# automerge/automerge-classic

Hardware: AMD Instinct MI355X
Metric: CRDT ops/sec applied (bulk replay) (higher is better)
Workload: dtype u32

## Files before the change

### automerge_classic_amd/csrc/am355_api.hip

```cpp
#include "am355_ctx.h"
#include "am355_scan.h"

static bool ctx_init(am355_ctx* c) {
  {
    unsigned hw = std::thread::hardware_concurrency();
    const char* env = getenv("AM355_HOST_THREADS");
    unsigned want = env && atoi(env) > 0 ? (unsigned)atoi(env) : std::min(hw ? hw : 4u, 64u);
    c->pool.reset(new HostPool(want > 1 ? want - 1 : 0));
  }
  int prio_low = 0, prio_high = 0;
  (void)hipDeviceGetStreamPriorityRange(&prio_low, &prio_high);
  auto make_stream = [](Stream& s, int prio) { return hipStreamCreateWithPriority(&s.h, hipStreamNonBlocking, prio) == hipSuccess; };
  if (!make_stream(c->stream, prio_high)) return false;
  {
    const char* env = getenv("AM355_HASH_CUS");
    int want = env ? atoi(env) : 0;
    bool made = false;
    if (want > 0) {
      hipDeviceProp_t prop;
      if (hipGetDeviceProperties(&prop, c->device) == hipSuccess && prop.multiProcessorCount > want) {
        int n_cu = prop.multiProcessorCount;
        std::vector<uint32_t> mask((size_t)(n_cu + 31) / 32, 0u);
        for (int k = 0; k < want; k++) { int cu = n_cu - 1 - k; mask[(size_t)cu / 32] |= 1u << (cu % 32); }
        made = hipExtStreamCreateWithCUMask(&c->stream2.h, (uint32_t)mask.size(), mask.data()) == hipSuccess;
// ... 54 lines not shown
extern "C" int am355_get_hashes(const am355_ctx* c, uint8_t* out) {
  if (!c || !out) return AM355_E_ARG;
  if (!c->replayed || !c->h_hashes.p || c->is_document) return AM355_E_STATE;
  memcpy(out, c->h_hashes.p, 32 * (size_t)c->n_changes);
  return AM355_OK;
}

extern "C" int am355_arena_epoch(const am355_ctx* c, uint64_t* epoch) {
  if (!c || !epoch) return AM355_E_ARG;
  *epoch = c->arena_epoch;
  return AM355_OK;
}

extern "C" int am355_get_hashes_range(const am355_ctx* c, uint32_t first, uint32_t count, uint8_t* out) {
  if (!c || (!out && count)) return AM355_E_ARG;
  if (!c->replayed || !c->h_hashes.p || c->is_document) return AM355_E_STATE;
  if (first > c->n_changes || count > c->n_changes - first) return AM355_E_ARG;
  if (count) memcpy(out, (const uint8_t*)c->h_hashes.p + 32 * (size_t)first, 32 * (size_t)count);
  return AM355_OK;
}

extern "C" int am355_applied_in_input_order(const am355_ctx* c, int* yes) {
  if (!c || !yes) return AM355_E_ARG;
  if (!c->replayed || c->is_document) return AM355_E_STATE;
  bool ok = c->pending_change.empty() && c->n_pending == 0 && c->applied_change.size() == c->n_changes;
  for (uint32_t i = 0; ok && i < c->n_changes; i++) ok = c->applied_change[i] == i;
  *yes = ok ? 1 : 0;
  return AM355_OK;
}

extern "C" int am355_resident_counters(const am355_ctx* c, uint64_t out[3]) {
  if (!c || !out) return AM355_E_ARG;
  out[0] = c->n_resident_calls;
  out[1] = c->n_resident_fallbacks;
  out[2] = c->n_resorder_calls;
  return AM355_OK;
}

extern "C" int am355_resident_maps_only_calls(const am355_ctx* c, uint64_t* out) {
  if (!c || !out) return AM355_E_ARG;
  *out = c->n_maps_only_calls;
  return AM355_OK;
}

extern "C" int am355_set_resident_new_actors(am355_ctx* c, int on) {
  if (!c) return AM355_E_ARG;
  c->resident_new_actors = on != 0;
  return AM355_OK;
}

extern "C" int am355_resident_new_actor_calls(const am355_ctx* c, uint64_t out[2]) {
  if (!c || !out) return AM355_E_ARG;
  out[0] = c->n_new_actor_calls;
  out[1] = c->n_rank_rewrites;
  return AM355_OK;
}

extern "C" int am355_set_resident_map_merge(am355_ctx* c, int on) {
  if (!c) return AM355_E_ARG;
  c->resident_map_merge = on != 0;
  return AM355_OK;
}

extern "C" int am355_resident_map_merge_calls(const am355_ctx* c, uint64_t out[2]) {
  if (!c || !out) return AM355_E_ARG;
  out[0] = c->n_map_merge_calls;
  out[1] = c->n_map_merge_declined;
  return AM355_OK;
}

extern "C" int am355_set_resident_new_objects(am355_ctx* c, int on) {
  if (!c) return AM355_E_ARG;
  c->resident_new_objects = on != 0;
  return AM355_OK;
}

extern "C" int am355_resident_new_object_calls(const am355_ctx* c, uint64_t out[2]) {
  if (!c || !out) return AM355_E_ARG;
  out[0] = c->n_new_object_calls;
  out[1] = c->n_new_object_declined;
  return AM355_OK;
}

extern "C" int am355_get_raw(const am355_ctx* c, const uint8_t** arena, const uint64_t** offsets, uint32_t* n) {
  if (!c || !c->staged) return AM355_E_STATE;
  if (arena) *arena = c->raw.data();
  if (offsets) *offsets = c->raw_off.data();
  if (n) *n = c->n_changes;
  return AM355_OK;
}

extern "C" int am355_get_applied(const am355_ctx* c, uint32_t* out, uint32_t* n_applied) {
  if (!c || !n_applied) return AM355_E_ARG;
  if (!c->replayed || c->is_document) return AM355_E_STATE;
  *n_applied = (uint32_t)c->applied_change.size();
  if (out) memcpy(out, c->applied_change.data(), 4 * c->applied_change.size());
  return AM355_OK;
}

extern "C" int am355_test_sort(am355_ctx* c, uint64_t* keys, uint32_t* vals, uint32_t n, int key_bits) {
  if (!c) return AM355_E_ARG;
  (void)hipSetDevice(c->device);
  DevBuf ka, kb, va, vb, ws;
  if (!ka.ensure(8 * (size_t)n + 8) || !kb.ensure(8 * (size_t)n + 8) || !va.ensure(4 * (size_t)n + 4) || !vb.ensure(4 * (size_t)n + 4) || !ws.ensure(sort_workspace_bytes(n)))
    return fail(c, AM355_E_NOMEM, "alloc");
  hipStream_t st = c->stream;
  (void)hipMemcpyAsync(ka.p, keys, 8 * (size_t)n, hipMemcpyHostToDevice, st);
  (void)hipMemcpyAsync(va.p, vals, 4 * (size_t)n, hipMemcpyHostToDevice, st);
  int res = radix_sort_pairs(ka.as<uint64_t>(), va.as<uint32_t>(), kb.as<uint64_t>(), vb.as<uint32_t>(), n, 0, key_bits, ws.p, st);
  (void)hipMemcpyAsync(keys, res ? kb.p : ka.p, 8 * (size_t)n, hipMemcpyDeviceToHost, st);
  (void)hipMemcpyAsync(vals, res ? vb.p : va.p, 4 * (size_t)n, hipMemcpyDeviceToHost, st);
  HIPCHK(c, hipStreamSynchronize(st));
  HIPCHK(c, hipGetLastError());
  return AM355_OK;
}

extern "C" int am355_test_scan(am355_ctx* c, const uint32_t* in, uint32_t* out, uint32_t n, uint32_t* total) {
  if (!c) return AM355_E_ARG;
  (void)hipSetDevice(c->device);
  DevBuf di, dt, ws;
  if (!di.ensure(4 * (size_t)n + 4) || !dt.ensure(4) || !ws.ensure(scan_workspace_bytes(n))) return fail(c, AM355_E_NOMEM, "alloc");
  hipStream_t st = c->stream;
  (void)hipMemcpyAsync(di.p, in, 4 * (size_t)n, hipMemcpyHostToDevice, st);
  exclusive_scan_u32(di.as<uint32_t>(), di.as<uint32_t>(), n, dt.as<uint32_t>(), ws.p, st);
  (void)hipMemcpyAsync(out, di.p, 4 * (size_t)n, hipMemcpyDeviceToHost, st);
  (void)hipMemcpyAsync(total, dt.p, 4, hipMemcpyDeviceToHost, st);
  HIPCHK(c, hipStreamSynchronize(st));
  return AM355_OK;
}

namespace {
struct TestImage {
  DevBuf d;
  uint8_t* p = nullptr;
  size_t bytes = 0;
  bool up(const void* host, size_t n, hipStream_t st) {
    if (!d.ensure(n + 16)) return false;
    p = (uint8_t*)(((uintptr_t)d.p + 15) & ~(uintptr_t)15);
    bytes = n;
    if (n) (void)hipMemcpyAsync(p, host, n, hipMemcpyHostToDevice, st);
    return true;
  }
  void down(void* host, hipStream_t st) const {
    if (bytes) (void)hipMemcpyAsync(host, p, bytes, hipMemcpyDeviceToHost, st);
  }
  uint32_t* words(size_t off = 0) const { return (uint32_t*)p + off; }
};
int test_finish(am355_ctx* c) {
  HIPCHK(c, hipStreamSynchronize(c->stream));
  HIPCHK(c, hipGetLastError());
  return AM355_OK;
}

__global__ __launch_bounds__(BLOCK) void k_test_carry_produce(const uint32_t* __restrict__ v, uint32_t n, CarryScan cs) {
  __shared__ uint32_t s[BLOCK / WAVE];
  const uint32_t i = gtid();
  (void)carry_publish(cs, i < n ? v[i] : 0u, s);
}
__global__ __launch_bounds__(BLOCK) void k_test_carry_consume(const uint32_t* __restrict__ v, uint32_t n, CarryScan cs, uint32_t* __restrict__ out,
                                                              uint32_t* __restrict__ out_wg, uint32_t* __restrict__ wg_total) {
  __shared__ uint32_t s[BLOCK / WAVE];
  const uint32_t i = gtid();
  const uint32_t x = i < n ? v[i] : 0u;
  uint32_t total;
  const uint32_t in_wg = block_exclusive_scan_u32(x, s, &total);
  const uint32_t pre = carry_prefix(cs, x, s);
// ... 170 lines not shown
    db.down(buf, st);
    return test_finish(c);
  });
}

extern "C" int am355_test_copy(am355_ctx* c, uint8_t* dst, size_t dst_bytes, const uint8_t* src, size_t src_bytes, int src_pinned, const uint32_t* ranges, uint32_t n_ranges,
                               uint32_t* n_added) {
  if (!c || !dst || !src || (!ranges && n_ranges)) return AM355_E_ARG;
  return guarded(c, [&]() -> int {
    (void)hipSetDevice(c->device);
    hipStream_t st = c->stream;
    TestImage dd, ds;
    HostBuf hs;
    const uint8_t* s0;
    if (!dd.up(dst, dst_bytes, st)) return fail(c, AM355_E_NOMEM, "alloc");
    if (src_pinned) {
      if (!hs.ensure(src_bytes + 16)) return fail(c, AM355_E_NOMEM, "alloc");
      uint8_t* h = (uint8_t*)(((uintptr_t)hs.p + 15) & ~(uintptr_t)15);
      memcpy(h, src, src_bytes);
      s0 = h;
    } else {
      if (!ds.up(src, src_bytes, st)) return fail(c, AM355_E_NOMEM, "alloc");
      s0 = ds.p;
    }
    CopyRanges r;
    for (uint32_t k = 0; k < n_ranges; k++) {
      const uint32_t* q = ranges + 3 * (size_t)k;
      if ((size_t)q[0] + q[2] > dst_bytes || (size_t)q[1] + q[2] > src_bytes) return fail(c, AM355_E_ARG, "am355_test_copy: range %u leaves its buffer", k);
      if (!r.add(dd.p + q[0], s0 + q[1], q[2])) return fail(c, AM355_E_ARG, "am355_test_copy: add() refused range %u", k);
    }
    if (n_added) *n_added = r.n;
    launch_copy_ranges(r, st);
    dd.down(dst, st);
    return test_finish(c);
  });
}

extern "C" int am355_test_signal_words(am355_ctx* c, const uint32_t* a, uint32_t n_a, const uint32_t* b, uint32_t n_b, uint32_t seq, uint32_t* host_words,
                                       uint32_t host_words_n, uint32_t* seq_word) {
  if (!c || (!a && n_a) || (!b && n_b) || !host_words || !seq_word || (size_t)n_a + n_b > host_words_n) return AM355_E_ARG;
  return guarded(c, [&]() -> int {
    (void)hipSetDevice(c->device);
    hipStream_t st = c->stream;
    TestImage da, db;
    HostBuf h;
    if (!da.up(a, 4 * (size_t)n_a, st) || !db.up(b, 4 * (size_t)n_b, st) || !h.ensure(4 * ((size_t)host_words_n + 1))) return fail(c, AM355_E_NOMEM, "alloc");
    uint32_t* hw = h.as<uint32_t>();
    memcpy(hw, host_words, 4 * (size_t)host_words_n);
    hw[host_words_n] = *seq_word;
    launch_signal_words(da.words(), n_a, db.words(), n_b, hw, (volatile uint32_t*)(hw + host_words_n), seq, st);
    int rc = test_finish(c);
    if (rc != AM355_OK) return rc;
    memcpy(host_words, hw, 4 * (size_t)host_words_n);
    *seq_word = hw[host_words_n];
    return AM355_OK;
  });
}

extern "C" int am355_test_carried_scan(am355_ctx* c, const uint32_t* v, uint32_t n, uint32_t* out, uint32_t* out_wg, uint32_t* wg_total) {
  if (!c || !v || !out || !out_wg || !wg_total || !n || n > 0xffffff00u) return AM355_E_ARG;
  return guarded(c, [&]() -> int {
    (void)hipSetDevice(c->device);
    hipStream_t st = c->stream;
    const uint32_t wgs = (n + BLOCK - 1) / BLOCK;
    const size_t group_words = ((size_t)(wgs >> CARRY_GROUP_SHIFT) + 1) * CARRY_GROUP_STRIDE;
    TestImage dv;
    DevBuf d_out, d_wg, d_tot, d_carry;
    if (!dv.up(v, 4 * (size_t)n, st) || !d_out.ensure(4 * (size_t)n) || !d_wg.ensure(4 * (size_t)n) || !d_tot.ensure(4 * (size_t)wgs) ||
        !d_carry.ensure(4 * (wgs + group_words)))
      return fail(c, AM355_E_NOMEM, "alloc");
    CarryScan cs;
    cs.wg_sum = d_carry.as<uint32_t>();
    cs.group_sum = cs.wg_sum + wgs;
    (void)hipMemsetAsync(cs.group_sum, 0, 4 * group_words, st);
    hipLaunchKernelGGL(k_test_carry_produce, dim3(wgs), dim3(BLOCK), 0, st, (const uint32_t*)dv.words(), n, cs);
    hipLaunchKernelGGL(k_test_carry_consume, dim3(wgs), dim3(BLOCK), 0, st, (const uint32_t*)dv.words(), n, cs, d_out.as<uint32_t>(), d_wg.as<uint32_t>(), d_tot.as<uint32_t>());
    (void)hipMemcpyAsync(out, d_out.p, 4 * (size_t)n, hipMemcpyDeviceToHost, st);
    (void)hipMemcpyAsync(out_wg, d_wg.p, 4 * (size_t)n, hipMemcpyDeviceToHost, st);
    (void)hipMemcpyAsync(wg_total, d_tot.p, 4 * (size_t)wgs, hipMemcpyDeviceToHost, st);
    return test_finish(c);
  });
}

extern "C" int am355_get_rows(am355_ctx* c, uint32_t* obj_actor, uint32_t* obj_ctr, uint32_t* key_actor, uint32_t* key_ctr, uint32_t* key_off,
                              uint32_t* key_len, uint32_t* action, uint32_t* val_tl, uint32_t* val_off, uint32_t* pred_num, uint32_t* id_ctr,
                              uint32_t* id_actor, uint8_t* insert, uint32_t* succ_cnt) {
  if (!c || !c->replayed) return AM355_E_STATE;
  if (c->shard_world > 1) return fail(c, AM355_E_UNSUPPORTED, "am355_get_rows on a sharded context (foreign rows are decoded as far as their object columns only)");
  (void)hipSetDevice(c->device);
  size_t N = c->n_ops;
  hipStream_t st = c->stream;
  auto pull = [&](void* dst, const void* src, size_t bytes) { if (dst && bytes) (void)hipMemcpyAsync(dst, src, bytes, hipMemcpyDeviceToHost, st); };
  pull(obj_actor, c->cols.obj_actor, 4 * N); pull(obj_ctr, c->cols.obj_ctr, 4 * N); pull(key_actor, c->cols.key_actor, 4 * N);
  pull(key_ctr, c->cols.key_ctr, 4 * N); pull(key_off, c->cols.key_off, 4 * N); pull(key_len, c->cols.key_len, 4 * N);
  pull(action, c->cols.action, 4 * N); pull(val_tl, c->cols.val_tl, 4 * N); pull(val_off, c->cols.val_off, 4 * N);
  pull(pred_num, c->cols.pred_num, 4 * N); pull(id_ctr, c->cols.id_ctr, 4 * N); pull(id_actor, c->cols.id_actor, 4 * N);
  pull(insert, c->cols.insert, N); pull(succ_cnt, c->mb.succ_cnt, 4 * N);
  HIPCHK(c, hipStreamSynchronize(st));
  return AM355_OK;
}

extern "C" int am355_load_changes(am355_ctx* c, const uint8_t* arena, const uint64_t* offsets, uint32_t n) { return guarded(c, [&]() { return load_changes_impl(c, arena, offsets, n); }); }
extern "C" int am355_load_document(am355_ctx* c, const uint8_t* doc, size_t len) { return guarded(c, [&]() { return load_document_impl(c, doc, len); }); }
extern "C" int am355_backend_load(am355_ctx* c, const uint8_t* doc, size_t len) { return guarded(c, [&]() { return backend_load_impl(c, doc, len); }); }
extern "C" int am355_replay(am355_ctx* c) { return guarded(c, [&]() { return replay_impl(c); }); }
extern "C" int am355_fetch_ir(am355_ctx* c, am355_patch_ir* out) { return guarded(c, [&]() { return fetch_ir_impl(c, out); }); }
extern "C" int am355_patch_json(am355_ctx* c, const char** json, size_t* len) { return guarded(c, [&]() { return patch_json_impl(c, json, len); }); }
extern "C" int am355_save(am355_ctx* c, uint32_t flags, const uint8_t** out_bytes, size_t* out_len) { return guarded(c, [&]() { return save_impl(c, flags, out_bytes, out_len); }); }
extern "C" int am355_doc_changes(am355_ctx* c, uint32_t flags, const uint8_t** arena, const uint64_t** offsets, uint32_t* n, const uint8_t** hashes) { return guarded(c, [&]() { return doc_changes_impl(c, flags, arena, offsets, n, hashes); }); }
extern "C" int am355_import_fragments(am355_ctx* c, const uint8_t* frags, const uint64_t* offsets, uint32_t world) { return guarded(c, [&]() { return import_fragments_impl(c, frags, offsets, world); }); }
extern "C" int am355_apply_changes(am355_ctx* c, const uint8_t* arena, const uint64_t* offsets, uint32_t n) { return guarded(c, [&]() { return apply_changes_impl(c, arena, offsets, n); }); }
extern "C" int am355_apply_patch_json(am355_ctx* c, const char** json, size_t* len) { return guarded(c, [&]() { return apply_patch_json_impl(c, json, len); }); }
extern "C" int am355_get_dep_graph(am355_ctx* c, const uint32_t** dep_first, const uint32_t** dep_index, uint32_t* n) { return guarded(c, [&]() { return get_dep_graph_impl(c, dep_first, dep_index, n); }); }
extern "C" int am355_sync_bloom_build(am355_ctx* c, const uint32_t* idx, uint32_t n, uint8_t* bits, size_t cap) {
  return guarded(c, [&]() { return sync_bloom_impl(c, idx, n, n, 10, 7, nullptr, 0, bits, cap, true); });
}
extern "C" int am355_sync_bloom_probe(am355_ctx* c, const uint32_t* idx, uint32_t n, uint32_t num_entries, uint32_t bits_per_entry, uint32_t num_probes, const uint8_t* bits,
                                      size_t n_bytes, uint8_t* contains) {
  return guarded(c, [&]() { return sync_bloom_impl(c, idx, n, num_entries, bits_per_entry, num_probes, bits, n_bytes, contains, n, false); });
}
```

### automerge_classic_amd/csrc/am355_ctx.h

```cpp
#pragma once
#include "../../include/am355.h"
#include "am355_decode.h"
#include "am355_merge.h"
#include "am355_bigcol.h"
#include "am355_encode.h"
#include "am355_prims.h"
#include "am355_render.h"
#include "am355_host.h"
#include "am355_pinflate.h"
#include "am355_history.h"
#include "am355_delta.h"
#include "am355_resorder.h"
#include "am355_apply.h"
#include "am355_sync.h"
#include "am355_sched.h"
#include "am355_hist.h"
#include "am355_canary.h"

#include <zlib.h>

#include <algorithm>
#include <atomic>
#include <chrono>
#include <cstdarg>
// ... 234 lines not shown
      cv_.wait(l, [&]() { return stop_ || state_.load(std::memory_order_acquire) == 1; });
      sleeping_.store(false, std::memory_order_release);
      if (stop_) return;
    }
  }
  static uint64_t now_us() { return (uint64_t)std::chrono::duration_cast<std::chrono::microseconds>(std::chrono::steady_clock::now().time_since_epoch()).count(); }
  std::function<void()> job_;
  std::atomic<int> state_{0};
  std::atomic<bool> sleeping_{false};
  std::mutex m_;
  std::condition_variable cv_;
  bool stop_ = false;
  std::thread t_;
};

struct Hash32 {
  uint8_t b[32];
  bool operator==(const Hash32& o) const { return memcmp(b, o.b, 32) == 0; }
};
struct Hash32Hasher {
  size_t operator()(const Hash32& h) const { size_t v; memcpy(&v, h.b, sizeof v); return v; }
};

}
using namespace am355_host;

struct am355_ctx {
  ~am355_ctx();
  int device = 0;
  Stream stream;
  Stream stream2;
  Stream stream3;
  Stream stream4;
  Event ev_fork, ev_join;
  Event ev[8];
  Event ev_parse, ev_b0, ev_b1;
  Event ev_counts, ev_runs;
  std::string err;
  uint32_t flags = 0;

  PinnedBytes raw;
  std::unique_ptr<HostPool> pool;
  std::unique_ptr<AsyncLane> lane;
  std::vector<uint64_t> raw_off;
  uint32_t n_changes = 0;
  DevBuf d_plan_totals;
  bool spec_launched = false;
  bool spec_large_launched = false;
  uint32_t spec_cap_ops = 0, spec_cap_preds = 0;
  uint32_t hint_ops = 0, hint_preds = 0, hint_large = 0;
  bool staged = false, replayed = false, ir_fetched = false;
  int ir_copy_enqueued = 0;
  bool prefetch_ir = false;
  bool has_unknown_cols = false;
  bool staging_in_flight = false;
  bool is_document = false;
  ChangeMeta doc_meta{};
  std::vector<uint32_t> doc_actor_rank;
  DevBuf d_arena, d_offsets, d_metas;
  uint64_t arena_epoch = 1;
  CopyRanges pending_up;
  std::vector<uint32_t> breaks_dev;
  void* breaks_dev_ptr = nullptr;
  HostBuf h_breaks_ahead;
  bool offsets_on_device = false;
  HostBuf h_metas, h_offsets, h_sig;
  uint32_t sig_seq = 0;
  Event ev_s1;
  Event ev_fills;
  Event ev_sched;
  Event ev_plan, ev_tables;
  void* counts_zeroed_at = nullptr; size_t counts_zeroed = 0;
  bool phase_events = false;
  bool inline_fills = true;
  DevBuf d_big, d_bigvals, d_ks;
  HostBuf h_biginfo;
  BigColDesc doc_cols{};
  bool doc_serial = false;
  DevBuf d_entries, d_amap_base, d_amap_prov, d_slots, d_first_idx, d_hashes, d_hash_tab, d_min_idx, d_has_dep, d_words, d_slot_rank, d_scan1, d_plan_sums, d_dep_idx, d_self_idx, d_rank_ids;
  HostBuf h_dep_idx, h_self_idx, h_amap, h_amap_base;
  HostBuf h_slots, h_hashes, h_has_dep, h_words, h_stage, h_s1;
  DevBuf d_s1;
  ChangeBrief* hp_briefs = nullptr;
  uint32_t* hp_distinct = nullptr;
  bool have_host_metas = false;
  uint32_t amap_cap = 0, slot_mask = 0, hash_mask = 0;
  bool used_fast_path = false;

  std::vector<ChangePlan> plans;
  std::vector<uint32_t> applied_change, applied_op_base;
  struct DocSum {
    static constexpr size_t PIECE = (size_t)4 << 20;
    std::thread t;
    std::unique_ptr<std::atomic<uint8_t>[]> copied;
    size_t n_pieces = 0;
    bool pending = false, ok = false;
    bool wait() {
      if (t.joinable()) t.join();
      pending = false;
      return ok;
    }
    ~DocSum() { if (t.joinable()) t.join(); }
  } doc_sum;
  std::vector<uint8_t> doc_bytes;
  std::vector<uint8_t> saved;
  HistoryOutput history;
  bool history_ok = false; uint32_t history_flags = 0;
  std::vector<std::vector<uint8_t>> inflate_scratch;
  std::vector<std::unique_ptr<PInflateJob>> pinflate_jobs;
  std::vector<uint32_t> doc_col_rows;
  std::vector<std::pair<uint32_t, std::vector<uint8_t>>> doc_chg_cols;
  std::vector<uint8_t> doc_tail;
  bool doc_other_ops_cols = false;
  DevBuf d_save, d_enc, d_encout;
  HostBuf h_encout;
  std::vector<uint32_t> amap;
  std::vector<ActorSpan> spans;
  std::vector<uint32_t> actor_tab_off;
  std::vector<std::string> actors;
  std::vector<uint32_t> clock_actor;
  std::vector<uint64_t> clock_seq;
  std::vector<uint8_t> heads;
  uint32_t n_applied = 0, n_pending = 0;
  uint64_t n_ops = 0, n_preds = 0, max_op = 0;
  DevBuf d_plans, d_amap, d_tables;
  ActorSpan* p_spans = nullptr;
  uint32_t* p_tab_off = nullptr;

  DevBuf d_cols, d_pred, d_merge, d_sort, d_ir, d_counts;
  OpCols cols{};
  MergeBufs mb{};
  PatchIR ir{};
  HostBuf h_counts;
  Counts counts{};

  HostBuf h_ir, h_rows;
  am355_patch_ir hir{};
  std::vector<uint32_t> actor_off;
  std::vector<uint8_t> actor_bytes;
  std::string json;

  am355_stats stats{};

  std::vector<uint32_t> pending_change;
  std::vector<uint32_t> pass_first_row;
  DevBuf d_delta, d_pass, d_delta_edit, d_sched, d_hist;
  HostBuf h_sched;
  bool key_unbounded = false;
  bool device_scheduled = false;
  HostBuf h_delta;
  DeltaBufs delta{};
  bool h_tables_current = false, h_tables_were_current = false;
  bool batch_list_only = false;
  void* apply_tail = nullptr;
  ApplyPatch apply;
  bool apply_ready = false;
  std::vector<uint32_t> dep_first, dep_index;
  bool dep_graph_ready = false;
  DevBuf d_sync;
  std::vector<uint32_t> stream_breaks;
  bool breaks_exact = true, children_hazard = false, in_apply = false;
  uint32_t graph_mode = 0, doc_n_changes = 0, sched_prefix = 0;
  bool doc_head_index_known = true, sched_graph_after = true;
  bool doc_graph_known = false;
  uint64_t doc_rows = 0;
  bool doc_rows_known = false;
  bool no_history = false;
  DevBuf d_breaks;
  HostBuf h_delta_tabs;
  bool state_checked = false;
  std::string apply_json;

  struct Keep { bool want = false; uint32_t n_changes = 0; uint64_t n_ops = 0, n_preds = 0; } keep;
  uint32_t cols_cap_ops = 0, cols_cap_preds = 0;
  bool resident_valid = false;
  struct ResidentMark { uint32_t lost[8] = {}; uint32_t n_changes = 0; uint64_t n_ops = 0, n_preds = 0; } res_mark;
  uint32_t seed_list_inc = 0;
  std::vector<uint32_t> hash_index;
  uint32_t hash_index_n = 0;
  std::vector<uint32_t> res_rank_of;
  uint32_t res_rank_n = 0;
  struct ActorMemo { std::vector<uint8_t> bytes; std::vector<uint32_t> ranks; };
  std::vector<ActorMemo> res_actor_memo;
  DevBuf d_pos, d_order_alt, d_resorder;
  uint32_t* order_alt_ptr = nullptr;
  HostBuf h_resorder;
  bool pos_valid = false;
  bool ir_stale = false;
  uint64_t n_resorder_calls = 0;
  uint64_t n_maps_only_calls = 0;
  HostBuf h_res_metas;
  uint32_t res_dep_base = 0;
  std::vector<uint32_t> res_dep_first, res_dep_index;
  uint64_t n_resident_calls = 0, n_resident_fallbacks = 0;
  bool resident_new_actors = false;
  uint64_t n_new_actor_calls = 0, n_rank_rewrites = 0;
  bool resident_map_merge = false;
  uint64_t n_map_merge_calls = 0, n_map_merge_declined = 0;
  bool resident_new_objects = false;
  uint64_t n_new_object_calls = 0, n_new_object_declined = 0;
  DevBuf d_map_alt, d_mapmerge;
  am355_ir_map* map_alt_ptr = nullptr;
  std::string resident_why;

  uint32_t shard_rank = 0, shard_world = 1;
  std::vector<uint8_t> stitched;
  void* shard_comm = nullptr;
  DevBuf d_shard_send, d_shard_recv, d_shard_sizes;
  HostBuf h_shard_sizes, h_shard_frags;
  std::vector<uint64_t> shard_fragment_bytes;
// ... 89 lines not shown
```

### automerge_classic_amd/csrc/am355_decode.h

```cpp
#pragma once
#include "am355_internal.h"

namespace am355 {
struct ParseFills {
  uint32_t* p[5];
  uint64_t n_words[5];
  uint32_t value[5];
  uint32_t n;
};
void parse_changes_host(const uint8_t* arena, const uint64_t* offsets, uint32_t n_changes, ChangeMeta* metas, uint32_t* n_entries);
void launch_parse_changes(const uint8_t* arena, const uint64_t* offsets, uint32_t n_changes, ChangeMeta* metas, uint32_t* n_entries, const ParseFills& fills,
                          hipStream_t st, bool fat = false);
int change_wave_class(const ChangeMeta& m);
void launch_hash_changes(const uint8_t* arena, const uint64_t* offsets, uint32_t n, uint8_t* hashes, uint32_t* min_idx, uint32_t* hash_tab,
                         uint32_t tab_mask, uint32_t* flags, hipStream_t st);
void launch_deps_resolve(const uint8_t* arena, const ChangeMeta* metas, const uint8_t* hashes, uint32_t n, const uint32_t* hash_tab, uint32_t tab_mask,
                         const uint32_t* min_idx, uint8_t* has_dependent, uint32_t* fast_flags, uint32_t* dep_idx, uint32_t* self_idx, hipStream_t st);
void launch_actor_intern(const uint8_t* arena, ChangeMeta* metas, uint32_t n, const uint32_t* amap_base, uint32_t* amap, uint32_t amap_cap,
                         unsigned long long* slots, uint32_t slot_mask, uint32_t* first_idx, uint32_t* flags, uint32_t* fast_flags, uint32_t* distinct,
                         void* rank_ids, ChangeBrief* briefs, uint32_t* slot_rank, unsigned long long* block_sums, uint32_t* plan_words, hipStream_t st,
                         ChangeBrief* host_briefs = nullptr);
size_t rank_ids_bytes();
size_t plan_block_sums_bytes(uint32_t n);
uint32_t distinct_capacity();
void launch_plan(const ChangeBrief* briefs, uint32_t n, const uint32_t* distinct, const uint32_t* slot_rank, uint32_t slot_mask, const unsigned long long* block_sums,
                 ChangePlan* plans, ChangePlan* plans_serial, const uint32_t* words, const uint32_t* plan_words, HostSignals* sig, uint32_t seq, hipStream_t st,
                 PlanTotals* dev_totals = nullptr, uint32_t* host_s1 = nullptr);
void launch_decode_speculative(const uint8_t* arena, const ChangeMeta* metas, const ChangePlan* plans, uint32_t n_changes, const PlanTotals* totals, uint32_t cap_ops,
                               uint32_t cap_preds, uint32_t cap_distinct, const uint32_t* amap, const uint32_t* slot_rank, OpCols cols, uint32_t* flags, hipStream_t st,
                               hipStream_t aux, bool with_large, uint32_t shard_rank = 0, uint32_t shard_world = 1);
void launch_decode_planned(const uint8_t* arena, const ChangeMeta* metas, const ChangePlan* plans, const ChangePlan* plans_serial, uint32_t n_changes,
                           uint32_t n_small, uint32_t n_large, uint32_t n_serial, const uint32_t* amap, const uint32_t* slot_rank, OpCols cols, uint32_t* flags,
                           hipStream_t st, hipStream_t aux, uint32_t shard_rank = 0, uint32_t shard_world = 1);
void launch_decode_columns(const uint8_t* arena, const ChangeMeta* metas, const ChangePlan* plans, uint32_t n_small, uint32_t n_large, uint32_t n_serial,
                           const uint32_t* amap, const uint32_t* slot_rank, OpCols cols, uint32_t* flags, hipStream_t st, hipStream_t aux, uint32_t shard_rank = 0,
                           uint32_t shard_world = 1);
void launch_doc_count(const uint8_t* arena, ChangeMeta* meta, hipStream_t st);
void launch_decode_document(const uint8_t* arena, const ChangeMeta* meta, const ChangePlan* plan, const uint32_t* actor_rank, OpCols cols,
                            uint32_t* flags, hipStream_t st);
void launch_keystr_expand(const uint32_t* run_start, const uint32_t* run_off, const uint32_t* run_len, const uint32_t* n_runs, uint32_t n_rows,
                          uint32_t* key_off, uint32_t* key_len, hipStream_t st);
}
```

### automerge_classic_amd/csrc/am355_decode.hip

```cpp
#include "am355_decode.h"
#include "am355_scan.h"

#include <cstdlib>

namespace am355 {

struct __attribute__((packed)) U8B {
  uint64_t v;
};
__host__ __device__ __forceinline__ uint64_t load_u64_unaligned(const uint8_t* p) { return ((const U8B*)p)->v; }
#ifdef AM355_LDS_IS_DISTINCT
__device__ __forceinline__ uint64_t load_u64_unaligned(LdsBytes p) { return ((const __attribute__((address_space(3))) U8B*)p)->v; }
#endif

template <class P>
struct CurT {
  P p;
  uint32_t off, len;
  uint64_t win;
  uint32_t win_off;
  __host__ __device__ __forceinline__ CurT() {}
  static constexpr uint32_t WIN_EMPTY = 0xffffff00u;
  __host__ __device__ __forceinline__ CurT(P p_, uint32_t off_, uint32_t len_) : p(p_), off(off_), len(len_), win(0), win_off(WIN_EMPTY) {}
  __host__ __device__ __forceinline__ uint32_t byte_at(uint32_t o) {
// ... 1034 lines not shown
  if (s_fallback) { if (t == 0) plan_words[0] = 1; return; }
#pragma unroll
  for (uint32_t k = 0; k < PER; k++) {
    const uint32_t a = t + k * BLOCK;
    if (a >= nd) break;
    uint32_t rank = 0;
    const uint32_t my_len = rec[k].len;
    static_assert(PLAN_ID_MAX == 32, "rank_actors compares four 64-bit words");
    const unsigned long long m0 = rec[k].w[0], m1 = rec[k].w[1], m2 = rec[k].w[2], m3 = rec[k].w[3];
    for (uint32_t j = 0; j < nd; j++) {
      const unsigned long long x0 = s_id[j][0], x1 = s_id[j][1], x2 = s_id[j][2], x3 = s_id[j][3];
      const bool less = x0 != m0 ? x0 < m0 : x1 != m1 ? x1 < m1 : x2 != m2 ? x2 < m2 : x3 != m3 ? x3 < m3 : s_len[j] < my_len;
      rank += less ? 1u : 0u;
    }
    slot_rank[slot_of[k]] = rank;
  }
}

__global__ __launch_bounds__(WAVE) void k_actor_first(ChangeMeta* __restrict__ metas, uint32_t n, const uint32_t* __restrict__ amap_base,
                                                       const uint32_t* __restrict__ amap, uint32_t amap_cap, const uint32_t* __restrict__ first_idx,
                                                       uint32_t* __restrict__ fast_flags) {
  wave_priority_high();
  uint32_t c = blockIdx.x, lane = threadIdx.x;
  if (c >= n) return;
  ChangeMeta* m = &metas[c];
  if (m->flags) return;
  uint32_t base = amap_base[c], ne = m->n_entries;
  if ((uint64_t)base + ne > amap_cap) return;
  uint32_t mx = 0;
  for (uint32_t k = lane; k < ne; k += WAVE) {
    uint32_t f = first_idx[amap[base + k]];
    mx = f > mx ? f : mx;
  }
  for (int d = WAVE / 2; d >= 1; d >>= 1) {
    uint32_t o = __shfl_xor(mx, d);
    mx = o > mx ? o : mx;
  }
  if (lane == 0) {
    m->max_first = mx;
    if (mx > c) atomicOr(fast_flags, (uint32_t)FF_LATE_ACTOR);
  }
}

__global__ __launch_bounds__(BLOCK) void k_actor_check(const uint8_t* __restrict__ arena, ChangeMeta* __restrict__ metas, uint32_t n,
                                                       const uint32_t* __restrict__ amap_base, const uint32_t* __restrict__ amap, uint32_t amap_cap,
                                                       const uint32_t* __restrict__ first_idx, uint32_t* __restrict__ flags, uint32_t* __restrict__ fast_flags,
                                                       ChangeBrief* __restrict__ briefs, const uint32_t* __restrict__ distinct, const RankId* __restrict__ rank_ids,
                                                       uint32_t* __restrict__ slot_rank, unsigned long long* __restrict__ block_sums, uint32_t* __restrict__ plan_words,
                                                       ChangeBrief* __restrict__ host_briefs) {
  wave_priority_high();
  __shared__ unsigned long long s_scan[BLOCK / WAVE][3];
  if (blockIdx.x + 1 == gridDim.x) {
    rank_actors(distinct, rank_ids, slot_rank, plan_words);
    return;
  }
  uint32_t c = gtid();
  const bool in_range = c < n;
  ChangeBrief br{};
  if (in_range) {
    ChangeMeta* m = &metas[c];
    br.seq = m->seq;
    br.start_op = (uint32_t)m->start_op;
    br.n_ops = m->n_ops;
    br.n_preds = m->n_preds;
    br.n_entries = m->n_entries;
    br.author_slot = m->author_slot;
    br.flags_fits = m->flags;
    if (!m->flags) {
      int wc = wave_class_of(*m);
      if (wc >= 1) br.flags_fits |= 0x80000000u;
      if (wc == 2) br.flags_fits |= 0x40000000u;
      if (m->pad & 1) br.flags_fits |= 0x20000000u;
    }
    briefs[c] = br;
    if (host_briefs) host_briefs[c] = br;
  }
  const bool valid = in_range && !(br.flags_fits & 0x1fffffffu);
  const bool has = valid && br.n_ops != 0;
  const bool small = has && (br.flags_fits & 0x40000000u), large = has && !small && (br.flags_fits & 0x80000000u), serial = has && !small && !large;
  unsigned long long ex[3], t1[3], t2[3];
  block_scan3(valid ? br.n_ops : 0u, valid ? br.n_preds : 0u, valid ? br.n_entries : 0u, s_scan, ex, t1);
  block_scan3(small ? 1u : 0u, large ? 1u : 0u, serial ? 1u : 0u, s_scan, ex, t2);
  uint32_t mx_op = has ? br.start_op + br.n_ops - 1 : 0u, bad = in_range ? (br.flags_fits & 0x1fffffffu) : 0u, unknown = in_range ? (br.flags_fits & 0x20000000u) : 0u;
  for (int d = WAVE / 2; d >= 1; d >>= 1) {
    uint32_t o = __shfl_xor(mx_op, d), ob = __shfl_xor(bad, d), ou = __shfl_xor(unknown, d);
    mx_op = o > mx_op ? o : mx_op;
    bad |= ob;
    unknown |= ou;
  }
  if ((threadIdx.x & (WAVE - 1)) == 0) {
    if (mx_op) atomicMax(&plan_words[1], mx_op);
    if (bad) atomicOr(&plan_words[2], bad);
    if (unknown) atomicOr(&plan_words[3], 1u);
  }
  if (threadIdx.x == 0) {
    unsigned long long* out = block_sums + (size_t)blockIdx.x * PLAN_SUMS;
    out[0] = t1[0]; out[1] = t1[1]; out[2] = t1[2]; out[3] = t2[0]; out[4] = t2[1]; out[5] = t2[2];
  }
}

__global__ __launch_bounds__(BLOCK) void k_plan_apply(const ChangeBrief* __restrict__ briefs, uint32_t n, const uint32_t* __restrict__ slot_rank, uint32_t slot_mask,
                                                      const unsigned long long* __restrict__ block_sums, ChangePlan* __restrict__ plans,
                                                      ChangePlan* __restrict__ plans_serial, const uint32_t* __restrict__ words, const uint32_t* __restrict__ plan_words,
                                                      const uint32_t* __restrict__ distinct, HostSignals* sig, uint32_t seq, PlanTotals* __restrict__ dev_totals,
                                                      uint32_t* __restrict__ host_s1) {
  wave_priority_high();
  __shared__ unsigned long long s_scan[BLOCK / WAVE][3];
  __shared__ unsigned long long s_base[6];
  {
    unsigned long long p0 = 0, p1 = 0, p2 = 0, p3 = 0, p4 = 0, p5 = 0;
    for (uint32_t j = threadIdx.x; j < blockIdx.x; j += BLOCK) {
      const unsigned long long* q = block_sums + (size_t)j * PLAN_SUMS;
      p0 += q[0]; p1 += q[1]; p2 += q[2]; p3 += q[3]; p4 += q[4]; p5 += q[5];
    }
    unsigned long long ex[3], t1[3], t2[3];
    block_scan3(p0, p1, p2, s_scan, ex, t1);
    block_scan3(p3, p4, p5, s_scan, ex, t2);
    if (threadIdx.x == 0) { s_base[0] = t1[0]; s_base[1] = t1[1]; s_base[2] = t1[2]; s_base[3] = t2[0]; s_base[4] = t2[1]; s_base[5] = t2[2]; }
    __syncthreads();
  }
  const uint32_t c = gtid();
  const bool in_range = c < n;
  ChangeBrief br{};
  if (in_range) br = briefs[c];
  const bool valid = in_range && !(br.flags_fits & 0x1fffffffu);
  const bool has = valid && br.n_ops != 0;
  const bool small = has && (br.flags_fits & 0x40000000u), large = has && !small && (br.flags_fits & 0x80000000u), serial = has && !small && !large;
  unsigned long long e1[3], e2[3], t1[3], t2[3];
  block_scan3(valid ? br.n_ops : 0u, valid ? br.n_preds : 0u, valid ? br.n_entries : 0u, s_scan, e1, t1);
  block_scan3(small ? 1u : 0u, large ? 1u : 0u, serial ? 1u : 0u, s_scan, e2, t2);
  if (has) {
    ChangePlan pl{c, (uint32_t)(s_base[0] + e1[0]), (uint32_t)(s_base[1] + e1[1]), (uint32_t)(s_base[2] + e1[2]),
                  br.author_slot <= slot_mask ? slot_rank[br.author_slot] : 0u, br.n_entries};
    if (small) plans[(uint32_t)(s_base[3] + e2[0])] = pl;
    else if (large) plans[n - 1 - (uint32_t)(s_base[4] + e2[1])] = pl;
    else plans_serial[(uint32_t)(s_base[5] + e2[2])] = pl;
  }
  if (blockIdx.x + 1 == gridDim.x && host_s1) {
    const uint32_t nd = distinct[0] < DISTINCT_CAP ? distinct[0] : DISTINCT_CAP;
    const uint32_t* src = words;
    for (uint32_t i = threadIdx.x; i < 16; i += BLOCK) host_s1[i] = src[i];
    uint32_t* hd = host_s1 + 16;
    for (uint32_t i = threadIdx.x; i < 1 + nd; i += BLOCK) hd[i] = distinct[i];
    const unsigned long long* ids = (const unsigned long long*)(distinct + 2 + DISTINCT_CAP);
    unsigned long long* hids = (unsigned long long*)(hd + 2 + DISTINCT_CAP);
    for (uint32_t i = threadIdx.x; i < nd; i += BLOCK) hids[i] = ids[i];
    __threadfence_system();
    __syncthreads();
  }
  if (blockIdx.x + 1 == gridDim.x && threadIdx.x == 0) {
    unsigned long long ops = s_base[0] + t1[0], preds = s_base[1] + t1[1], ent = s_base[2] + t1[2];
    PlanTotals z{};
    z.n_ops = (uint32_t)ops; z.n_preds = (uint32_t)preds; z.n_entries = (uint32_t)ent;
    z.n_small = (uint32_t)(s_base[3] + t2[0]); z.n_large = (uint32_t)(s_base[4] + t2[1]); z.n_serial = (uint32_t)(s_base[5] + t2[2]);
    z.max_op = plan_words[1];
    z.fallback = (plan_words[0] || ops >= 0x7ffffff0ull || preds >= 0xfffffff0ull || ent >= 0xfffffff0ull) ? 1u : 0u;
    z.flags_a = words[0] | plan_words[2]; z.fast_a = words[1]; z.total_entries = words[2]; z.n_distinct = distinct[0];
    z.reserved[0] = plan_words[3];
    if (dev_totals) *dev_totals = z;
    signal_host((uint32_t*)&sig->plan, (const uint32_t*)&z, sizeof(PlanTotals) / 4, &sig->plan_seq, seq);
  }
}

struct Rle {
  Cur c;
  int state;
  int64_t count;
  bool have_last, last_null;
  int64_t last;
  uint32_t last_off, last_len;
};

__device__ __forceinline__ void rle_init(Rle& r, const uint8_t* p, uint32_t len) {
  r.c = Cur(p, 0, len);
  r.state = 0;
  r.count = 0;
  r.have_last = false;
  r.last_null = true;
  r.last = 0;
  r.last_off = r.last_len = 0;
}

enum { RT_UINT = 0, RT_INT = 1, RT_UTF8 = 2 };

struct RVal {
  bool is_null;
  int64_t i;
  uint32_t off, len;
};

template <int TYPE>
__device__ __forceinline__ bool rle_raw(Rle& r, RVal& v) {
  v.is_null = false;
  if (TYPE == RT_UINT) {
    uint64_t u;
    if (!read_uleb(r.c, u)) return false;
    v.i = (int64_t)u;
  } else if (TYPE == RT_INT) {
    if (!read_sleb(r.c, v.i)) return false;
  } else {
    uint64_t n;
    if (!read_uleb(r.c, n)) return false;
    v.off = r.c.off;
    v.len = (uint32_t)n;
    if (!skip_bytes(r.c, n)) return false;
  }
  return true;
}

template <int TYPE>
__device__ __forceinline__ bool rle_same(const Rle& r, const RVal& v) {
  if (!r.have_last || r.last_null) return false;
  if (TYPE == RT_UTF8) {
    return r.last_len == v.len && bytes_equal(r.c.p, r.last_off, v.off, v.len, r.c.len);
  }
  return r.last == v.i;
}

template <int TYPE>
__device__ __forceinline__ void rle_set_last(Rle& r, const RVal& v) {
  r.have_last = true;
  r.last_null = v.is_null;
  r.last = v.i;
  r.last_off = v.off;
  r.last_len = v.len;
}

template <int TYPE>
__device__ bool rle_next(Rle& r, RVal& v) {
  if (r.count == 0 && r.c.off >= r.c.len) {
    v.is_null = true;
    v.i = 0;
    v.off = v.len = 0;
    return true;
  }
  if (r.count == 0) {
    int64_t n;
    if (!read_sleb(r.c, n)) return false;
    if (n > 1) {
      RVal x;
      x.off = x.len = 0;
      x.i = 0;
      if (!rle_raw<TYPE>(r, x)) return false;
// ... 865 lines not shown
      if (nul) k = 0;
      int64_t incl = carry + wave_incl_scan_i64(k, lane);
      carry = __shfl(incl, WAVE - 1);
      if (i < n) {
        if ((uint64_t)incl > n_preds_cap) { err |= F_BAD_RLE; k = 0; incl = 0; }
        o.pred_num[base + i] = (uint32_t)k;
        o.pred_first[base + i] = pl.pred_base + (uint32_t)(incl - k);
      }
    }
    total_preds = (uint64_t)carry > n_preds_cap ? 0 : (uint32_t)carry;
  }
  load_col(C_PRED_ACTOR);
  err |= L.err;
  for (uint32_t j = lane; j < total_preds; j += WAVE) {
    bool nul; int64_t v;
    wv_row_value<false>(L, j, nul, v, err);
    uint32_t r = 0;
    if (nul) err |= F_UNSUPPORTED;
    else if ((uint64_t)v >= pl.n_actors) err |= F_BAD_ROW;
    else r = L.rank[v];
    o.pred_actor[pl.pred_base + j] = r;
  }
  load_col(C_PRED_CTR);
  err |= L.err;
  {
    int64_t carry = 0;
    for (uint32_t j0 = 0; j0 < total_preds; j0 += WAVE) {
      uint32_t j = j0 + lane;
      bool nul = true; int64_t d = 0;
      if (j < total_preds) wv_row_value<true>(L, j, nul, d, err);
      int64_t abs = carry + wave_incl_scan_i64(nul ? 0 : d, lane);
      carry = __shfl(abs, WAVE - 1);
      if (j < total_preds) {
        if (nul) err |= F_UNSUPPORTED;
        else if (abs < 0 || (uint64_t)abs >= NONE32) err |= F_OVERFLOW;
        o.pred_ctr[pl.pred_base + j] = (uint32_t)abs;
      }
    }
  }
  }
  if (err) atomicOr(flags, err);
}

int change_wave_class(const ChangeMeta& m) { return wave_class_of(m); }

void launch_parse_changes(const uint8_t* arena, const uint64_t* offsets, uint32_t n_changes, ChangeMeta* metas, uint32_t* n_entries, const ParseFills& fills,
                          hipStream_t st, bool fat) {
  if (!n_changes && !fills.n) return;
  if (fat) hipLaunchKernelGGL(k_parse_changes<true>, dim3(n_changes ? n_changes : 64), dim3(WAVE), 0, st, arena, offsets, n_changes, metas, n_entries, fills);
  else hipLaunchKernelGGL(k_parse_changes<false>, dim3(n_changes ? n_changes : 64), dim3(WAVE), 0, st, arena, offsets, n_changes, metas, n_entries, fills);
}

void launch_hash_changes(const uint8_t* arena, const uint64_t* offsets, uint32_t n, uint8_t* hashes, uint32_t* min_idx, uint32_t* hash_tab,
                         uint32_t tab_mask, uint32_t* flags, hipStream_t st) {
  if (!n) return;
  hipLaunchKernelGGL(k_hash_changes, dim3((n + HASH_LANES - 1) / HASH_LANES), dim3(2 * HASH_LANES), 0, st, arena, offsets, n, hashes, min_idx, flags);
  AM355_LAUNCH_INDEPENDENT(k_hash_insert, dim3((n + BLOCK - 1) / BLOCK), dim3(BLOCK), st, (const uint8_t*)hashes, n, hash_tab, tab_mask, min_idx);
}

void launch_deps_resolve(const uint8_t* arena, const ChangeMeta* metas, const uint8_t* hashes, uint32_t n, const uint32_t* hash_tab, uint32_t tab_mask,
                         const uint32_t* min_idx, uint8_t* has_dependent, uint32_t* fast_flags, uint32_t* dep_idx, uint32_t* self_idx, hipStream_t st) {
  if (!n) return;
  AM355_LAUNCH_INDEPENDENT(k_deps_resolve, dim3(n), dim3(WAVE), st, arena, metas, hashes, n, hash_tab, tab_mask, min_idx, has_dependent, fast_flags, dep_idx,
                           self_idx);
}

void launch_actor_intern(const uint8_t* arena, ChangeMeta* metas, uint32_t n, const uint32_t* amap_base, uint32_t* amap, uint32_t amap_cap,
                         unsigned long long* slots, uint32_t slot_mask, uint32_t* first_idx, uint32_t* flags, uint32_t* fast_flags, uint32_t* distinct,
                         void* rank_ids, ChangeBrief* briefs, uint32_t* slot_rank, unsigned long long* block_sums, uint32_t* plan_words, hipStream_t st,
                         ChangeBrief* host_briefs) {
  if (n)
    hipLaunchKernelGGL(k_actor_intern, dim3(n), dim3(WAVE), 0, st, arena, metas, n, amap_base, amap, amap_cap, slots, slot_mask, first_idx, flags,
                       fast_flags, distinct, (RankId*)rank_ids);
  if (n) hipLaunchKernelGGL(k_actor_first, dim3(n), dim3(WAVE), 0, st, metas, n, amap_base, (const uint32_t*)amap, amap_cap, (const uint32_t*)first_idx, fast_flags);
  hipLaunchKernelGGL(k_actor_check, dim3((n + BLOCK - 1) / BLOCK + 1), dim3(BLOCK), 0, st, arena, metas, n, amap_base, (const uint32_t*)amap, amap_cap,
                     (const uint32_t*)first_idx, flags, fast_flags, briefs, (const uint32_t*)distinct, (const RankId*)rank_ids, slot_rank, block_sums, plan_words,
                     host_briefs);
}

size_t rank_ids_bytes() { return sizeof(RankId) * PLAN_RANK_MAX; }

size_t plan_block_sums_bytes(uint32_t n) { return sizeof(unsigned long long) * PLAN_SUMS * ((size_t)(n + BLOCK - 1) / BLOCK + 1); }

void launch_plan(const ChangeBrief* briefs, uint32_t n, const uint32_t* distinct, const uint32_t* slot_rank, uint32_t slot_mask, const unsigned long long* block_sums,
                 ChangePlan* plans, ChangePlan* plans_serial, const uint32_t* words, const uint32_t* plan_words, HostSignals* sig, uint32_t seq, hipStream_t st,
                 PlanTotals* dev_totals, uint32_t* host_s1) {
  uint32_t nb = (n + BLOCK - 1) / BLOCK;
  hipLaunchKernelGGL(k_plan_apply, dim3(nb ? nb : 1), dim3(BLOCK), 0, st, briefs, n, slot_rank, slot_mask, block_sums, plans, plans_serial, words, plan_words,
                     distinct, sig, seq, dev_totals, host_s1);
}

uint32_t distinct_capacity() { return DISTINCT_CAP; }

__global__ __launch_bounds__(WAVE) void k_doc_count(const uint8_t* __restrict__ arena, ChangeMeta* __restrict__ meta) {
  uint32_t lane = threadIdx.x;
  if (lane > 1) return;
  int slot = lane == 0 ? C_ACTION : C_PRED_NUM;
  uint64_t cnt, sum;
  bool ok = rle_count_sum(arena + meta->base + meta->col_off[slot], meta->col_len[slot], cnt, sum);
  if (!ok) { atomicOr(&meta->flags, (uint32_t)F_BAD_RLE); return; }
  if (lane == 0) meta->n_ops = (uint32_t)cnt; else meta->n_preds = (uint32_t)sum;
}

void launch_doc_count(const uint8_t* arena, ChangeMeta* meta, hipStream_t st) {
  AM355_LAUNCH_INDEPENDENT(k_doc_count, dim3(1), dim3(WAVE), st, arena, meta);
}

__global__ __launch_bounds__(BLOCK) void k_keystr_expand(const uint32_t* __restrict__ run_start, const uint32_t* __restrict__ run_off,
                                                          const uint32_t* __restrict__ run_len, const uint32_t* __restrict__ n_runs_p, uint32_t n_rows,
                                                          uint32_t* __restrict__ key_off, uint32_t* __restrict__ key_len) {
  uint32_t row = gtid();
  if (row >= n_rows) return;
  uint32_t nr = *n_runs_p;
  uint32_t off = 0, len = NONE32;
  if (nr && row < run_start[nr]) {
    uint32_t lo = 0, hi = nr;
    while (hi - lo > 1) {
      uint32_t mid = (lo + hi) >> 1;
      if (run_start[mid] <= row) lo = mid; else hi = mid;
    }
    off = run_off[lo];
    len = run_len[lo];
  }
  key_off[row] = off;
  key_len[row] = len;
}

void launch_keystr_expand(const uint32_t* run_start, const uint32_t* run_off, const uint32_t* run_len, const uint32_t* n_runs, uint32_t n_rows,
                          uint32_t* key_off, uint32_t* key_len, hipStream_t st) {
  if (!n_rows) return;
  AM355_LAUNCH_INDEPENDENT(k_keystr_expand, dim3((n_rows + BLOCK - 1) / BLOCK), dim3(BLOCK), st, run_start, run_off, run_len, n_runs, n_rows, key_off, key_len);
}

void launch_decode_document(const uint8_t* arena, const ChangeMeta* meta, const ChangePlan* plan, const uint32_t* actor_rank, OpCols cols,
                            uint32_t* flags, hipStream_t st) {
  ActorXlate x{actor_rank, nullptr, 0, 1};
  AM355_LAUNCH_INDEPENDENT(k_decode_columns, dim3(1, T_NUM_DOC), dim3(WAVE), st, arena, meta, plan, 1u, x, cols, flags, 0);
}

static uint32_t decode_group_split(uint32_t n_waves, uint32_t shard_world, bool large_class = false) {
  static const uint32_t split_max = []() { const char* e = getenv("AM355_DECODE_SPLIT_MAX"); return e && atol(e) > 0 ? (uint32_t)atol(e) : 1536u; }();
  return (shard_world <= 1 && n_waves <= (large_class ? 512u : split_max)) ? 4u : 1u;
}

void launch_decode_columns(const uint8_t* arena, const ChangeMeta* metas, const ChangePlan* plans, uint32_t n_small, uint32_t n_large, uint32_t n_serial,
                           const uint32_t* amap, const uint32_t* slot_rank, OpCols cols, uint32_t* flags, hipStream_t st, hipStream_t aux, uint32_t shard_rank,
                           uint32_t shard_world) {
  ActorXlate x{amap, slot_rank, shard_rank, shard_world};
  if (n_large && n_small + n_large <= 1024) { n_large += n_small; n_small = 0; }
  hipStream_t s2 = (n_small && aux) ? aux : st;
  if (n_small) hipLaunchKernelGGL(k_decode_wave<WaveLdsSmall>, dim3(n_small, decode_group_split(n_small, shard_world)), dim3(WAVE), 0, st, arena, metas, plans, n_small, x, cols, flags, DecodeGate{});
  if (n_large) hipLaunchKernelGGL(k_decode_wave<WaveLdsLarge>, dim3(n_large, decode_group_split(n_large, shard_world, true)), dim3(WAVE), 0, s2, arena, metas, plans + n_small, n_large, x, cols, flags, DecodeGate{});
  if (n_serial)
    AM355_LAUNCH_INDEPENDENT(k_decode_columns, dim3((n_serial + WAVE - 1) / WAVE, T_NUM), dim3(WAVE), s2, arena, metas, plans + n_small + n_large, n_serial,
                             x, cols, flags, 0);
}

void launch_decode_planned(const uint8_t* arena, const ChangeMeta* metas, const ChangePlan* plans, const ChangePlan* plans_serial, uint32_t n_changes,
                           uint32_t n_small, uint32_t n_large, uint32_t n_serial, const uint32_t* amap, const uint32_t* slot_rank, OpCols cols, uint32_t* flags,
                           hipStream_t st, hipStream_t aux, uint32_t shard_rank, uint32_t shard_world) {
  ActorXlate x{amap, slot_rank, shard_rank, shard_world};
  hipStream_t s2 = (n_small && aux) ? aux : st;
  if (n_small) hipLaunchKernelGGL(k_decode_wave<WaveLdsSmall>, dim3(n_small, decode_group_split(n_small, shard_world)), dim3(WAVE), 0, st, arena, metas, plans, n_small, x, cols, flags, DecodeGate{});
  if (n_large) hipLaunchKernelGGL(k_decode_wave<WaveLdsLarge>, dim3(n_large, decode_group_split(n_large, shard_world, true)), dim3(WAVE), 0, s2, arena, metas, plans + (n_changes - n_large), n_large, x, cols, flags, DecodeGate{});
  if (n_serial)
    AM355_LAUNCH_INDEPENDENT(k_decode_columns, dim3((n_serial + WAVE - 1) / WAVE, T_NUM), dim3(WAVE), s2, arena, metas, plans_serial, n_serial, x, cols, flags, 0);
// ... 16 lines not shown
```

### automerge_classic_amd/csrc/am355_internal.h

```cpp
#pragma once
#include "am355_device.h"

namespace am355 {

enum ColSlot { C_OBJ_ACTOR, C_OBJ_CTR, C_KEY_ACTOR, C_KEY_CTR, C_KEY_STR, C_INSERT, C_ACTION, C_VAL_LEN, C_VAL_RAW, C_PRED_NUM, C_PRED_ACTOR, C_PRED_CTR,
               C_ID_ACTOR, C_ID_CTR, C_NUM };

struct ChangeMeta {
  uint64_t base;
  uint32_t len;
  uint32_t flags;
  uint64_t seq, start_op;
  uint32_t n_entries;
  uint32_t author_slot;
  uint32_t max_first;
  uint32_t pad;
  uint32_t n_deps, deps_off;
  uint32_t actor_off, actor_len;
  uint32_t n_other, others_off;
  uint32_t col_off[C_NUM], col_len[C_NUM];
  uint32_t n_ops, n_preds;
};

struct ChangeBrief {
  uint64_t seq;
  uint32_t start_op, n_ops, n_preds, n_entries, author_slot;
  uint32_t flags_fits;
};

enum FastFlag : uint32_t {
  FF_DUP_HASH = 1u << 0,
  FF_MISSING_DEP = 1u << 1,
  FF_LATE_DEP = 1u << 2,
  FF_LATE_ACTOR = 1u << 3,
  FF_CAPACITY = 1u << 4
};

struct ChangePlan {
  uint32_t change;
  uint32_t op_base;
  uint32_t pred_base;
  uint32_t amap_base;
  uint32_t author;
  uint32_t n_actors;
};

struct PlanTotals {
  uint32_t n_ops, n_preds, n_entries;
  uint32_t n_small, n_large, n_serial;
  uint32_t max_op;
  uint32_t fallback;
  uint32_t flags_a, fast_a, total_entries, n_distinct;
  uint32_t reserved[4];
};

__host__ __device__ inline bool decode_gate_open(const PlanTotals& t, uint32_t cap_ops, uint32_t cap_preds, uint32_t cap_distinct) {
  return !t.fallback && !t.flags_a && !t.fast_a && t.n_ops <= cap_ops && t.n_preds <= cap_preds && t.n_distinct <= cap_distinct;
}
struct DecodeGate {
  const PlanTotals* totals = nullptr;
  uint32_t cap_ops = 0, cap_preds = 0, cap_distinct = 0, n_changes = 0, large = 0;
};

struct HostSignals {
  volatile uint32_t plan_seq;    uint32_t pad0[15];
  PlanTotals plan;
  volatile uint32_t counts_seq;  uint32_t pad1[15];
  uint32_t counts[32];
  volatile uint32_t runs_seq;    uint32_t pad2[15];
  uint32_t runs[16];
  volatile uint32_t final_seq;   uint32_t pad3[15];
  uint32_t final_counts[16];
  volatile uint32_t resorder_seq;  uint32_t pad4[15];
  uint32_t resorder[16];
  volatile uint32_t delta_mid_seq; uint32_t pad5[15];
  uint32_t delta_mid[16];
  volatile uint32_t delta_end_seq; uint32_t pad6[15];
  uint32_t delta_end[16];
  volatile uint32_t mapmerge_seq;  uint32_t pad7[15];
  uint32_t mapmerge[16];
};

struct ActorSpan {
  uint32_t start_op, n_ops, op_base;
};

struct OpCols {
  uint32_t *obj_actor, *obj_ctr;
  uint32_t *key_actor, *key_ctr;
  uint32_t *key_off, *key_len;
  uint32_t *action, *val_tl, *val_off;
  uint32_t *pred_first, *pred_num;
  uint32_t *id_ctr, *id_actor;
  uint8_t* insert;
  uint32_t *pred_actor, *pred_ctr;
};

__host__ __device__ __forceinline__ uint32_t shard_owner(uint32_t obj_actor, uint32_t obj_ctr, uint32_t world) {
  return obj_actor == NONE32 ? 0u : (obj_ctr + obj_actor) % world;
}

}
```

### automerge_classic_amd/csrc/am355_merge.h

```cpp
#pragma once
#include "am355_internal.h"
#include "am355_scan.h"
#include "am355_prims.h"
#include "../../include/am355.h"
#include <stddef.h>

namespace am355 {

struct Counts {
  uint32_t flags;
  uint32_t n_map_emit;
  uint32_t n_list_ins;
  uint32_t n_list_upd;
  uint32_t n_objects;
  uint32_t max_key_len;
  uint32_t n_edits;
  uint32_t pad;
  uint32_t n_runs;
  uint32_t euler_done;
  uint32_t n_erecs;
  uint32_t n_head_children;
  uint32_t n_quirk;
  uint32_t n_list_inc;
  uint32_t map_group_big;
  uint32_t reserved[1];
};

struct MapKeyStats {
  uint32_t or_len, or_inv_len;
  uint32_t or_b[4], or_inv_b[4];
};
constexpr uint32_t MAP_KEY_STATS_WORD = 16;

struct MergeBufs {
  const uint8_t* arena;
  OpCols ops;
  uint32_t n_ops, n_preds, n_actors;
  uint32_t shard_rank, shard_world;
  uint32_t first_row, seed_list_inc, row_stride;
  const uint32_t* actor_tab_off;
  const ActorSpan* spans;
  uint32_t bits_ctr, bits_actor;
  uint32_t *obj_row, *ref_row, *succ_cnt, *inc_cnt, *val_cnt, *obj_index;
  unsigned long long *inc_sum, *last_inc;
  uint8_t* kind;
  uint32_t *em_row;
  unsigned long long* em_trig;
  uint32_t *ins_row;
  uint32_t *upd_row;
  uint64_t *key_a, *key_b;
  uint32_t *val_a, *val_b;
  void* sort_ws;
  uint32_t *first_child;
  uint32_t *next_sib;
  uint32_t *child_head;
  uint32_t *child_next;
  uint32_t *head_child;
  uint32_t *obj_n;
  uint32_t *run_heads, *row_run;
  uint32_t *list_vis, *list_cnt;
  CarryScan cs_ins, cs_make, cs_runs, cs_vis, cs_cnt, cs_erec;
  unsigned long long *euler_a, *euler_b;
  uint32_t *order;
  uint32_t *scan_a, *scan_b;
  uint32_t *obj_first_pos;
  void* scan_ws;
  Counts* counts;
  size_t counts_bytes;
  void* zero_base;
  size_t zero_bytes;
  HostSignals* sig;
  uint32_t sig_seq;
  void* fill_base;
  size_t fill_bytes;
};

size_t merge_counts_bytes(uint32_t n_ops);
void merge_bind_counts(MergeBufs& b, void* d_counts_block);

struct PatchIR {
  am355_ir_object* obj;
  am355_ir_map* map;
  am355_ir_edit* edit;
  uint32_t *e_row;
  uint32_t *e_elem;
  uint32_t *e_index;
  uint32_t *e_flags;
};

size_t merge_scratch_pairs(uint32_t n_ops);

bool wait_host_signal(volatile uint32_t* seq_word, uint32_t seq, hipStream_t st);

enum { MERGE_FILL_ROWS = 1, MERGE_FILL_TABLES = 2 };
bool merge_prepare(MergeBufs& b, hipStream_t aux, int what = MERGE_FILL_ROWS | MERGE_FILL_TABLES, const FillRanges* extra = nullptr);
void merge_run(MergeBufs& b, PatchIR& ir, Counts* h_counts, hipStream_t st, hipEvent_t ev_counts, hipEvent_t ev_runs, bool resolved = false);
void merge_run_maps(MergeBufs& b, PatchIR& ir, Counts* h_counts, hipStream_t st);
void merge_resolve(MergeBufs& b, hipStream_t st);

struct MapMergeBufs {
  uint32_t T0, n_new;
  uint32_t n_map, n_obj;
  const am355_ir_map* map;
  am355_ir_map* map_new;
  uint32_t *dead, *dead_ex;
  uint32_t *obj_base;
  uint32_t *row_gap;
  uint32_t *srt_gap, *srt_oi;
  uint32_t *words;
  HostSignals* sig;
  uint32_t sig_seq;
};
enum MapMergeWord { MM_DECLINE = 0,
                    MM_OTHER_ROWS = 1,
                    MM_N_NEW = 2,
                    MM_MAX_KEY = 3,
                    MM_N_DEAD = 4,
                    MM_FLAGS = 5,
                    MM_WORDS = 8 };
constexpr uint32_t MAPMERGE_ROWS_MAX = 16384;
size_t mapmerge_bytes(uint32_t n_new, uint32_t n_map, uint32_t n_obj);
void mapmerge_bind(MapMergeBufs& m, void* block, uint32_t n_new, uint32_t n_map, uint32_t n_obj);
void mapmerge_find(MergeBufs& b, const PatchIR& ir, MapMergeBufs& m, hipStream_t st);
void mapmerge_write(MergeBufs& b, PatchIR& ir, MapMergeBufs& m, uint32_t n_new_rec, uint32_t max_key, hipStream_t st);

void doc_patch(MergeBufs& b, PatchIR& ir, Counts* h_counts, hipStream_t st);

struct SaveBufs {
  uint32_t *map_flag, *map_ex, *upd_flag, *upd_ex, *upd_cnt, *pos_of, *list_off, *final_pos, *src_of, *map_perm;
  uint32_t *obj_rank, *rank_obj, *base_by_rank;
  uint32_t *map_begin, *map_end, *list_begin, *list_end;
  uint64_t *succ_key_a, *succ_key_b;
  uint32_t *succ_val_a, *succ_val_b;
  uint32_t* words;
  OpCols out;
};
void save_phase1(MergeBufs& b, SaveBufs& s, hipStream_t st);
void save_phase2(MergeBufs& b, PatchIR& ir, SaveBufs& s, const uint32_t* words, uint32_t n_obj, uint32_t n_ins, const uint32_t* doc_actor, hipStream_t st);

}
```

### automerge_classic_amd/csrc/am355_merge.hip

```cpp
#include "am355_merge.h"
#include "am355_prims.h"
#include "am355_rows.h"

#include <algorithm>
#include <atomic>
#include <chrono>
#include <cstdio>
#include <cstdlib>
#include <cstring>

namespace am355 {

__global__ __launch_bounds__(BLOCK) void k_resolve(MergeBufs b) {
  wave_priority_high();
  uint32_t g = b.first_row + gtid();
  const bool in_range = g < b.n_ops;
  if (b.seed_list_inc && gtid() == 0) atomicAdd(&b.counts->n_list_inc, b.seed_list_inc);
  const OpCols& o = b.ops;
  uint32_t err = 0;
  uint32_t a = in_range ? o.action[g] : 1;
  bool ins = in_range && o.insert[g] != 0;
  unsigned long long my_id = in_range ? pack_id(o.id_ctr[g], o.id_actor[g]) : 0;

  uint32_t oa = in_range ? o.obj_actor[g] : NONE32, oc = in_range ? o.obj_ctr[g] : 0;
// ... 535 lines not shown
  if (m.sig) signal_host(m.sig->mapmerge, m.words, MM_WORDS, &m.sig->mapmerge_seq, m.sig_seq);
}

__global__ __launch_bounds__(BLOCK) void k_mm_place(MergeBufs b, MapMergeBufs m, const uint32_t* __restrict__ perm, uint32_t n_rec) {
  const uint32_t k = gtid();
  if (k >= n_rec) return;
  const uint32_t g = b.em_row[perm[k]], gap = m.row_gap[g - m.T0];
  m.srt_gap[k] = gap;
  m.srt_oi[k] = obj_index_of(b, b.obj_row[g]);
  m.map_new[gap - m.dead_ex[gap] + k] = map_record_of(b, g);
}

__global__ __launch_bounds__(BLOCK) void k_mm_write(PatchIR ir, MapMergeBufs m, uint32_t n_rec, uint32_t rec_blocks) {
  if (blockIdx.x < rec_blocks) {
    const uint32_t i = gtid();
    if (i >= m.n_map || m.dead[i]) return;
    uint32_t lo = 0, hi = n_rec;
    while (lo < hi) { const uint32_t mid = (lo + hi) >> 1; if (m.srt_gap[mid] <= i) lo = mid + 1; else hi = mid; }
    m.map_new[i - m.dead_ex[i] + lo] = m.map[i];
    return;
  }
  const uint32_t oi = (blockIdx.x - rec_blocks) * BLOCK + threadIdx.x;
  if (oi >= m.n_obj) return;
  const uint32_t first = m.obj_base[oi], end = m.obj_base[oi + 1];
  uint32_t lo = 0, hi = n_rec;
  while (lo < hi) { const uint32_t mid = (lo + hi) >> 1; if (m.srt_oi[mid] < oi) lo = mid + 1; else hi = mid; }
  const uint32_t in_front = lo;
  hi = n_rec;
  while (lo < hi) { const uint32_t mid = (lo + hi) >> 1; if (m.srt_oi[mid] <= oi) lo = mid + 1; else hi = mid; }
  const uint32_t begin_new = first - m.dead_ex[first] + in_front, end_new = end - m.dead_ex[end] + lo;
  ir.obj[oi].map_begin = end_new > begin_new ? begin_new : 0u;
  ir.obj[oi].map_end = end_new > begin_new ? end_new : 0u;
}

static int bits_for(uint64_t max_value) {
  int b = 1;
  while (b < 64 && (max_value >> b)) b++;
  return b;
}

struct ListKeyBits {
  int b_row, b_ctr, b_actor;
};

__global__ __launch_bounds__(BLOCK) void k_list_keys(MergeBufs b, uint64_t* __restrict__ keys, uint32_t* __restrict__ vals, uint32_t n, ListKeyBits kb) {
  uint32_t i = gtid();
  if (i >= n) return;
  uint32_t g = b.ins_row[i];
  uint32_t ref = b.ref_row[g];
  uint64_t is_head = ref == NONE32 ? 1 : 0;
  uint64_t parent = is_head ? b.obj_row[g] : ref;
  uint64_t mask_c = (1ull << kb.b_ctr) - 1, mask_a = (1ull << kb.b_actor) - 1;
  uint64_t k = is_head << (kb.b_row + kb.b_ctr + kb.b_actor) | parent << (kb.b_ctr + kb.b_actor) | (~(uint64_t)b.ops.id_ctr[g] & mask_c) << kb.b_actor |
               (~(uint64_t)b.ops.id_actor[g] & mask_a);
  keys[i] = k;
  vals[i] = g;
}

__global__ __launch_bounds__(BLOCK) void k_list_link(MergeBufs b, const uint64_t* __restrict__ keys, const uint32_t* __restrict__ vals, uint32_t n,
                                                     ListKeyBits kb) {
  uint32_t j = gtid();
  if (j >= n) return;
  int sh = kb.b_ctr + kb.b_actor;
  uint64_t pk = keys[j] >> sh;
  uint32_t v = vals[j];
  bool is_head = (pk >> kb.b_row) != 0;
  bool first = j == 0 || (keys[j - 1] >> sh) != pk;
  bool last = j + 1 == n || (keys[j + 1] >> sh) != pk;
  if (first) {
    uint32_t parent = (uint32_t)(pk & ((1ull << kb.b_row) - 1));
    b.first_child[is_head ? b.n_ops + parent : parent] = v;
  }
  b.next_sib[v] = last ? NONE32 : vals[j + 1];
}

constexpr uint32_t SEG_SORT_MAX = 256;

__device__ __forceinline__ uint32_t parent_slot(const MergeBufs& b, uint32_t g) {
  uint32_t ref = b.ref_row[g];
  return ref == NONE32 ? b.n_ops + b.obj_row[g] : ref;
}

constexpr uint32_t HEAD_CHILD_MAX = 2048;
constexpr uint32_t HEAD_CHILD_THREADS = 1024;

__global__ __launch_bounds__(BLOCK) void k_child_push(MergeBufs b) {
  wave_priority_high();
  uint32_t i = gtid();
  bool in_range = i < b.counts->n_list_ins;
  uint32_t v = in_range ? b.ins_row[i] : 0;
  bool head_child = in_range && b.ref_row[v] == NONE32;
  if (in_range) b.child_next[v] = atomicExch(&b.child_head[parent_slot(b, v)], v);
  uint32_t slot = wave_append(&b.counts->n_head_children, head_child);
  if (head_child && slot < HEAD_CHILD_MAX) b.head_child[slot] = v;
}

__global__ __launch_bounds__(HEAD_CHILD_THREADS) void k_head_children(MergeBufs b) {
  wave_priority_high();
  __shared__ unsigned long long s_id[HEAD_CHILD_MAX];
  __shared__ uint32_t s_obj[HEAD_CHILD_MAX], s_row[HEAD_CHILD_MAX];
  const uint32_t n = b.counts->n_head_children;
  if (n == 0 || n > HEAD_CHILD_MAX) return;
  for (uint32_t k = threadIdx.x; k < n; k += HEAD_CHILD_THREADS) {
    uint32_t v = b.head_child[k];
    s_row[k] = v;
    s_obj[k] = b.obj_row[v];
    s_id[k] = pack_id(b.ops.id_ctr[v], b.ops.id_actor[v]);
  }
  __syncthreads();
  for (uint32_t k = threadIdx.x; k < n; k += HEAD_CHILD_THREADS) {
    const uint32_t obj = s_obj[k];
    const unsigned long long kv = s_id[k];
    unsigned long long best_id = 0;
    uint32_t greater = 0, best = NONE32;
    for (uint32_t j = 0; j < n; j++) {
      if (s_obj[j] != obj || j == k) continue;
      unsigned long long ku = s_id[j];
      if (ku > kv) greater++;
      else if (best == NONE32 || ku > best_id) { best = s_row[j]; best_id = ku; }
    }
    uint32_t v = s_row[k];
    b.next_sib[v] = best;
    if (greater == 0) b.first_child[b.n_ops + obj] = v;
  }
}

template <bool FROM_LINKS>
__global__ __launch_bounds__(BLOCK) void k_child_order(MergeBufs b, uint32_t* __restrict__ is_head) {
  wave_priority_high();
  __shared__ uint32_t s_red[BLOCK / WAVE];
  const uint32_t ni = b.counts->n_list_ins;
  if (blockIdx.x * BLOCK >= ni) return;
  uint32_t i = gtid();
  uint32_t head = 0;
  if (i < ni) {
    const OpCols& o = b.ops;
    uint32_t v = b.ins_row[i], ps = parent_slot(b, v);
    bool first, none_after;
    if (FROM_LINKS) {
      first = b.first_child[ps] == v;
      none_after = b.next_sib[v] == NONE32;
    } else if (ps >= b.n_ops && b.counts->n_head_children <= HEAD_CHILD_MAX) {
      first = none_after = false;
    } else {
      unsigned long long kv = pack_id(o.id_ctr[v], o.id_actor[v]), best_id = 0;
      uint32_t greater = 0, best = NONE32, steps = 0;
      bool abandoned = false;
      for (uint32_t u = b.child_head[ps]; u != NONE32; u = b.child_next[u]) {
        if (++steps > SEG_SORT_MAX) { abandoned = true; break; }
        if (u == v) continue;
        unsigned long long ku = pack_id(o.id_ctr[u], o.id_actor[u]);
        if (ku > kv) greater++;
        else if (best == NONE32 || ku > best_id) { best = u; best_id = ku; }
      }
      if (abandoned) {
        b.counts->pad = 1;
        b.next_sib[v] = NONE32;
        first = false;
        none_after = false;
      } else {
        b.next_sib[v] = best;
        if (greater == 0) b.first_child[ps] = v;
        first = greater == 0;
        none_after = best == NONE32;
      }
    }
    head = (i > 0 && ps == b.ins_row[i - 1] && first && none_after) ? 0u : 1u;
    is_head[i] = head;
  }
  carry_publish(b.cs_runs, head, s_red);
}

__global__ __launch_bounds__(BLOCK) void k_run_heads(MergeBufs b, const uint32_t* __restrict__ is_head, uint32_t* __restrict__ head_ex,
                                                     uint32_t* __restrict__ heads, uint32_t* __restrict__ row_run) {
  wave_priority_high();
  __shared__ uint32_t s_red[BLOCK / WAVE];
  const uint32_t n = b.counts->n_list_ins;
  if (blockIdx.x * BLOCK >= n) return;
  uint32_t i = gtid();
  uint32_t flag = i < n ? is_head[i] : 0;
  uint32_t k = carry_prefix(b.cs_runs, flag, s_red);
  if (i >= n) return;
  head_ex[i] = k;
  if (flag) {
    heads[k] = i;
    row_run[b.ins_row[i]] = k;
    if (i > 0) row_run[b.ins_row[i - 1]] = k - 1;
  }
  if (i + 1 == n) {
    uint32_t H = k + flag;
    heads[H] = n;
    row_run[b.ins_row[i]] = H - 1;
    b.counts->n_runs = H;
    if (b.sig) signal_host(b.sig->runs, (const uint32_t*)b.counts, 16, &b.sig->runs_seq, b.sig_seq);
  }
}

__device__ __forceinline__ unsigned long long euler_pack(uint32_t succ, uint32_t dist) { return (unsigned long long)dist << 32 | succ; }

__global__ __launch_bounds__(BLOCK) void k_euler_init_runs(MergeBufs b, const uint32_t* __restrict__ heads, const uint32_t* __restrict__ row_run,
                                                           unsigned long long* __restrict__ el) {
  wave_priority_high();
  uint32_t k = gtid();
  uint32_t H = b.counts->n_runs, END = 2 * H;
  if (k == 0) el[END] = euler_pack(END, 0);
  if (k >= H) return;
  uint32_t i0 = heads[k], i1 = heads[k + 1];
  uint32_t h = b.ins_row[i0], t = b.ins_row[i1 - 1];
  uint32_t fc = b.first_child[t], ns = b.next_sib[h], ref = b.ref_row[h];
  el[2 * (size_t)k] = euler_pack(fc != NONE32 ? 2 * row_run[fc] : 2 * k + 1, i1 - i0);
  el[2 * (size_t)k + 1] = euler_pack(ns != NONE32 ? 2 * row_run[ns] : (ref != NONE32 ? 2 * row_run[ref] + 1 : END), 0);
}

constexpr uint32_t EULER_LDS_ENTRIES = 16384;
constexpr uint32_t EULER_LDS_THREADS = 1024;
__global__ __launch_bounds__(EULER_LDS_THREADS) void k_euler_rank_lds(Counts* __restrict__ counts, unsigned long long* __restrict__ el) {
  wave_priority_high();
  __shared__ unsigned long long L[EULER_LDS_ENTRIES];
  __shared__ uint32_t s_wave[EULER_LDS_THREADS / WAVE];
  const uint32_t H = counts->n_runs, END = 2 * H, E = END + 1;
  if (H == 0 || E > EULER_LDS_ENTRIES) return;
  const uint32_t t = threadIdx.x, lane = t & (WAVE - 1), wv = t / WAVE;
  constexpr uint32_t PER = EULER_LDS_ENTRIES / EULER_LDS_THREADS;
  int rounds = 1;
  while ((E >> rounds) != 0) rounds++;
  unsigned long long e[PER];
  uint32_t ends = 0;
#pragma unroll
  for (uint32_t j = 0; j < PER; j++) {
    const uint32_t x = t + j * EULER_LDS_THREADS;
    e[j] = x < E ? el[x] : 0ull;
    ends += (x < END && (uint32_t)e[j] == END) ? 1u : 0u;
  }
  ends = wave_sum_u32(ends);
  if (lane == 0) s_wave[wv] = ends;
  __syncthreads();
  uint32_t paths = 0;
  for (uint32_t k = 0; k < EULER_LDS_THREADS / WAVE; k++) paths += s_wave[k];
  __syncthreads();
  if (paths == 1) {
    uint32_t* P = (uint32_t*)L;
    uint32_t* Wt = P + EULER_LDS_ENTRIES;
#pragma unroll
    for (uint32_t j = 0; j < PER; j++) {
      const uint32_t x = t + j * EULER_LDS_THREADS;
      if (x < E) P[x] = (uint32_t)e[j] << 16 | (x < END ? 1u : 0u);
      Wt[x] = 0;
    }
    __syncthreads();
    uint32_t pv[PER];
#pragma unroll
    for (uint32_t j = 0; j < PER; j++) {
      const uint32_t x = t + j * EULER_LDS_THREADS;
// ... 654 lines not shown
      fits &= f.add(b.order, 4 * ((size_t)N + 2), 0xffffffffu);
      fits &= f.add(b.first_child, 4 * (2 * (size_t)N + 4), 0xffffffffu);
      fits &= f.add(b.child_head, 4 * (2 * (size_t)N + 3), 0xffffffffu);
    }
  }
  if (extra)
    for (uint32_t k = 0; k < extra->n; k++) fits &= f.add(extra->p[k], 4 * (size_t)extra->n_words[k], extra->value[k]);
  if (!fits) return false;
  launch_fill_ranges(f, aux);
  return true;
}

static void order_map_emissions(MergeBufs& b, PatchIR& ir, const Counts* hc, hipStream_t st, uint32_t* ride_with_list_order = nullptr,
                                const MapKeyStats* ks = nullptr, bool trigger_passes = false, const uint32_t** perm_only = nullptr) {
  uint32_t ne = hc->n_map_emit;
  if (!ne) return;
  uint32_t* perm_a = b.val_a;
  uint32_t* perm_b = b.val_b;
  int cur = 0;
  bool by_rank = false;
  bool last_is_chunk0 = false;
  auto pass = [&](int mode, uint32_t chunk, int bits, int begin_bit = 0) {
    last_is_chunk0 = mode == MK_CHUNK && chunk == 0;
    uint32_t* pin = cur ? perm_b : perm_a;
    uint64_t* kin = cur ? b.key_b : b.key_a;
    const bool fused = sort_is_fused(ne) && bits > begin_bit;
    if (fused)
      hipLaunchKernelGGL(k_map_keys_hist, dim3(sort_tiles(ne)), dim3(BLOCK), 0, st, b, (const uint32_t*)pin, kin, ne, mode, chunk, (const uint32_t*)nullptr, begin_bit,
                         sort_first_table(b.sort_ws), sort_tiles(ne));
    else
      AM355_LAUNCH_INDEPENDENT(k_map_keys, grid_for(ne), dim3(BLOCK), st, b, (const uint32_t*)pin, kin, ne, mode, chunk, (const uint32_t*)nullptr);
    int res = cur ? radix_sort_pairs(b.key_b, perm_b, b.key_a, perm_a, ne, begin_bit, bits, b.sort_ws, st, fused)
                  : radix_sort_pairs(b.key_a, perm_a, b.key_b, perm_b, ne, begin_bit, bits, b.sort_ws, st, fused);
    cur ^= res;
  };
  if (ne <= BLOCK && !perm_only) {
    if (ride_with_list_order) *ride_with_list_order = ne;
    else hipLaunchKernelGGL(k_map_small_finish, dim3(1), dim3(BLOCK), 0, st, b, ne, ir);
    return;
  }
  if (ne <= MAP_SORT_SMALL) {
    hipLaunchKernelGGL(k_map_sort_small, grid_for(ne), dim3(BLOCK), 0, st, b, ne, (const uint32_t*)nullptr, perm_b);
    cur = 1;
  } else {
    AM355_LAUNCH_INDEPENDENT(k_iota, grid_for(ne), dim3(BLOCK), st, perm_a, ne);
    static const bool trigger_env = getenv("AM355_MAP_TRIGGER_PASSES") != nullptr;
    by_rank = !(trigger_passes || trigger_env);
    if (!by_rank) pass(MK_TRIGGER, 0, b.bits_ctr + b.bits_actor);
    static const bool all_passes = getenv("AM355_MAP_ALL_PASSES") != nullptr;
    const bool have_stats = ks && !all_passes;
    if (!have_stats || (ks->or_len & ks->or_inv_len)) pass(MK_LEN, 0, bits_for(hc->max_key_len));
    uint32_t chunks = (hc->max_key_len + 7) / 8;
    for (uint32_t c = chunks; c-- > 0;) {
      uint32_t used = hc->max_key_len - 8 * c < 8 ? hc->max_key_len - 8 * c : 8;
      auto varies = [&](uint32_t j) {
        const uint32_t pos = 8 * c + j;
        if (!have_stats || pos >= 16) return true;
        const uint32_t sh = 24 - 8 * (pos & 3);
        return (((ks->or_b[pos >> 2] & ks->or_inv_b[pos >> 2]) >> sh) & 0xffu) != 0;
      };
      for (int j = (int)used - 1; j >= 0;) {
        if (!varies((uint32_t)j)) { j--; continue; }
        int j_hi = j;
        while (j - 1 >= 0 && varies((uint32_t)(j - 1))) j--;
        pass(MK_CHUNK, c, 64 - 8 * j, 64 - 8 * (j_hi + 1));
        j--;
      }
    }
    if (hc->n_objects) pass(MK_OBJECT, 0, bits_for(hc->n_objects));
  }
  if (by_rank) {
    AM355_LAUNCH_INDEPENDENT(k_map_group_rank, grid_for(ne), dim3(BLOCK), st, b, (const uint32_t*)(cur ? perm_b : perm_a), cur ? perm_a : perm_b, ne,
                             last_is_chunk0 ? (const uint64_t*)(cur ? b.key_b : b.key_a) : (const uint64_t*)nullptr);
    cur ^= 1;
  }
  if (perm_only) { *perm_only = cur ? perm_b : perm_a; return; }
  AM355_LAUNCH_INDEPENDENT(k_map_finish, grid_for(ne), dim3(BLOCK), st, b, (const uint32_t*)(cur ? perm_b : perm_a), ne, ir);
}

void merge_resolve(MergeBufs& b, hipStream_t st) {
  if (b.n_ops) hipLaunchKernelGGL(k_resolve, grid_for(std::max(b.n_ops - b.first_row, 1u)), dim3(BLOCK), 0, st, b);
}

void merge_run(MergeBufs& b, PatchIR& ir, Counts* hc, hipStream_t st, hipEvent_t ev_counts, hipEvent_t ev_runs, bool resolved) {
  const uint32_t N = b.n_ops;
  const bool trace = getenv("AM355_TRACE") != nullptr;
  auto t_begin = std::chrono::steady_clock::now();
  auto lap = [&](const char* what) {
    if (trace) fprintf(stderr, "  merge_run: %-24s +%8.3f ms\n", what, std::chrono::duration<double, std::milli>(std::chrono::steady_clock::now() - t_begin).count());
  };
  Counts* hc_runs = hc + 1;
  if (!N) {
    (void)hipMemsetAsync(ir.obj, 0, sizeof(am355_ir_object), st);
    (void)hipMemsetAsync(ir.edit, 0, sizeof(am355_ir_edit), st);
    (void)hipMemcpyAsync(hc, b.counts, sizeof(Counts), hipMemcpyDeviceToHost, st);
    (void)hipStreamSynchronize(st);
    return;
  }
  uint32_t* is_head = b.scan_a;
  uint32_t* head_ex = b.scan_b;
  uint32_t* heads = b.run_heads;
  uint32_t* row_run = b.row_run;
  if (!resolved) hipLaunchKernelGGL(k_resolve, grid_for(std::max(N - b.first_row, 1u)), dim3(BLOCK), 0, st, b);
  hipLaunchKernelGGL(k_emit, grid_for(N), dim3(BLOCK), 0, st, b);
  hipLaunchKernelGGL(k_compact_rows, grid_for(N), dim3(BLOCK), 0, st, b, ir);
  if (!b.sig) (void)hipMemcpyAsync(hc, b.counts, sizeof(Counts), hipMemcpyDeviceToHost, st);
  if (ev_counts) (void)hipEventRecord(ev_counts, st);
  hipLaunchKernelGGL(k_child_push, grid_for(N), dim3(BLOCK), 0, st, b);
  hipLaunchKernelGGL(k_head_children, dim3(1), dim3(HEAD_CHILD_THREADS), 0, st, b);
  hipLaunchKernelGGL(k_child_order<false>, grid_for(N), dim3(BLOCK), 0, st, b, is_head);
  hipLaunchKernelGGL(k_run_heads, grid_for(N), dim3(BLOCK), 0, st, b, (const uint32_t*)is_head, head_ex, heads, row_run);
  if (!b.sig) {
    (void)hipMemcpyAsync(hc_runs, b.counts, sizeof(Counts), hipMemcpyDeviceToHost, st);
    (void)hipEventRecord(ev_runs, st);
  }
  AM355_LAUNCH_INDEPENDENT(k_euler_init_runs, grid_for(N), dim3(BLOCK), st, b, (const uint32_t*)heads, (const uint32_t*)row_run, b.euler_a);
  hipLaunchKernelGGL(k_euler_rank_lds, dim3(1), dim3(EULER_LDS_THREADS), 0, st, b.counts, b.euler_a);

  lap("first half enqueued");
  MapKeyStats key_stats;
  if (b.sig) read_phase_counts(b, &b.sig->counts_seq, b.sig->counts, hc, st, &key_stats);
  else (void)hipEventSynchronize(ev_counts);
  lap("counts read");
  if (hc->flags) { (void)hipStreamSynchronize(st); return; }
  const uint32_t ni = hc->n_list_ins, nu = hc->n_list_upd, n_obj = hc->n_objects + 1;
  uint32_t map_small = 0;
  order_map_emissions(b, ir, hc, st, ni && n_obj <= OBJ_LDS_MAX ? &map_small : nullptr, b.sig ? &key_stats : nullptr);

  if (ni) {
    if (b.sig) read_phase_counts(b, &b.sig->runs_seq, b.sig->runs, hc_runs, st);
    else (void)hipEventSynchronize(ev_runs);
    lap("runs read");
    uint32_t H = hc_runs->n_runs;
    ListKeyBits kb{bits_for(N), (int)b.bits_ctr, (int)b.bits_actor};
    if (hc_runs->pad) {
      int total_bits = 1 + kb.b_row + kb.b_ctr + kb.b_actor;
      (void)hipMemsetAsync(&b.counts->pad, 0, 3 * sizeof(uint32_t), st);
      (void)hipMemsetAsync(b.cs_runs.group_sum, 0, (size_t)((uint8_t*)b.counts + b.counts_bytes - (uint8_t*)b.cs_runs.group_sum), st);
      (void)hipMemsetAsync(b.first_child, 0xff, sizeof(uint32_t) * (2 * (size_t)N + 1), st);
      AM355_LAUNCH_INDEPENDENT(k_list_keys, grid_for(ni), dim3(BLOCK), st, b, b.key_a, b.val_a, ni, kb);
      int res = radix_sort_pairs(b.key_a, b.val_a, b.key_b, b.val_b, ni, 0, total_bits, b.sort_ws, st);
      AM355_LAUNCH_INDEPENDENT(k_list_link, grid_for(ni), dim3(BLOCK), st, b, (const uint64_t*)(res ? b.key_b : b.key_a), (const uint32_t*)(res ? b.val_b : b.val_a), ni, kb);
      hipLaunchKernelGGL(k_child_order<true>, grid_for(ni), dim3(BLOCK), 0, st, b, is_head);
      hipLaunchKernelGGL(k_run_heads, grid_for(ni), dim3(BLOCK), 0, st, b, (const uint32_t*)is_head, head_ex, heads, row_run);
      (void)hipMemcpyAsync(hc_runs, b.counts, sizeof(Counts), hipMemcpyDeviceToHost, st);
      AM355_LAUNCH_INDEPENDENT(k_euler_init_runs, grid_for(ni), dim3(BLOCK), st, b, (const uint32_t*)heads, (const uint32_t*)row_run, b.euler_a);
      hipLaunchKernelGGL(k_euler_rank_lds, dim3(1), dim3(EULER_LDS_THREADS), 0, st, b.counts, b.euler_a);
      (void)hipStreamSynchronize(st);
      H = hc_runs->n_runs;
    }
    const unsigned long long* el = b.euler_a;
    if (2 * (uint64_t)H + 1 > EULER_LDS_ENTRIES) {
      int rounds = bits_for(2ull * H + 1);
      unsigned long long *e0 = b.euler_a, *e1 = b.euler_b;
      for (int r = 0; r < rounds; r++) {
        AM355_LAUNCH_INDEPENDENT(k_euler_jump, grid_for(2 * H + 1), dim3(BLOCK), st, H, (const unsigned long long*)e0, e1);
        unsigned long long* t = e0;
        e0 = e1;
        e1 = t;
      }
      el = e0;
    }
    if (n_obj <= OBJ_LDS_MAX) {
      hipLaunchKernelGGL(k_list_order_objs, dim3(grid_for(ni).x + (map_small ? 1u : 0u)), dim3(BLOCK), 0, st, b, ir, n_obj, ni, (const uint32_t*)is_head,
                         (const uint32_t*)head_ex, (const uint32_t*)heads, (const uint32_t*)row_run, el, map_small);
    } else {
      AM355_LAUNCH_INDEPENDENT(k_obj_n, grid_for(n_obj + 1), dim3(BLOCK), st, b, ir, n_obj, (const uint32_t*)row_run, el);
      exclusive_scan_u32(b.obj_n, b.obj_first_pos, n_obj + 1, nullptr, b.scan_ws, st);
      AM355_LAUNCH_INDEPENDENT(k_list_order, grid_for(ni), dim3(BLOCK), st, b, ni, (const uint32_t*)is_head, (const uint32_t*)head_ex, (const uint32_t*)heads, el);
    }
    uint32_t* vis_ex = b.scan_a;
    uint32_t* cnt_ex = b.scan_b;
    unsigned long long* vl_min = nullptr;
    if (hc->n_quirk) {
      vl_min = el == b.euler_a ? b.euler_b : b.euler_a;
      (void)hipMemsetAsync(vl_min, 0xff, sizeof(unsigned long long) * (size_t)N, st);
      AM355_LAUNCH_INDEPENDENT(k_quirk_rows, grid_for(N), dim3(BLOCK), st, b, vl_min);
    }
    static const bool unfused = getenv("AM355_LIST_UNFUSED") != nullptr;
    uint32_t* vis_base = unfused ? nullptr : b.list_vis;
    if (unfused) {
      hipLaunchKernelGGL(k_list_counts, grid_for(ni), dim3(BLOCK), 0, st, b, ni, (const unsigned long long*)vl_min);
      hipLaunchKernelGGL(k_list_scan, grid_for(ni), dim3(BLOCK), 0, st, b, ni, vis_ex, cnt_ex);
    } else {
      hipLaunchKernelGGL(k_list_counts_pub, grid_for(ni), dim3(BLOCK), 0, st, b, ni, (const unsigned long long*)vl_min);
    }
    const uint64_t* uk = b.key_a;
    const uint32_t* uv = b.val_a;
    if (nu) {
      AM355_LAUNCH_INDEPENDENT(k_upd_keys, grid_for(nu), dim3(BLOCK), st, b, b.key_a, b.val_a, nu);
      int r2 = radix_sort_pairs(b.key_a, b.val_a, b.key_b, b.val_b, nu, 0, kb.b_row + kb.b_ctr + kb.b_actor, b.sort_ws, st);
      uk = r2 ? b.key_b : b.key_a;
      uv = r2 ? b.val_b : b.val_a;
    }
    if (unfused)
      AM355_LAUNCH_INDEPENDENT(k_list_edits, grid_for(ni), dim3(BLOCK), st, b, ni, (const uint32_t*)vis_ex, (const uint32_t*)cnt_ex, uk, uv, nu, ir,
                               (const unsigned long long*)vl_min);
    else
      hipLaunchKernelGGL(k_list_scan_edits, grid_for(ni), dim3(BLOCK), 0, st, b, ni, uk, uv, nu, ir, (const unsigned long long*)vl_min, vis_base);
    hipLaunchKernelGGL(k_edit_runs, grid_for(N), dim3(BLOCK), 0, st, b, ir);
    hipLaunchKernelGGL(k_edit_pack, grid_for(N), dim3(BLOCK), 0, st, b, ir, (const uint32_t*)vis_base);
  } else {
// ... 365 lines not shown
```

### automerge_classic_amd/csrc/am355_replay.hip

```cpp
#include "am355_ctx.h"


struct HashSet {
  std::vector<const uint8_t*> slot;
  size_t mask = 0;
  void init(size_t n) {
    size_t cap = 16;
    while (cap < n * 2 + 2) cap <<= 1;
    slot.assign(cap, nullptr);
    mask = cap - 1;
  }
  static uint64_t key(const uint8_t* h) { uint64_t v; memcpy(&v, h, 8); return v * 0x9e3779b97f4a7c15ull; }
  const uint8_t** find(const uint8_t* h) {
    size_t i = (size_t)(key(h) >> 20) & mask;
    while (slot[i]) {
      if (slot[i] != (const uint8_t*)1 && memcmp(slot[i], h, 32) == 0) return &slot[i];
      i = (i + 1) & mask;
    }
    return nullptr;
  }
  bool has(const uint8_t* h) { return find(h) != nullptr; }
  void add(const uint8_t* h) {
    size_t i = (size_t)(key(h) >> 20) & mask;
    while (slot[i] && slot[i] != (const uint8_t*)1) i = (i + 1) & mask;
// ... 317 lines not shown
  if (getenv("AM355_DEBUG_TIMING")) {
    auto T4 = std::chrono::steady_clock::now();
    auto ms = [](auto a, auto b) { return std::chrono::duration<double, std::milli>(b - a).count(); };
    fprintf(stderr, "schedule: actors %.3f rank %.3f causal %.3f plan %.3f ms\n", ms(T0, T1), ms(T1, T2), ms(T2, T3), ms(T3, T4));
  }
  return AM355_OK;
}





static uint32_t rank_device_actors(am355_ctx* c, std::vector<uint32_t>& slot_rank) {
  const uint32_t* distinct = c->hp_distinct;
  const unsigned long long* slots = (const unsigned long long*)(distinct + 2 + distinct_capacity());
  const uint8_t* raw = c->raw.data();
  uint32_t n_slots = c->slot_mask + 1;
  struct Ent { uint32_t slot, off, len; };
  static thread_local std::vector<Ent> ents;
  ents.clear();
  uint32_t nd = distinct[0];
  for (uint32_t k = 0; k < nd; k++) {
    uint32_t i = distinct[1 + k];
    ents.push_back(Ent{i, (uint32_t)((slots[k] >> 16) - 1), (uint32_t)(slots[k] & 0xffff)});
  }
  std::sort(ents.begin(), ents.end(), [&](const Ent& x, const Ent& y) {
    uint32_t m = std::min(x.len, y.len);
    int r = m ? memcmp(raw + x.off, raw + y.off, m) : 0;
    return r ? r < 0 : x.len < y.len;
  });
  uint32_t na = (uint32_t)ents.size();
  slot_rank.assign(n_slots, 0);
  c->actors.resize(na);
  for (uint32_t r = 0; r < na; r++) {
    slot_rank[ents[r].slot] = r;
    c->actors[r].assign((const char*)raw + ents[r].off, ents[r].len);
  }
  return na;
}

static int plan_fast(am355_ctx* c, std::vector<uint32_t>& slot_rank, const uint32_t* order = nullptr, uint32_t n_applied = 0, const uint32_t* pass = nullptr) {
  const ChangeBrief* br = c->hp_briefs;
  uint32_t n = order ? n_applied : c->n_changes;
  uint32_t na = rank_device_actors(c, slot_rank);
  static thread_local std::vector<uint64_t> clock;
  static thread_local std::vector<uint32_t> span_cnt;
  clock.assign(na, 0);
  span_cnt.assign(na + 1, 0);
  c->clock_actor.clear();
  c->plans.clear();
  c->plans.reserve(n);
  c->applied_change.resize(n);
  c->applied_op_base.resize(n);
  c->pass_first_row.clear();
  uint64_t ops = 0, preds = 0, entries = 0, max_op = 0;
  for (uint32_t t = 0; t < n; t++) {
    const uint32_t ci = order ? order[t] : t;
    const ChangeBrief& m = br[ci];
    if (order && t > 0 && pass[ci] != pass[order[t - 1]]) c->pass_first_row.push_back((uint32_t)ops);
    c->applied_change[t] = ci;
    c->applied_op_base[t] = (uint32_t)ops;
    uint32_t author = slot_rank[m.author_slot];
    if (m.seq != clock[author] + 1) { c->flags |= AM355_F_BAD_SEQ; return fail(c, AM355_E_INVALID, "sequence number %llu out of order", (unsigned long long)m.seq); }
    if (clock[author] == 0) c->clock_actor.push_back(author);
    clock[author] = m.seq;
    if (m.n_ops) {
      c->plans.push_back(ChangePlan{ci, (uint32_t)ops, (uint32_t)preds, (uint32_t)entries, author, m.n_entries});
      span_cnt[author]++;
      max_op = std::max<uint64_t>(max_op, (uint64_t)m.start_op + m.n_ops - 1);
    }
    ops += m.n_ops;
    preds += m.n_preds;
    entries += m.n_entries;
    if (ops >= 0x7ffffff0ull || preds >= 0xfffffff0ull) { c->flags |= AM355_F_OVERFLOW; return fail(c, AM355_E_UNSUPPORTED, "more than 2^31 ops in one batch"); }
  }
  c->n_applied = n;
  c->n_pending = 0;
  c->pending_change.clear();
  c->n_ops = ops;
  c->n_preds = preds;
  c->max_op = max_op;
  c->clock_seq.clear();
  for (uint32_t a : c->clock_actor) c->clock_seq.push_back(clock[a]);
  c->actor_tab_off.assign(na + 1, 0);
  for (uint32_t a = 0; a < na; a++) c->actor_tab_off[a + 1] = c->actor_tab_off[a] + span_cnt[a];
  c->spans.resize(c->actor_tab_off[na]);
  for (uint32_t a = 0; a < na; a++) span_cnt[a] = c->actor_tab_off[a];
  for (const ChangePlan& pl : c->plans) c->spans[span_cnt[pl.author]++] = ActorSpan{br[pl.change].start_op, br[pl.change].n_ops, pl.op_base};
  for (uint32_t a = 0; a < na; a++) {
    ActorSpan* v = c->spans.data() + c->actor_tab_off[a];
    size_t k_n = c->actor_tab_off[a + 1] - c->actor_tab_off[a];
    bool sorted = true;
    for (size_t k = 1; k < k_n; k++) sorted = sorted && v[k - 1].start_op <= v[k].start_op;
    if (!sorted) std::sort(v, v + k_n, [](const ActorSpan& x, const ActorSpan& y) { return x.start_op < y.start_op; });
    for (size_t k = 1; k < k_n; k++)
      if ((uint64_t)v[k - 1].start_op + v[k - 1].n_ops > v[k].start_op) {
        c->flags |= AM355_F_DUP_OPID;
        return fail(c, AM355_E_INVALID, "overlapping op id ranges for one actor (duplicate operation ID)");
      }
  }
  return AM355_OK;
}

static int carve_cols(am355_ctx* c, uint32_t N, uint32_t P, bool estimate = false) {
  canary_scope("replay buffers (carve_cols: op rows, preds)");
  static const bool no_cap = getenv("AM355_NO_ROW_CAP") != nullptr;
  if (c->in_apply && !no_cap && !estimate) {
    N = (uint32_t)std::min<uint64_t>((uint64_t)N + N / 4 + 65536, 0x7ffffff0u);
    P = (uint32_t)std::min<uint64_t>((uint64_t)P + P / 4 + 65536, 0xfffffff0u);
  }
  c->cols_cap_ops = N;
  c->cols_cap_preds = P;
  c->resident_valid = false;
  size_t Nc = (size_t)N + 1;
  size_t bytes = 13 * carve_size(Nc, 4) + carve_size(Nc, 1);
  if (!c->d_cols.ensure(bytes) || !c->d_pred.ensure(2 * carve_size((size_t)P + 1, 4))) return fail(c, AM355_E_NOMEM, "device allocation failed (op rows)");
  canary_forget(c->d_cols.p, c->d_cols.cap); canary_forget(c->d_pred.p, c->d_pred.cap);
  uint8_t* p = c->d_cols.as<uint8_t>();
  OpCols& o = c->cols;
  o.obj_actor = carve<uint32_t>(p, Nc); o.obj_ctr = carve<uint32_t>(p, Nc); o.key_actor = carve<uint32_t>(p, Nc); o.key_ctr = carve<uint32_t>(p, Nc);
  o.key_off = carve<uint32_t>(p, Nc); o.key_len = carve<uint32_t>(p, Nc); o.action = carve<uint32_t>(p, Nc); o.val_tl = carve<uint32_t>(p, Nc);
  o.val_off = carve<uint32_t>(p, Nc); o.pred_first = carve<uint32_t>(p, Nc); o.pred_num = carve<uint32_t>(p, Nc); o.id_ctr = carve<uint32_t>(p, Nc);
  o.id_actor = carve<uint32_t>(p, Nc); o.insert = carve<uint8_t>(p, Nc);
  uint8_t* q = c->d_pred.as<uint8_t>();
  o.pred_actor = carve<uint32_t>(q, (size_t)P + 1);
  o.pred_ctr = carve<uint32_t>(q, (size_t)P + 1);
  return AM355_OK;
}

int setup_buffers(am355_ctx* c, uint32_t NA) {
  uint32_t N = (uint32_t)c->n_ops, P = (uint32_t)c->n_preds;
  int bits_ctr = bits_for64(c->max_op), bits_actor = bits_for64(NA ? NA - 1 : 0), bits_row = bits_for64(N);
  if (1 + bits_row + bits_ctr + bits_actor > 64) { c->flags |= AM355_F_OVERFLOW; return fail(c, AM355_E_UNSUPPORTED, "sort key wider than 64 bits"); }
  size_t Nc = (size_t)N + 1;
  c->resident_valid = false;
  c->order_alt_ptr = nullptr;
  c->map_alt_ptr = nullptr;
  c->pos_valid = false;
  c->ir_stale = false;
  canary_scope("replay buffers (setup_buffers: op rows, preds, merge scratch, sort scratch, patch IR)");
  if (!(c->spec_launched && N <= c->spec_cap_ops && P <= c->spec_cap_preds)) {
    c->spec_launched = false;
    int rcc = carve_cols(c, N, P);
    if (rcc) return rcc;
  }
  canary_scope("replay buffers (setup_buffers: merge scratch, sort scratch, patch IR)");
  static const bool no_cap = getenv("AM355_NO_ROW_CAP") != nullptr;
  const bool by_cap = c->in_apply && c->cols_cap_ops >= N && !no_cap;
  if (by_cap) Nc = std::min<size_t>(c->cols_cap_ops, (size_t)N + N / 4 + 65536) + 1;
  {
    size_t cw = carry_words((uint32_t)(Nc - 1));
    size_t bytes = 10 * carve_size(Nc, 4) + 3 * carve_size(Nc, 8) + carve_size(Nc, 1) + carve_size(2 * Nc + 2, 4) + 4 * carve_size(2 * Nc + 2, 4) +
                   3 * carve_size(Nc + 1, 4) + scan_workspace_bytes((uint32_t)(2 * Nc + 2)) + 256 +
                   6 * carve_size(Nc + 3, 4) + 6 * carve_size(cw, 4) + carve_size(2048, 4);
    size_t sort_bytes = 2 * carve_size(Nc, 8) + 2 * carve_size(Nc, 4) + sort_workspace_bytes((uint32_t)Nc) + 256;
    size_t ir_bytes = carve_size(Nc + 1, sizeof(am355_ir_object)) + carve_size(Nc, sizeof(am355_ir_map)) + carve_size(Nc + 1, sizeof(am355_ir_edit)) +
                      4 * carve_size(Nc, 4);
    if (!c->d_merge.ensure(bytes) || !c->d_sort.ensure(sort_bytes) || !c->d_ir.ensure(ir_bytes) || !c->d_counts.ensure(merge_counts_bytes(N)))
      return fail(c, AM355_E_NOMEM, "device allocation failed (merge)");
    canary_forget(c->d_merge.p, c->d_merge.cap); canary_forget(c->d_sort.p, c->d_sort.cap); canary_forget(c->d_ir.p, c->d_ir.cap);
    uint8_t* p = c->d_merge.as<uint8_t>();
    MergeBufs& b = c->mb;
    b.arena = c->d_arena.as<uint8_t>();
    b.ops = c->cols;
    b.n_ops = N; b.n_preds = P; b.n_actors = NA;
    b.shard_rank = c->shard_rank; b.shard_world = c->shard_world;
    b.sig = c->h_sig.as<HostSignals>(); b.sig_seq = c->sig_seq;
    b.actor_tab_off = c->p_tab_off;
    b.spans = c->p_spans;
    b.bits_ctr = (uint32_t)bits_ctr; b.bits_actor = (uint32_t)bits_actor;
    static const bool fill_kernel = getenv("AM355_FILL_KERNEL") != nullptr;
    b.first_row = 0; b.seed_list_inc = 0; b.row_stride = (by_cap || fill_kernel) ? (uint32_t)Nc : 0u;
    b.zero_base = p;
    b.succ_cnt = carve<uint32_t>(p, Nc); b.inc_cnt = carve<uint32_t>(p, Nc); b.val_cnt = carve<uint32_t>(p, Nc);
    b.inc_sum = carve<unsigned long long>(p, Nc); b.last_inc = carve<unsigned long long>(p, Nc);
    b.zero_bytes = (size_t)(p - (uint8_t*)b.zero_base) - (canary_on() ? 256 : 0);
    canary_allow(b.zero_base, b.zero_bytes);
// ... 88 lines not shown
  launch_decode_columns(c->d_arena.as<uint8_t>(), c->d_metas.as<ChangeMeta>(), (const ChangePlan*)d_tables, n_small, n_large, (uint32_t)np - n_small - n_large, d_amap,
                        d_rank, c->cols, &c->d_counts.as<Counts>()->flags, st, c->stream3, c->shard_rank, c->shard_world);
  HIPCHK(c, hipEventRecord(c->ev[3], st));
  HIPCHK(c, hipEventRecord(c->ev_join, c->stream3));
  HIPCHK(c, hipStreamWaitEvent(st, c->ev_join, 0));

  Counts* hc = c->h_counts.as<Counts>();
  merge_run(c->mb, c->ir, hc, st, (c->phase_events || !c->mb.sig) ? c->ev_counts.h : nullptr, c->ev_runs);
  HIPCHK(c, hipEventRecord(c->ev[5], st));
  if (hc->flags) return error_for_flags(c, hc->flags, "op set rejected");
  c->counts = *hc;
  c->counts.n_objects += 1;
  return AM355_OK;
}

struct GeneralOrder { const uint32_t* order; const uint32_t* pass; uint32_t n_applied; hipEvent_t ready; };
static int run_device_planned(am355_ctx* c, const PlanTotals& tot, uint32_t n_distinct, float* ms_host_plan, const GeneralOrder* go = nullptr) {
  hipStream_t st = c->stream;
  const bool trace = getenv("AM355_TRACE") != nullptr;
  auto t_begin = std::chrono::steady_clock::now();
  auto lap = [&](const char* what) {
    if (trace) fprintf(stderr, "  planned: %-26s +%8.3f ms\n", what, std::chrono::duration<double, std::milli>(std::chrono::steady_clock::now() - t_begin).count());
  };
  uint32_t n = c->n_changes;
  c->n_ops = tot.n_ops;
  c->n_preds = tot.n_preds;
  c->max_op = tot.max_op;
  auto al = [](size_t b) { return (b + 255) & ~(size_t)255; };
  size_t o_tab = al(sizeof(ActorSpan) * (size_t)n + 16), tables_bytes = o_tab + al(4 * ((size_t)n_distinct + 1) + 16);
  if (!c->d_tables.ensure(tables_bytes) || !c->h_stage.ensure(tables_bytes)) return fail(c, AM355_E_NOMEM, "device allocation failed");
  uint8_t* d_tables = c->d_tables.as<uint8_t>();
  c->p_spans = (ActorSpan*)d_tables;
  c->p_tab_off = (uint32_t*)(d_tables + o_tab);
  c->sig_seq++;
  int rcb = setup_buffers(c, n_distinct);
  if (rcb) return rcb;
  lap("buffers carved");
  const bool spec_done = c->spec_launched && decode_gate_open(tot, c->spec_cap_ops, c->spec_cap_preds, distinct_capacity()) &&
                         c->counts_zeroed_at == c->d_counts.p && c->mb.counts_bytes <= c->counts_zeroed;
  if (trace && c->spec_launched && !spec_done)
    fprintf(stderr, "  planned: speculative decode not usable: ops %u / cap %u, preds %u / cap %u, distinct %u, fast_a %x flags_a %x fallback %u, counts %p/%p %zu/%zu\n", tot.n_ops,
            c->spec_cap_ops, tot.n_preds, c->spec_cap_preds, tot.n_distinct, tot.fast_a, tot.flags_a, tot.fallback, c->counts_zeroed_at, c->d_counts.p, c->mb.counts_bytes, c->counts_zeroed);
  if (c->spec_launched && !spec_done) {
    c->spec_launched = false;
    HIPCHK(c, hipStreamSynchronize(c->stream3));
    HIPCHK(c, hipStreamSynchronize(st));
    int rc2 = setup_buffers(c, n_distinct);
    if (rc2) return rc2;
  }
  if (!spec_done && !(c->counts_zeroed_at == c->d_counts.p && c->mb.counts_bytes <= c->counts_zeroed)) HIPCHK(c, hipMemsetAsync(c->d_counts.p, 0, c->mb.counts_bytes, st));
  c->counts_zeroed_at = nullptr;
  c->hint_large = tot.n_large;
  if (spec_done) {
    c->hint_ops = std::max(c->hint_ops, tot.n_ops);
    c->hint_preds = std::max(c->hint_preds, tot.n_preds);
    const uint32_t host_large = c->spec_large_launched ? 0u : tot.n_large;
    if (tot.n_serial || host_large) {
      if (!c->spec_large_launched) {
        HIPCHK(c, hipEventRecord(c->ev_fork, st));
        HIPCHK(c, hipStreamWaitEvent(c->stream3, c->ev_fork, 0));
      }
      launch_decode_planned(c->d_arena.as<uint8_t>(), c->d_metas.as<ChangeMeta>(), c->d_plans.as<ChangePlan>(), c->d_plans.as<ChangePlan>() + std::max(n, 1u), n, 0,
                            host_large, tot.n_serial, c->d_amap_prov.as<uint32_t>(), c->d_slot_rank.as<uint32_t>(), c->cols, &c->d_counts.as<Counts>()->flags,
                            c->stream3, nullptr, c->shard_rank, c->shard_world);
    }
    lap("decode was launched behind the plan kernel");
  } else {
    c->hint_ops = tot.n_ops;
    c->hint_preds = tot.n_preds;
    if (tot.n_small && (tot.n_large || tot.n_serial)) {
      HIPCHK(c, hipEventRecord(c->ev_fork, st));
      HIPCHK(c, hipStreamWaitEvent(c->stream3, c->ev_fork, 0));
    }
    if (c->phase_events) HIPCHK(c, hipEventRecord(c->ev[2], st));
    launch_decode_planned(c->d_arena.as<uint8_t>(), c->d_metas.as<ChangeMeta>(), c->d_plans.as<ChangePlan>(), c->d_plans.as<ChangePlan>() + std::max(n, 1u), n,
                          tot.n_small, tot.n_large, tot.n_serial, c->d_amap_prov.as<uint32_t>(), c->d_slot_rank.as<uint32_t>(), c->cols,
                          &c->d_counts.as<Counts>()->flags, st, c->stream3, c->shard_rank, c->shard_world);
    lap("decode launched");
    if (c->phase_events) HIPCHK(c, hipEventRecord(c->ev[3], st));
  }
  c->spec_launched = false;
  const bool second_class = tot.n_small && (tot.n_large || tot.n_serial);
  hipStream_t fill_stream = second_class ? c->stream4 : c->stream3;
  if (!merge_prepare(c->mb, fill_stream)) return fail(c, AM355_E_DEVICE, "merge fills: more ranges than one launch takes");
  if (second_class) {
    HIPCHK(c, hipEventRecord(c->ev_join, c->stream3));
    HIPCHK(c, hipStreamWaitEvent(st, c->ev_join, 0));
  }
  lap("fills enqueued");
  if (go) HIPCHK(c, hipEventSynchronize(go->ready));
  auto t0 = std::chrono::steady_clock::now();
  std::vector<uint32_t> slot_rank;
  int rc = go ? plan_fast(c, slot_rank, go->order, go->n_applied, go->pass) : plan_fast(c, slot_rank);
  *ms_host_plan = std::chrono::duration<float, std::milli>(std::chrono::steady_clock::now() - t0).count();
  lap("plan_fast done");
  if (rc == AM355_OK && (c->n_ops != tot.n_ops || c->n_preds != tot.n_preds || c->max_op != tot.max_op || c->actors.size() != n_distinct))
    rc = fail(c, AM355_E_DEVICE, "internal: device and host plans disagree (%llu / %u ops)", (unsigned long long)c->n_ops, tot.n_ops);
  if (rc) { (void)hipStreamSynchronize(st); return rc; }
  {
    uint8_t* h = c->h_stage.as<uint8_t>();
    size_t b_spans = sizeof(ActorSpan) * c->spans.size(), b_tab = 4 * c->actor_tab_off.size();
    if (b_spans) memcpy(h, c->spans.data(), b_spans);
    memcpy(h + o_tab, c->actor_tab_off.data(), b_tab);
    HIPCHK(c, hipMemcpyAsync(d_tables, h, o_tab + b_tab, hipMemcpyHostToDevice, fill_stream));
    HIPCHK(c, hipEventRecord(c->ev_tables, fill_stream));
    HIPCHK(c, hipStreamWaitEvent(st, c->ev_tables, 0));
  }
  lap("tables enqueued");
  Counts* hc = c->h_counts.as<Counts>();
  merge_run(c->mb, c->ir, hc, st, (c->phase_events || !c->mb.sig) ? c->ev_counts.h : nullptr, c->ev_runs);
  HIPCHK(c, hipEventRecord(c->ev[5], st));
  if (hc->flags) return error_for_flags(c, hc->flags, "op set rejected");
  c->counts = *hc;
  c->counts.n_objects += 1;
  return AM355_OK;
}

static int replay_document_stages(am355_ctx* c) {
  auto t_begin = std::chrono::steady_clock::now();
  const bool trace = getenv("AM355_TRACE") != nullptr;
  auto lap = [&](const char* what) {
    if (trace) fprintf(stderr, "replay_document: %-28s +%8.3f ms\n", what, std::chrono::duration<double, std::milli>(std::chrono::steady_clock::now() - t_begin).count());
  };
  hipStream_t st = c->stream;
  uint32_t NA = (uint32_t)c->actors.size();
  if (!c->d_plans.ensure(sizeof(ChangePlan)) || !c->d_amap.ensure(4 * (size_t)std::max(NA, 1u)) || !c->d_words.ensure(4 * W_NUM) || !c->h_words.ensure(4 * W_NUM))
    return fail(c, AM355_E_NOMEM, "device allocation failed");
  HIPCHK(c, hipEventRecord(c->ev[0], st));
  c->doc_col_rows.clear();
  if (c->doc_serial) {
    HIPCHK(c, hipMemcpyAsync(c->d_metas.p, &c->doc_meta, sizeof(ChangeMeta), hipMemcpyHostToDevice, st));
    launch_doc_count(c->d_arena.as<uint8_t>(), c->d_metas.as<ChangeMeta>(), st);
    HIPCHK(c, hipMemcpyAsync(c->h_metas.p, c->d_metas.p, sizeof(ChangeMeta), hipMemcpyDeviceToHost, st));
    HIPCHK(c, hipEventRecord(c->ev[1], st));
    HIPCHK(c, hipStreamSynchronize(st));
    const ChangeMeta* hm = c->h_metas.as<ChangeMeta>();
    if (hm->flags) return error_for_flags(c, hm->flags, "malformed document columns");
    c->n_ops = hm->n_ops;
    c->n_preds = hm->n_preds;
    c->n_applied = c->n_changes;
    c->n_pending = 0;
    c->max_op = 0xffffffffu >> 8;
    if (c->n_ops >= 0x7ffffff0ull) { c->flags |= AM355_F_OVERFLOW; return fail(c, AM355_E_UNSUPPORTED, "more than 2^31 rows in one document"); }
    int rc = setup_buffers(c, NA);
    if (rc) return rc;
    ChangePlan pl{0, 0, 0, 0, NONE32, NA};
    HIPCHK(c, hipMemcpyAsync(c->d_plans.p, &pl, sizeof pl, hipMemcpyHostToDevice, st));
    HIPCHK(c, hipMemcpyAsync(c->d_amap.p, c->doc_actor_rank.data(), 4 * (size_t)NA, hipMemcpyHostToDevice, st));
    HIPCHK(c, hipMemsetAsync(c->d_counts.p, 0, c->mb.counts_bytes, st));
    HIPCHK(c, hipMemsetAsync(c->d_words.p, 0, 4 * W_NUM, st));
    HIPCHK(c, hipEventRecord(c->ev[2], st));
    launch_decode_document(c->d_arena.as<uint8_t>(), c->d_metas.as<ChangeMeta>(), c->d_plans.as<ChangePlan>(), c->d_amap.as<uint32_t>(), c->cols,
                           &c->d_counts.as<Counts>()->flags, st);
  } else {
    const BigColDesc& d = c->doc_cols;
    const ChangeMeta& m = c->doc_meta;
    if (!c->d_big.ensure(bigcol_work_bytes(d.tok_bytes)) || !c->d_ks.ensure(keystr_work_bytes(m.col_len[C_KEY_STR])) || !c->h_biginfo.ensure(sizeof(BigColInfo)))
      return fail(c, AM355_E_NOMEM, "device allocation failed (document index)");
    BigColWork w;
    canary_forget(c->d_big.p, c->d_big.cap);
    bigcol_carve(w, c->d_big.p, d.tok_bytes);
    canary_arm();
    uint32_t *ks_start, *ks_off, *ks_len;
    uint32_t* d_words = c->d_words.as<uint32_t>();
    HIPCHK(c, hipMemsetAsync(d_words, 0, 4 * W_NUM, st));
    HIPCHK(c, hipMemcpyAsync(c->d_amap.p, c->doc_actor_rank.data(), 4 * (size_t)NA, hipMemcpyHostToDevice, st));
    lap("actor ranks enqueued");
    HIPCHK(c, hipEventRecord(c->ev_b0, st));
    HIPCHK(c, hipStreamWaitEvent(c->stream2, c->ev_b0, 0));
    KeyStage ks;
    ks.max_jumps = c->key_unbounded ? 0u : 64u;
    canary_forget(c->d_ks.p, c->d_ks.cap);
    keystr_index_begin(c->d_arena.as<uint8_t>(), m.col_off[C_KEY_STR], m.col_len[C_KEY_STR], c->d_ks.p, ks, d_words + W_TOTAL_ENTRIES, d_words + W_FAST_B,
                       c->stream2);
    keystr_index_finish(ks, false, &ks_start, &ks_off, &ks_len, d_words + W_FLAGS_B, c->stream2);
    HIPCHK(c, hipEventRecord(c->ev_b1, c->stream2));
    lap("key stream enqueued");
    BigColInfo* hi = c->h_biginfo.as<BigColInfo>();
    bigcol_index_tokens(c->d_arena.as<uint8_t>(), d, w, st);
    HIPCHK(c, hipMemcpyAsync(hi, w.info, sizeof(BigColInfo), hipMemcpyDeviceToHost, st));
    lap("token ends enqueued");
    HIPCHK(c, hipStreamSynchronize(st));
    bigcol_index_records(c->d_arena.as<uint8_t>(), d, w, hi->n_tokens, st);
    HIPCHK(c, hipMemcpyAsync(hi, w.info, sizeof(BigColInfo), hipMemcpyDeviceToHost, st));
    HIPCHK(c, hipEventRecord(c->ev[1], st));
    lap("enqueued index");
    HIPCHK(c, hipStreamSynchronize(st));
    lap("token index done");
    if (hi->flags) { (void)hipStreamSynchronize(c->stream2); return error_for_flags(c, hi->flags, "malformed document columns"); }
    BigColInfo info = *hi;
    c->doc_col_rows.assign(info.rows, info.rows + BIG_NCOL);
    uint32_t N = info.rows[BC_ACTION], Pcap = info.rows[BC_SUCC_ACTOR];
    if (N >= 0x7ffffff0u) { (void)hipStreamSynchronize(c->stream2); c->flags |= AM355_F_OVERFLOW; return fail(c, AM355_E_UNSUPPORTED, "more than 2^31 rows in one document"); }
// ... 901 lines not shown
      HIPCHK(c, hipMemcpy(cnt.data(), b.obj_n, 4 * NO, hipMemcpyDeviceToHost));
    }
    for (size_t k = 1; k < NO; k++) {
      const am355_ir_object &x = kept_obj[k], &y = obj[k];
      if (x.id_ctr != y.id_ctr || x.id_actor != y.id_actor || x.type != y.type || x.make_row != y.make_row)
        return fail(c, AM355_E_DEVICE, "internal: object %zu kept from the in-place calls is %u@%u type %u row %u, computed from scratch %u@%u type %u row %u", k,
                    x.id_ctr, x.id_actor, x.type, x.make_row, y.id_ctr, y.id_actor, y.type, y.make_row);
    }
    for (size_t k = 0; k < NO; k++)
      if (kept_first[k] != first[k] || kept_n[k] != cnt[k])
        return fail(c, AM355_E_DEVICE, "internal: object %zu kept from the in-place calls has %u elements from position %u, computed from scratch %u from %u", k,
                    kept_n[k], kept_first[k], cnt[k], first[k]);
  }
  return AM355_OK;
}

int replay_impl(am355_ctx* c) {
  if (!c) return AM355_E_ARG;
  if (!c->staged) return fail(c, AM355_E_STATE, "am355_load_changes must be called first");
  (void)hipSetDevice(c->device);
  c->replayed = c->ir_fetched = false;
  c->ir_copy_enqueued = 0;
  c->dep_graph_ready = false;
  c->flags = 0;
  c->spec_launched = false;
  c->batch_list_only = false;
  c->h_tables_were_current = c->h_tables_current;
  c->h_tables_current = false;
  if (c->is_document) return replay_document(c);
  auto t_begin = std::chrono::steady_clock::now();
  if (c->in_apply && c->keep.want) {
    c->keep.want = false;
    const int rr = replay_resident(c);
    if (rr != RESIDENT_FALLBACK) {
      if (rr != AM355_OK) return rr;
      am355_stats& s = c->stats;
      s.n_changes = c->n_changes; s.n_applied = c->n_applied; s.n_pending = 0; s.n_actors = (uint32_t)c->actors.size(); s.n_objects = c->counts.n_objects;
      s.n_heads = (uint32_t)(c->heads.size() / 32); s.n_ops = c->n_ops; s.max_op = c->max_op; s.raw_bytes = c->raw.size();
      s.n_map_values = c->counts.n_map_emit; s.n_list_elems = c->counts.n_list_ins; s.n_edits = c->counts.n_edits;
      s.ir_bytes = (uint64_t)c->counts.n_objects * sizeof(am355_ir_object) + (uint64_t)c->counts.n_map_emit * sizeof(am355_ir_map) +
                   ((uint64_t)c->counts.n_erecs + 1) * sizeof(am355_ir_edit);
      s.ms_parse = s.ms_decode = s.ms_merge = s.ms_order = s.ms_hash_stream = s.ms_host_schedule = 0;
      s.fast_path = 1;
      s.ms_total = std::chrono::duration<float, std::milli>(std::chrono::steady_clock::now() - t_begin).count();
      c->used_fast_path = true;
      c->device_scheduled = false;
      c->replayed = true;
      c->seed_list_inc = c->counts.n_list_inc;
      resident_mark(c);
      c->resident_valid = true;
      return AM355_OK;
    }
  }
  c->keep.want = false;
  { int orc = flush_uploads(c); if (!orc) orc = upload_offsets(c); if (orc) return orc; }
  const bool trace = getenv("AM355_TRACE") != nullptr;
  auto lap = [&](const char* what) {
    if (trace) fprintf(stderr, "replay: %-28s +%8.3f ms\n", what, std::chrono::duration<double, std::milli>(std::chrono::steady_clock::now() - t_begin).count());
  };
  hipStream_t sa = c->stream, sb = c->stream2;
  uint32_t n = c->n_changes;
  size_t n1 = std::max<size_t>(n, 1);
  c->slot_mask = pow2_at_least(4 * (uint64_t)n + 64) - 1;
  c->hash_mask = pow2_at_least(2 * (uint64_t)n + 64) - 1;
  if (c->amap_cap < 16 * n1 + 1024) c->amap_cap = (uint32_t)(16 * n1 + 1024);
  if (!c->d_entries.ensure(4 * n1) || !c->d_amap_base.ensure(4 * (n1 + 1)) || !c->d_amap_prov.ensure(4 * (size_t)c->amap_cap) ||
      !c->d_slots.ensure(8 * (size_t)(c->slot_mask + 1)) || !c->d_first_idx.ensure(4 * (size_t)(c->slot_mask + 1)) || !c->d_hashes.ensure(32 * n1) ||
      !c->d_hash_tab.ensure(4 * (size_t)(c->hash_mask + 1)) || !c->d_min_idx.ensure(4 * n1) || !c->d_has_dep.ensure(n1) || !c->d_words.ensure(4 * W_NUM) ||
      !c->d_scan1.ensure(scan_workspace_bytes((uint32_t)n1)) || !c->h_slots.ensure(8 * (size_t)(c->slot_mask + 1)) || !c->h_hashes.ensure(32 * n1) ||
      !c->h_has_dep.ensure(n1) || !c->h_words.ensure(4 * W_NUM) || !c->d_plans.ensure(2 * sizeof(ChangePlan) * n1) ||
      !c->d_slot_rank.ensure(4 * (size_t)(c->slot_mask + 1)) || !c->d_plan_sums.ensure(plan_block_sums_bytes(n)) ||
      !c->d_dep_idx.ensure(4 * (c->raw.size() / 32 + 2)) || !c->d_self_idx.ensure(4 * n1) || !c->d_rank_ids.ensure(rank_ids_bytes()))
    return fail(c, AM355_E_NOMEM, "device allocation failed (stage 1)");
  c->have_host_metas = false;
  const size_t s1_distinct = 64, s1_briefs = s1_distinct + ((12 * (size_t)distinct_capacity() + 16 + 63) & ~(size_t)63);
  const size_t s1_bytes = s1_briefs + sizeof(ChangeBrief) * n1;
  if (!c->d_s1.ensure(s1_bytes) || !c->h_s1.ensure(s1_bytes)) return fail(c, AM355_E_NOMEM, "device allocation failed (stage 1)");
  uint32_t* d_wa = c->d_s1.as<uint32_t>();
  uint32_t* d_distinct = (uint32_t*)(c->d_s1.as<uint8_t>() + s1_distinct);
  ChangeBrief* d_briefs = (ChangeBrief*)(c->d_s1.as<uint8_t>() + s1_briefs);
  const uint32_t* h_wa = c->h_s1.as<uint32_t>();
  c->hp_distinct = (uint32_t*)(c->h_s1.as<uint8_t>() + s1_distinct);
  c->hp_briefs = (ChangeBrief*)(c->h_s1.as<uint8_t>() + s1_briefs);
  uint32_t* d_words = c->d_words.as<uint32_t>();
  uint32_t* h_words = c->h_words.as<uint32_t>();
  HostSignals* sig = c->h_sig.as<HostSignals>();
  PlanTotals tot{};
  static const bool hash_after_parse = []() { const char* e = getenv("AM355_HASH_START"); return !(e && !strcmp(e, "intern")); }();

  HIPCHK(c, hipEventRecord(c->ev[0], sa));
  const size_t cb = merge_counts_bytes((uint32_t)std::min<size_t>(c->raw.size(), 0x7ffffff0u));
  c->counts_zeroed_at = nullptr;
  const bool counts_too = c->d_counts.ensure(cb);
  const bool fat_changes = n && c->raw.size() / n > 4096 && !getenv("AM355_PARSE_LEAN");
  if (c->inline_fills) {
    ParseFills f{};
    auto add = [&](void* q, size_t bytes, uint32_t v) { f.p[f.n] = (uint32_t*)q; f.n_words[f.n] = (bytes + 3) / 4; f.value[f.n] = v; f.n++; };
    add(d_words, 4 * W_NUM, 0);
    add(d_wa, s1_distinct + 16, 0);
    add(c->d_slots.p, 8 * (size_t)(c->slot_mask + 1), 0);
    add(c->d_first_idx.p, 4 * (size_t)(c->slot_mask + 1), 0xffffffffu);
    if (counts_too) add(c->d_counts.p, cb, 0);
    launch_parse_changes(c->d_arena.as<uint8_t>(), c->d_offsets.as<uint64_t>(), n, c->d_metas.as<ChangeMeta>(), c->d_entries.as<uint32_t>(), f, sa, fat_changes);
    HIPCHK(c, hipEventRecord(c->ev_parse, sa));
  } else {
    launch_parse_changes(c->d_arena.as<uint8_t>(), c->d_offsets.as<uint64_t>(), n, c->d_metas.as<ChangeMeta>(), c->d_entries.as<uint32_t>(), ParseFills{}, sa, fat_changes);
    HIPCHK(c, hipEventRecord(c->ev_parse, sa));
    HIPCHK(c, hipMemsetAsync(d_words, 0, 4 * W_NUM, c->stream3));
    HIPCHK(c, hipMemsetAsync(d_wa, 0, s1_distinct + 16, c->stream3));
    HIPCHK(c, hipMemsetAsync(c->d_slots.p, 0, 8 * (size_t)(c->slot_mask + 1), c->stream3));
    HIPCHK(c, hipMemsetAsync(c->d_first_idx.p, 0xff, 4 * (size_t)(c->slot_mask + 1), c->stream3));
    if (counts_too) HIPCHK(c, hipMemsetAsync(c->d_counts.p, 0, cb, c->stream3));
    HIPCHK(c, hipEventRecord(c->ev_join, c->stream3));
    HIPCHK(c, hipStreamWaitEvent(sa, c->ev_join, 0));
  }
  if (counts_too) {
    c->counts_zeroed_at = c->d_counts.p;
    c->counts_zeroed = cb;
  }

  auto enqueue_stream_b = [&]() -> int {
    HIPCHK(c, hipStreamWaitEvent(sb, hash_after_parse ? c->ev_parse : c->ev[1], 0));
    if (!c->inline_fills) HIPCHK(c, hipStreamWaitEvent(sb, c->ev_join, 0));
    HIPCHK(c, hipEventRecord(c->ev_b0, sb));
    HIPCHK(c, hipMemsetAsync(c->d_hash_tab.p, 0, 4 * (size_t)(c->hash_mask + 1), sb));
    HIPCHK(c, hipMemsetAsync(c->d_has_dep.p, 0, n1, sb));
    launch_hash_changes(c->d_arena.as<uint8_t>(), c->d_offsets.as<uint64_t>(), n, c->d_hashes.as<uint8_t>(), c->d_min_idx.as<uint32_t>(),
                    c->d_hash_tab.as<uint32_t>(), c->hash_mask, d_words + W_FLAGS_B, sb);
    launch_deps_resolve(c->d_arena.as<uint8_t>(), c->d_metas.as<ChangeMeta>(), c->d_hashes.as<uint8_t>(), n, c->d_hash_tab.as<uint32_t>(), c->hash_mask,
                    c->d_min_idx.as<uint32_t>(), c->d_has_dep.as<uint8_t>(), d_words + W_FAST_B, c->d_dep_idx.as<uint32_t>(), c->d_self_idx.as<uint32_t>(), sb);
    HIPCHK(c, hipMemcpyAsync(c->h_hashes.p, c->d_hashes.p, 32 * (size_t)n, hipMemcpyDeviceToHost, sb));
    HIPCHK(c, hipMemcpyAsync(c->h_has_dep.p, c->d_has_dep.p, n, hipMemcpyDeviceToHost, sb));
    HIPCHK(c, hipMemcpyAsync(h_words + W_FLAGS_B, d_words + W_FLAGS_B, 8, hipMemcpyDeviceToHost, sb));
    HIPCHK(c, hipEventRecord(c->ev_b1, sb));
    return AM355_OK;
  };
  static const bool enqueue_early = []() { const char* e = getenv("AM355_HASH_ENQUEUE"); return e && !strcmp(e, "early"); }();
  static const bool enqueue_thread = AM355_STREAMS_ORDER_ACROSS_THREADS && []() { const char* e = getenv("AM355_HASH_ENQUEUE"); return !e || !strcmp(e, "thread"); }();
  std::atomic<int> lane_rc{AM355_OK};
  struct LaneJoin {
    AsyncLane* l = nullptr;
    ~LaneJoin() { if (l) l->wait(); }
  } lane_join;
  bool b_enqueued = false;
  if (hash_after_parse && enqueue_early) { int rb = enqueue_stream_b(); if (rb) return rb; b_enqueued = true; }
  else if (hash_after_parse && enqueue_thread && n >= 512) {
    if (!c->lane) c->lane.reset(new AsyncLane);
    c->lane->post([&]() { (void)hipSetDevice(c->device); lane_rc.store(enqueue_stream_b()); });
    lane_join.l = c->lane.get();
    b_enqueued = true;
  }
  exclusive_scan_u32(c->d_entries.as<uint32_t>(), c->d_amap_base.as<uint32_t>(), n, d_wa + W_TOTAL_ENTRIES, c->d_scan1.p, sa);
  static const bool spec_env = []() { const char* e = getenv("AM355_SPEC_DECODE"); return !(e && *e == '0'); }();
  const bool spec_possible = spec_env && n && c->inline_fills && counts_too && hash_after_parse && !getenv("AM355_HOST_PLAN") && !(c->in_apply && c->graph_mode != 0) &&
                             c->d_plan_totals.ensure(sizeof(PlanTotals));
  for (int attempt = 0;; attempt++) {
    if (attempt) {
      HIPCHK(c, hipMemsetAsync(c->d_slots.p, 0, 8 * (size_t)(c->slot_mask + 1), sa));
      HIPCHK(c, hipMemsetAsync(c->d_first_idx.p, 0xff, 4 * (size_t)(c->slot_mask + 1), sa));
      HIPCHK(c, hipMemsetAsync(d_distinct, 0, 4, sa));
    }
    launch_actor_intern(c->d_arena.as<uint8_t>(), c->d_metas.as<ChangeMeta>(), n, c->d_amap_base.as<uint32_t>(), c->d_amap_prov.as<uint32_t>(), c->amap_cap,
                        c->d_slots.as<unsigned long long>(), c->slot_mask, c->d_first_idx.as<uint32_t>(), d_wa + W_FLAGS_A, d_wa + W_FAST_A,
                        d_distinct, c->d_rank_ids.p, d_briefs, c->d_slot_rank.as<uint32_t>(), c->d_plan_sums.as<unsigned long long>(), d_wa + 8, sa, c->hp_briefs);
    c->sig_seq++;
    launch_plan(d_briefs, n, d_distinct, c->d_slot_rank.as<uint32_t>(), c->slot_mask, c->d_plan_sums.as<unsigned long long>(), c->d_plans.as<ChangePlan>(),
                c->d_plans.as<ChangePlan>() + n1, d_wa, d_wa + 8, sig, c->sig_seq, sa, spec_possible ? c->d_plan_totals.as<PlanTotals>() : nullptr,
                c->h_s1.as<uint32_t>());
    const bool want_large_spec = spec_possible && attempt == 0 && c->hint_large != 0;
    if (want_large_spec) HIPCHK(c, hipEventRecord(c->ev_plan, sa));
    if (spec_possible && attempt == 0) {
      const uint64_t est = c->raw.size() / 2 + 1024;
      c->spec_cap_ops = (uint32_t)std::min<uint64_t>(std::max<uint64_t>(c->hint_ops, est), 0x7ffffff0u);
      c->spec_cap_preds = (uint32_t)std::min<uint64_t>(std::max<uint64_t>(c->hint_preds, est), 0x7ffffff0u);
      if (trace) fprintf(stderr, "replay: speculative decode: cap %u ops / %u preds (counter block %zu of %zu bytes)\n", c->spec_cap_ops, c->spec_cap_preds, merge_counts_bytes(c->spec_cap_ops), cb);
      if (merge_counts_bytes(c->spec_cap_ops) <= cb && carve_cols(c, c->spec_cap_ops, c->spec_cap_preds, true) == AM355_OK) {
        canary_arm();
        if (c->phase_events) { HIPCHK(c, hipEventRecord(c->ev[1], sa)); HIPCHK(c, hipEventRecord(c->ev[2], sa)); }
        if (want_large_spec) HIPCHK(c, hipStreamWaitEvent(c->stream3, c->ev_plan, 0));
        launch_decode_speculative(c->d_arena.as<uint8_t>(), c->d_metas.as<ChangeMeta>(), c->d_plans.as<ChangePlan>(), n, c->d_plan_totals.as<PlanTotals>(), c->spec_cap_ops,
                                  c->spec_cap_preds, distinct_capacity(), c->d_amap_prov.as<uint32_t>(), c->d_slot_rank.as<uint32_t>(), c->cols,
                                  &c->d_counts.as<Counts>()->flags, sa, c->stream3, want_large_spec, c->shard_rank, c->shard_world);
        c->spec_large_launched = want_large_spec;
        if (c->phase_events) HIPCHK(c, hipEventRecord(c->ev[3], sa));
        c->spec_launched = true;
      }
    }
    if ((c->phase_events && !c->spec_launched) || !hash_after_parse) HIPCHK(c, hipEventRecord(c->ev[1], sa));
    if (attempt == 0 && !b_enqueued) { int rb = enqueue_stream_b(); if (rb) return rb; b_enqueued = true; }
    lap("stage 1 enqueued");
    if (!wait_host_signal(&sig->plan_seq, c->sig_seq, sa)) {
      (void)hipStreamSynchronize(sb);
      (void)hipStreamSynchronize(c->stream3);
      return fail(c, AM355_E_DEVICE, "the device did not report the plan of this replay (%s)", hipGetErrorString(hipGetLastError()));
    }
    memcpy(&tot, (const void*)&sig->plan, sizeof tot);
    lap("stage 1 totals read");
    if (!(tot.fast_a & FF_CAPACITY) || attempt) break;
    c->spec_launched = false;
    c->amap_cap = tot.total_entries + 1024;
    if (!c->d_amap_prov.ensure(4 * (size_t)c->amap_cap)) return fail(c, AM355_E_NOMEM, "device allocation failed (actor tables)");
    HIPCHK(c, hipMemsetAsync(d_wa + W_FAST_A, 0, 4, sa));
    HIPCHK(c, hipMemsetAsync(d_wa + 8, 0, 32, sa));
  }

  auto t_h0 = std::chrono::steady_clock::now();
  float ms_host = 0;
  int rc = AM355_OK;
  if (tot.flags_a) { (void)hipStreamSynchronize(sa); (void)hipStreamSynchronize(sb); return error_for_flags(c, tot.flags_a, "malformed change"); }
  c->has_unknown_cols = tot.reserved[0] != 0;
  bool fast = tot.fast_a == 0;
  const bool lineage_schedule = c->in_apply && c->graph_mode != 0;
  if (lineage_schedule) fast = false;
  if (tot.n_distinct > distinct_capacity()) fast = false;
  const bool planned = !tot.fallback && !getenv("AM355_HOST_PLAN");
  std::vector<uint32_t> slot_rank;
  int opt_rc = AM355_OK;
  uint32_t opt_flags = 0;
  std::string opt_err;
  if (fast && planned) {
    float ms_plan = 0;
    opt_rc = run_device_planned(c, tot, tot.n_distinct, &ms_plan);
    ms_host += ms_plan;
    lap("run_device (device plan) done");
    opt_flags = c->flags;
    opt_err = c->err;
  } else {
    if (tot.fallback) {
      const ChangeBrief* br = c->hp_briefs;
      uint32_t dev_flags = 0;
      c->has_unknown_cols = false;
      for (uint32_t i = 0; i < n; i++) {
        dev_flags |= br[i].flags_fits & 0x1fffffffu;
        if (br[i].flags_fits & 0x20000000u) c->has_unknown_cols = true;
      }
      if (dev_flags) { (void)hipStreamSynchronize(sa); (void)hipStreamSynchronize(sb); return error_for_flags(c, dev_flags, "malformed change"); }
    }
    if (fast) {
      opt_rc = plan_fast(c, slot_rank);
      ms_host += std::chrono::duration<float, std::milli>(std::chrono::steady_clock::now() - t_h0).count();
      lap("plan_fast done");
      if (opt_rc == AM355_OK) opt_rc = run_device(c, &slot_rank);
      lap("run_device done");
      opt_flags = c->flags;
      opt_err = c->err;
    }
  }
  if (lane_join.l) { lane_join.l->wait(); lane_join.l = nullptr; if (lane_rc.load()) return lane_rc.load(); }
  HIPCHK(c, hipEventSynchronize(c->ev_b1));
  lap("hash stream joined");
  if (h_words[W_FLAGS_B]) return error_for_flags(c, h_words[W_FLAGS_B], "checksum does not match data");
// ... 143 lines not shown
```

### automerge_classic_amd/csrc/am355_scan.h

```cpp
#pragma once
#include "am355_device.h"

namespace am355 {

__device__ __forceinline__ uint32_t wave_incl_scan_u32(uint32_t x, uint32_t lane) {
  for (int d = 1; d < WAVE; d <<= 1) {
    uint32_t y = __shfl_up(x, (unsigned)d);
    if (lane >= (uint32_t)d) x += y;
  }
  return x;
}

__device__ __forceinline__ uint32_t wave_sum_u32(uint32_t x) {
  for (int d = WAVE / 2; d >= 1; d >>= 1) x += __shfl_xor(x, d);
  return x;
}

__device__ __forceinline__ uint32_t block_sum_u32(uint32_t v, uint32_t* s) {
  uint32_t w = threadIdx.x / WAVE;
  uint32_t t = wave_sum_u32(v);
  if ((threadIdx.x & (WAVE - 1)) == 0) s[w] = t;
  __syncthreads();
  uint32_t total = 0;
  for (int k = 0; k < BLOCK / WAVE; k++) total += s[k];
  __syncthreads();
  return total;
}

__device__ __forceinline__ uint32_t block_exclusive_scan_u32(uint32_t v, uint32_t* s, uint32_t* total) {
  uint32_t lane = threadIdx.x & (WAVE - 1), w = threadIdx.x / WAVE;
  uint32_t incl = wave_incl_scan_u32(v, lane);
  if (lane == WAVE - 1) s[w] = incl;
  __syncthreads();
  uint32_t before = 0, all = 0;
  for (uint32_t k = 0; k < BLOCK / WAVE; k++) {
    uint32_t x = s[k];
    before += k < w ? x : 0;
    all += x;
  }
  __syncthreads();
  *total = all;
  return before + incl - v;
}

constexpr uint32_t CARRY_GROUP_SHIFT = 6;
constexpr uint32_t CARRY_GROUP_STRIDE = 64;
struct CarryScan {
  uint32_t* wg_sum;
  uint32_t* group_sum;
};
__host__ __device__ __forceinline__ size_t carry_words(uint32_t n_elems) {
  size_t wgs = ((size_t)n_elems + BLOCK - 1) / BLOCK + 1;
  return wgs + (wgs >> CARRY_GROUP_SHIFT) + 2;
}
__device__ __forceinline__ uint32_t carry_publish(const CarryScan& c, uint32_t v, uint32_t* s) {
  uint32_t total = block_sum_u32(v, s);
  if (threadIdx.x == 0) {
    c.wg_sum[blockIdx.x] = total;
    if (total) atomicAdd(&c.group_sum[(size_t)(blockIdx.x >> CARRY_GROUP_SHIFT) * CARRY_GROUP_STRIDE], total);
  }
  return total;
}
__device__ __forceinline__ uint32_t carry_prefix(const CarryScan& c, uint32_t v, uint32_t* s) {
  uint32_t g = blockIdx.x >> CARRY_GROUP_SHIFT, first = g << CARRY_GROUP_SHIFT;
  uint32_t part = 0;
  for (uint32_t k = threadIdx.x; k < g; k += BLOCK) part += c.group_sum[(size_t)k * CARRY_GROUP_STRIDE];
  if (first + threadIdx.x < blockIdx.x) part += c.wg_sum[first + threadIdx.x];
  uint32_t before = block_sum_u32(part, s);
  uint32_t total;
  return before + block_exclusive_scan_u32(v, s, &total);
}

}
```

### automerge_classic_amd/engine.py

```python
import ctypes
import os

import numpy as np

_HERE = os.path.dirname(os.path.abspath(__file__))
DEFAULT_LIB = os.path.join(_HERE, "csrc", "libam355.so")

AM355_OK = 0
AM355_E_DEVICE, AM355_E_ARG, AM355_E_INVALID, AM355_E_UNSUPPORTED, AM355_E_STATE, AM355_E_NOMEM = -1, -2, -3, -4, -5, -6

FLAG_NAMES = {
    1 << 0: "BAD_MAGIC", 1 << 1: "BAD_CHECKSUM", 1 << 2: "BAD_CHUNK", 1 << 3: "BAD_COLUMNS", 1 << 4: "BAD_LEB", 1 << 5: "BAD_RLE",
    1 << 6: "BAD_ROW", 1 << 7: "UNKNOWN_OBJECT", 1 << 8: "BAD_ELEM", 1 << 9: "BAD_PRED", 1 << 10: "DUP_OPID", 1 << 11: "BAD_COUNTER",
    1 << 12: "UNSUPPORTED", 1 << 13: "OVERFLOW", 1 << 16: "BAD_SEQ", 1 << 17: "UNKNOWN_ACTOR", 1 << 18: "BAD_DEFLATE",
}


class Stats(ctypes.Structure):
    _fields_ = [
        ("n_changes", ctypes.c_uint32), ("n_applied", ctypes.c_uint32), ("n_pending", ctypes.c_uint32),
        ("n_actors", ctypes.c_uint32), ("n_objects", ctypes.c_uint32), ("n_heads", ctypes.c_uint32),
        ("n_ops", ctypes.c_uint64), ("max_op", ctypes.c_uint64), ("raw_bytes", ctypes.c_uint64),
        ("n_map_values", ctypes.c_uint64), ("n_list_elems", ctypes.c_uint64), ("n_edits", ctypes.c_uint64),
        ("ir_bytes", ctypes.c_uint64),
        ("ms_total", ctypes.c_float), ("ms_parse", ctypes.c_float), ("ms_host_schedule", ctypes.c_float),
        ("ms_decode", ctypes.c_float), ("ms_merge", ctypes.c_float), ("ms_order", ctypes.c_float), ("ms_hash_stream", ctypes.c_float),
        ("fast_path", ctypes.c_uint32),
    ]

    def as_dict(self):
        return {k: getattr(self, k) for k, _ in self._fields_}


class EngineError(RuntimeError):
    def __init__(self, code, message, flags=0):
        names = [n for b, n in FLAG_NAMES.items() if flags & b]
        super().__init__(f"am355 error {code}: {message}" + (f" [{'|'.join(names)}]" if names else ""))
        self.code = code
        self.flags = flags
        self.flag_names = names


class InvalidChanges(EngineError):
    """The reference would throw on this input (the JS host re-runs it on the JS path to raise the exact error)."""


class UnsupportedChanges(EngineError):
    """Legal input outside the GPU-served subset (documented in DESIGN.md); the JS host uses the JS path."""


def _bind(path):
    if not os.path.exists(path):
        raise RuntimeError(f"HIP engine library not found: {path}. Build it with `python -c 'import __graft_entry__ as g; g.build()'` "
                           "(hipcc --offload-arch=gfx950). There is no CPU fallback.")
    L = ctypes.CDLL(path)
    vp, u32, u64p = ctypes.c_void_p, ctypes.c_uint32, ctypes.c_void_p
    L.am355_create.restype = vp
    L.am355_create.argtypes = [ctypes.c_int]
    L.am355_destroy.argtypes = [vp]
    L.am355_last_error.restype = ctypes.c_char_p
    L.am355_last_error.argtypes = [vp]
    L.am355_flags.restype = u32
    L.am355_flags.argtypes = [vp]
    L.am355_load_changes.argtypes = [vp, vp, u64p, u32]
    L.am355_load_document.argtypes = [vp, vp, ctypes.c_size_t]
    if hasattr(L, "am355_backend_load"):
        L.am355_backend_load.argtypes = [vp, vp, ctypes.c_size_t]
        L.am355_backend_load.restype = ctypes.c_int
    L.am355_replay.argtypes = [vp]
    L.am355_patch_json.argtypes = [vp, ctypes.POINTER(ctypes.c_char_p), ctypes.POINTER(ctypes.c_size_t)]
    L.am355_get_stats.argtypes = [vp, ctypes.POINTER(Stats)]
    L.am355_get_hashes.argtypes = [vp, vp]
    L.am355_test_sort.argtypes = [vp, vp, vp, u32, ctypes.c_int]
    L.am355_test_scan.argtypes = [vp, vp, vp, u32, vp]
    sz, ci = ctypes.c_size_t, ctypes.c_int
    for f, args in (("am355_test_scan_at", [vp, vp, u32, u32, vp, u32, u32, u32, vp]), ("am355_test_scan2", [vp, vp, vp, u32, u32, vp, vp, u32, u32, u32, vp, vp]),
                    ("am355_test_scan_terminators", [vp, vp, sz, u32, u32, vp, u32, u32, vp]), ("am355_test_max", [vp, vp, u32, vp]),
                    ("am355_test_sort_bits", [vp, vp, vp, u32, ci, ci, vp, ctypes.POINTER(ci)]), ("am355_test_chain_mark", [vp, vp, vp, u32, u32]),
                    ("am355_test_remap", [vp, vp, u32, u32, vp, u32, vp, u32, ctypes.POINTER(u32)]), ("am355_test_fill", [vp, vp, u32, u32, vp, u32, ctypes.POINTER(u32)]),
                    ("am355_test_copy", [vp, vp, sz, vp, sz, ci, vp, u32, ctypes.POINTER(u32)]), ("am355_test_signal_words", [vp, vp, u32, vp, u32, u32, vp, u32, vp]),
                    ("am355_test_carried_scan", [vp, vp, u32, vp, vp, vp])):
        if not hasattr(L, f):
            continue
        getattr(L, f).argtypes = args
        getattr(L, f).restype = ci
    L.am355_get_rows.argtypes = [vp] * 15
    L.am355_save.argtypes = [vp, u32, ctypes.POINTER(ctypes.c_void_p), ctypes.POINTER(ctypes.c_size_t)]
    L.am355_get_applied.argtypes = [vp, vp, ctypes.POINTER(u32)]
    L.am355_fetch_ir.argtypes = [vp, vp]
    L.am355_set_shard.argtypes = [vp, u32, u32]
    L.am355_fragment_size.argtypes = [vp, ctypes.POINTER(ctypes.c_size_t)]
    L.am355_export_fragment.argtypes = [vp, vp, ctypes.c_size_t, ctypes.c_int, ctypes.POINTER(ctypes.c_size_t)]
    L.am355_import_fragments.argtypes = [vp, vp, vp, u32]
    L.am355_shard_unique_id.argtypes = [vp]
    L.am355_shard_init.argtypes = [vp, vp, u32, u32]
    L.am355_sharded_replay.argtypes = [vp, ctypes.c_int]
    L.am355_shard_fragment_bytes.argtypes = [vp, vp, u32]
    L.am355_shard_finalize.argtypes = [vp]
    for f in ("am355_shard_unique_id", "am355_shard_init", "am355_sharded_replay", "am355_shard_fragment_bytes", "am355_shard_finalize"):
        getattr(L, f).restype = ctypes.c_int
    if hasattr(L, "am355_resident_counters"):
        L.am355_resident_counters.argtypes = [vp, vp]
        L.am355_resident_counters.restype = ctypes.c_int
    if hasattr(L, "am355_resident_maps_only_calls"):
        L.am355_resident_maps_only_calls.argtypes = [vp, ctypes.POINTER(ctypes.c_uint64)]
        L.am355_resident_maps_only_calls.restype = ctypes.c_int
    if hasattr(L, "am355_set_resident_new_actors"):
        L.am355_set_resident_new_actors.argtypes = [vp, ctypes.c_int]
        L.am355_set_resident_new_actors.restype = ctypes.c_int
        L.am355_resident_new_actor_calls.argtypes = [vp, vp]
        L.am355_resident_new_actor_calls.restype = ctypes.c_int
    if hasattr(L, "am355_set_resident_new_objects"):
        L.am355_set_resident_new_objects.argtypes = [vp, ctypes.c_int]
        L.am355_set_resident_new_objects.restype = ctypes.c_int
        L.am355_resident_new_object_calls.argtypes = [vp, vp]
        L.am355_resident_new_object_calls.restype = ctypes.c_int
    if hasattr(L, "am355_set_resident_map_merge"):
        L.am355_set_resident_map_merge.argtypes = [vp, ctypes.c_int]
        L.am355_set_resident_map_merge.restype = ctypes.c_int
        L.am355_resident_map_merge_calls.argtypes = [vp, vp]
        L.am355_resident_map_merge_calls.restype = ctypes.c_int
    L.am355_get_raw.argtypes = [vp, ctypes.POINTER(ctypes.c_void_p), ctypes.POINTER(ctypes.c_void_p), ctypes.POINTER(u32)]
    L.am355_doc_changes.argtypes = [vp, u32, ctypes.POINTER(ctypes.c_void_p), ctypes.POINTER(ctypes.c_void_p), ctypes.POINTER(u32), ctypes.POINTER(ctypes.c_void_p)]
    L.am355_apply_changes.argtypes = [vp, vp, u64p, u32]
    L.am355_apply_patch_json.argtypes = [vp, ctypes.POINTER(ctypes.c_char_p), ctypes.POINTER(ctypes.c_size_t)]
    L.am355_fetch_apply_ir.argtypes = [vp, vp]
    L.am355_reset.argtypes = [vp]
    L.am355_get_dep_graph.argtypes = [vp, ctypes.POINTER(ctypes.c_void_p), ctypes.POINTER(ctypes.c_void_p), ctypes.POINTER(u32)]
    L.am355_sync_bloom_build.argtypes = [vp, vp, u32, vp, ctypes.c_size_t]
    L.am355_sync_bloom_probe.argtypes = [vp, vp, u32, u32, u32, u32, vp, ctypes.c_size_t, vp]
    L.am355_get_pending.argtypes = [vp, vp, ctypes.POINTER(u32)]
    L.am355_forget_call_history.argtypes = [vp, ctypes.c_int]
    L.am355_hash_graph_known.argtypes = [vp, ctypes.c_int, ctypes.POINTER(ctypes.c_int)]
    L.am355_set_phase_events.argtypes = [vp, ctypes.c_int]
    for f in ("am355_load_changes", "am355_load_document", "am355_replay", "am355_patch_json", "am355_get_stats", "am355_get_hashes", "am355_test_sort",
              "am355_test_scan", "am355_get_rows", "am355_save", "am355_get_applied", "am355_fetch_ir", "am355_get_raw", "am355_set_shard", "am355_fragment_size", "am355_export_fragment",
              "am355_import_fragments", "am355_doc_changes", "am355_apply_changes", "am355_apply_patch_json", "am355_fetch_apply_ir", "am355_reset", "am355_get_pending", "am355_forget_call_history", "am355_hash_graph_known", "am355_set_phase_events", "am355_get_dep_graph", "am355_sync_bloom_build", "am355_sync_bloom_probe"):
        getattr(L, f).restype = ctypes.c_int
    return L


_libs = {}


def load_library(path=DEFAULT_LIB):
    if path not in _libs:
        _libs[path] = _bind(path)
    return _libs[path]


class Engine:

    def __init__(self, device=0, lib_path=DEFAULT_LIB):
        self._L = load_library(lib_path)
        self.device = device
        self.lib_path = lib_path
        self._h = self._L.am355_create(device)
        if not self._h:
            raise RuntimeError("am355_create failed: no usable MI355X / HIP device (the engine has no CPU fallback)")
        self._n_changes = 0

    def set_phase_events(self, on):
        self._check(self._L.am355_set_phase_events(self._h, 1 if on else 0))

# ... 222 lines not shown
        out = np.zeros_like(a)
        total = np.zeros(1, dtype=np.uint32)
        self._check(self._L.am355_test_scan(self._h, a.ctypes.data, out.ctypes.data, a.size, total.ctypes.data))
        return out, int(total[0])

    @staticmethod
    def _img(a, dtype=np.uint32):
        return None if a is None else np.ascontiguousarray(a, dtype=dtype).copy()

    @staticmethod
    def _ptr(a):
        return None if a is None else a.ctypes.data

    def prim_scan(self, in_buf, in_off, n, out_buf=None, out_off=0, total=None):
        a, o = self._img(in_buf), self._img(out_buf)
        t = None if total is None else np.array([total], dtype=np.uint32)
        self._check(self._L.am355_test_scan_at(self._h, a.ctypes.data, a.size, in_off, self._ptr(o), 0 if o is None else o.size, in_off if o is None else out_off, n, self._ptr(t)))
        return a, o, None if t is None else int(t[0])

    def prim_scan2(self, in_a, in_b, in_off, n, out_a=None, out_b=None, out_off=0, total_a=None, total_b=None):
        a, b, oa, ob = self._img(in_a), self._img(in_b), self._img(out_a), self._img(out_b)
        ta = None if total_a is None else np.array([total_a], dtype=np.uint32)
        tb = None if total_b is None else np.array([total_b], dtype=np.uint32)
        self._check(self._L.am355_test_scan2(self._h, a.ctypes.data, b.ctypes.data, a.size, in_off, self._ptr(oa), self._ptr(ob), 0 if oa is None else oa.size,
                                             in_off if oa is None else out_off, n, self._ptr(ta), self._ptr(tb)))
        return a, b, oa, ob, None if ta is None else int(ta[0]), None if tb is None else int(tb[0])

    def prim_scan_terminators(self, bytes_buf, byte_off, L, out_buf, out_off, total=None):
        b, o = self._img(bytes_buf, np.uint8), self._img(out_buf)
        t = None if total is None else np.array([total], dtype=np.uint32)
        self._check(self._L.am355_test_scan_terminators(self._h, b.ctypes.data, b.size, byte_off, L, o.ctypes.data, o.size, out_off, self._ptr(t)))
        return o, None if t is None else int(t[0])

    def prim_max(self, values, before):
        v = self._img(values)
        t = np.array([before], dtype=np.uint32)
        self._check(self._L.am355_test_max(self._h, v.ctypes.data, v.size, t.ctypes.data))
        return int(t[0])

    def prim_sort(self, keys, vals, begin_bit, end_bit, first_table=None):
        k, v, tab = self._img(keys, np.uint64), self._img(vals), self._img(first_table)
        res = ctypes.c_int(-1)
        self._check(self._L.am355_test_sort_bits(self._h, k.ctypes.data, v.ctypes.data, k.size, begin_bit, end_bit, self._ptr(tab), ctypes.byref(res)))
        return k, v, res.value

    def prim_chain_mark(self, nxt, mark, n):
        nx, m = self._img(nxt), self._img(mark)
        self._check(self._L.am355_test_chain_mark(self._h, nx.ctypes.data, m.ctypes.data, m.size, n))
        return m

    def prim_remap(self, buf, base_off, ranges, table):
        b, tab = self._img(buf), self._img(table)
        r = np.array([[f, c, s, g & 0xFFFFFFFF, k] for f, c, s, g, k in ranges], dtype=np.uint32).reshape(-1, 5)
        added = ctypes.c_uint32(0)
        self._check(self._L.am355_test_remap(self._h, b.ctypes.data, b.size, base_off, r.ctypes.data, len(ranges), tab.ctypes.data, tab.size, ctypes.byref(added)))
        return b, added.value

    def prim_fill(self, buf, base_off, ranges):
        b = self._img(buf)
        r = np.array(ranges, dtype=np.uint32).reshape(-1, 3)
        added = ctypes.c_uint32(0)
        self._check(self._L.am355_test_fill(self._h, b.ctypes.data, b.size, base_off, r.ctypes.data, len(ranges), ctypes.byref(added)))
        return b, added.value

    def prim_copy(self, dst, src, ranges, src_pinned):
        d, s = self._img(dst, np.uint8), self._img(src, np.uint8)
        r = np.array(ranges, dtype=np.uint32).reshape(-1, 3)
        added = ctypes.c_uint32(0)
        self._check(self._L.am355_test_copy(self._h, d.ctypes.data, d.size, s.ctypes.data, s.size, 1 if src_pinned else 0, r.ctypes.data, len(ranges), ctypes.byref(added)))
        return d, added.value

    def prim_signal_words(self, a, b, seq, host_words, seq_word):
        wa, wb, h = self._img(a), self._img(b), self._img(host_words)
        s = np.array([seq_word], dtype=np.uint32)
        self._check(self._L.am355_test_signal_words(self._h, wa.ctypes.data, wa.size, wb.ctypes.data, wb.size, seq, h.ctypes.data, h.size, s.ctypes.data))
        return h, int(s[0])

    def prim_carried_scan(self, values):
        v = self._img(values)
        out, out_wg, tot = np.empty_like(v), np.empty_like(v), np.empty((v.size + 255) // 256, dtype=np.uint32)
        self._check(self._L.am355_test_carried_scan(self._h, v.ctypes.data, v.size, out.ctypes.data, out_wg.ctypes.data, tot.ctypes.data))
        return out, out_wg, tot

    def rows(self):
        n = int(self.stats().n_ops)
        names = ["obj_actor", "obj_ctr", "key_actor", "key_ctr", "key_off", "key_len", "action", "val_tl", "val_off", "pred_num",
                 "id_ctr", "id_actor", "insert", "succ_cnt"]
        arrs = {k: np.zeros(n, dtype=np.uint8 if k == "insert" else np.uint32) for k in names}
        self._check(self._L.am355_get_rows(self._h, *[arrs[k].ctypes.data for k in names]))
        return arrs


def replay_patch_json(log, device=0, lib_path=DEFAULT_LIB):
    eng = Engine(device, lib_path)
    try:
        eng.load_changes(log)
        eng.replay()
        return eng.patch_json()
    finally:
        eng.close()
```

### include/am355.h

```cpp
#ifndef AM355_H
#define AM355_H
#include <stddef.h>
#include <stdint.h>

#ifdef __cplusplus
extern "C" {
#endif

typedef struct am355_ctx am355_ctx;

enum {
  AM355_OK = 0,
  AM355_E_DEVICE = -1,
  AM355_E_ARG = -2,
  AM355_E_INVALID = -3,
  AM355_E_UNSUPPORTED = -4,
  AM355_E_STATE = -5,
  AM355_E_NOMEM = -6
};

enum {
  AM355_F_BAD_MAGIC = 1u << 0, AM355_F_BAD_CHECKSUM = 1u << 1, AM355_F_BAD_CHUNK = 1u << 2, AM355_F_BAD_COLUMNS = 1u << 3,
  AM355_F_BAD_LEB = 1u << 4, AM355_F_BAD_RLE = 1u << 5, AM355_F_BAD_ROW = 1u << 6, AM355_F_UNKNOWN_OBJECT = 1u << 7,
  AM355_F_BAD_ELEM = 1u << 8, AM355_F_BAD_PRED = 1u << 9, AM355_F_DUP_OPID = 1u << 10, AM355_F_BAD_COUNTER = 1u << 11,
// ... 73 lines not shown
  uint32_t val_tl;
  uint32_t val_off;
  uint32_t pad;
} am355_ir_edit;

typedef struct {
  uint32_t n_objects, n_map, n_edits, n_values;
  const am355_ir_object *objects;
  const am355_ir_map *map;
  const am355_ir_edit *edits;
  uint64_t max_op;
  uint32_t n_actors;
  const uint32_t *actor_off;
  const uint8_t *actor_bytes;
  uint32_t n_clock;
  const uint32_t *clock_actor;
  const uint64_t *clock_seq;
  uint32_t n_heads;
  const uint8_t *heads;
  uint32_t pending;
  const uint8_t *arena;
  uint64_t arena_len;
} am355_patch_ir;
int am355_fetch_ir(am355_ctx *ctx, am355_patch_ir *out);

int am355_apply_changes(am355_ctx *ctx, const uint8_t *arena, const uint64_t *offsets, uint32_t n_changes);
int am355_reset(am355_ctx *ctx);
int am355_forget_call_history(am355_ctx *ctx, int from_document);
int am355_hash_graph_known(am355_ctx *ctx, int set, int *known);

int am355_get_pending(const am355_ctx *ctx, uint32_t *out, uint32_t *n_pending);
int am355_apply_patch_json(am355_ctx *ctx, const char **json, size_t *len);
int am355_fetch_apply_ir(am355_ctx *ctx, am355_patch_ir *out);

int am355_get_dep_graph(am355_ctx *ctx, const uint32_t **dep_first, const uint32_t **dep_index, uint32_t *n_changes);
int am355_sync_bloom_build(am355_ctx *ctx, const uint32_t *idx, uint32_t n, uint8_t *bits, size_t capacity);
int am355_sync_bloom_probe(am355_ctx *ctx, const uint32_t *idx, uint32_t n, uint32_t num_entries, uint32_t bits_per_entry, uint32_t num_probes,
                           const uint8_t *bits, size_t n_bytes, uint8_t *contains);

int am355_set_shard(am355_ctx *ctx, uint32_t rank, uint32_t world);
int am355_fragment_size(am355_ctx *ctx, size_t *bytes);
int am355_export_fragment(am355_ctx *ctx, void *dst, size_t capacity, int dst_is_device, size_t *len);
int am355_import_fragments(am355_ctx *ctx, const uint8_t *frags, const uint64_t *offsets, uint32_t world);

#define AM355_SHARD_ID_BYTES 128
int am355_shard_unique_id(uint8_t id[AM355_SHARD_ID_BYTES]);
int am355_shard_init(am355_ctx *ctx, const uint8_t id[AM355_SHARD_ID_BYTES], uint32_t rank, uint32_t world);
int am355_sharded_replay(am355_ctx *ctx, int stitch_on_all_ranks);
int am355_shard_fragment_bytes(am355_ctx *ctx, uint64_t *bytes, uint32_t capacity);
int am355_shard_finalize(am355_ctx *ctx);

int am355_resident_counters(const am355_ctx *ctx, uint64_t out[3]);
int am355_resident_maps_only_calls(const am355_ctx *ctx, uint64_t *out);
int am355_set_resident_new_actors(am355_ctx *ctx, int on);
int am355_resident_new_actor_calls(const am355_ctx *ctx, uint64_t out[2]);
int am355_set_resident_map_merge(am355_ctx *ctx, int on);
int am355_resident_map_merge_calls(const am355_ctx *ctx, uint64_t out[2]);
int am355_set_resident_new_objects(am355_ctx *ctx, int on);
int am355_resident_new_object_calls(const am355_ctx *ctx, uint64_t out[2]);

int am355_arena_epoch(const am355_ctx *ctx, uint64_t *epoch);
int am355_get_hashes_range(const am355_ctx *ctx, uint32_t first, uint32_t count, uint8_t *out);
int am355_applied_in_input_order(const am355_ctx *ctx, int *yes);

int am355_test_sort(am355_ctx *ctx, uint64_t *keys, uint32_t *vals, uint32_t n, int key_bits);
int am355_test_scan(am355_ctx *ctx, const uint32_t *in, uint32_t *out, uint32_t n, uint32_t *total);
int am355_test_scan_at(am355_ctx *ctx, uint32_t *in_buf, uint32_t in_words, uint32_t in_off, uint32_t *out_buf, uint32_t out_words, uint32_t out_off,
                       uint32_t n, uint32_t *total);
int am355_test_scan2(am355_ctx *ctx, uint32_t *in_a, uint32_t *in_b, uint32_t in_words, uint32_t in_off, uint32_t *out_a, uint32_t *out_b, uint32_t out_words,
                     uint32_t out_off, uint32_t n, uint32_t *total_a, uint32_t *total_b);
int am355_test_scan_terminators(am355_ctx *ctx, const uint8_t *bytes_buf, size_t bytes_len, uint32_t byte_off, uint32_t L, uint32_t *out_buf, uint32_t out_words,
                                uint32_t out_off, uint32_t *total);
int am355_test_max(am355_ctx *ctx, const uint32_t *v, uint32_t n, uint32_t *inout);
int am355_test_sort_bits(am355_ctx *ctx, uint64_t *keys, uint32_t *vals, uint32_t n, int begin_bit, int end_bit, const uint32_t *first_table, int *result_buffer);
int am355_test_chain_mark(am355_ctx *ctx, const uint32_t *next, uint32_t *mark, uint32_t mark_words, uint32_t n);
int am355_test_remap(am355_ctx *ctx, uint32_t *buf, uint32_t words, uint32_t base_off, const uint32_t *ranges, uint32_t n_ranges, const uint32_t *table, uint32_t n_old,
                     uint32_t *n_added);
int am355_test_fill(am355_ctx *ctx, uint32_t *buf, uint32_t words, uint32_t base_off, const uint32_t *ranges, uint32_t n_ranges, uint32_t *n_added);
int am355_test_copy(am355_ctx *ctx, uint8_t *dst, size_t dst_bytes, const uint8_t *src, size_t src_bytes, int src_pinned, const uint32_t *ranges, uint32_t n_ranges,
                    uint32_t *n_added);
int am355_test_signal_words(am355_ctx *ctx, const uint32_t *a, uint32_t n_a, const uint32_t *b, uint32_t n_b, uint32_t seq, uint32_t *host_words, uint32_t host_words_n,
                            uint32_t *seq_word);
int am355_test_carried_scan(am355_ctx *ctx, const uint32_t *v, uint32_t n, uint32_t *out, uint32_t *out_wg, uint32_t *wg_total);
int am355_get_rows(am355_ctx *ctx, uint32_t *obj_actor, uint32_t *obj_ctr, uint32_t *key_actor, uint32_t *key_ctr, uint32_t *key_off,
                   uint32_t *key_len, uint32_t *action, uint32_t *val_tl, uint32_t *val_off, uint32_t *pred_num, uint32_t *id_ctr,
                   uint32_t *id_actor, uint8_t *insert, uint32_t *succ_cnt);

#ifdef __cplusplus
}
#endif
#endif
```

Measured before the change: 1.208 billion.

## Build actor span tables on device and overlap with merge instead of host

Adds a k_span_tables kernel that rebuilds the per-actor span and table-offset arrays on the GPU from the change briefs and plan block sums. It validates span ordering and falls back to a host-side redo path when the check fails. The plan scan is factored into a shared helper, and the plan kernel now also counts changes with no ops. The aim is to drop host-side table construction and upload from the critical path before the merge runs. In exchange it adds an extra kernel, a workspace clear and a last-block reduction, plus a fallback path that must re-run the decode.

Result: no change. 1.208 billion (-0.0%).

```diff
diff --git a/automerge_classic_amd/csrc/am355_api.hip b/automerge_classic_amd/csrc/am355_api.hip
--- a/automerge_classic_amd/csrc/am355_api.hip
+++ b/automerge_classic_amd/csrc/am355_api.hip
@@ -160,6 +160,21 @@
   return AM355_OK;
 }
 
+extern "C" int am355_chain_counters(const am355_ctx* c, uint64_t out[4]) {
+  if (!c || !out) return AM355_E_ARG;
+  out[0] = c->n_span_device;
+  out[1] = c->n_span_redo;
+  out[2] = c->counts.n_head_children;
+  out[3] = 0;
+  return AM355_OK;
+}
+
+extern "C" int am355_set_span_redo(am355_ctx* c, int on) {
+  if (!c) return AM355_E_ARG;
+  c->span_redo_next = on != 0;
+  return AM355_OK;
+}
+
 extern "C" int am355_get_raw(const am355_ctx* c, const uint8_t** arena, const uint64_t** offsets, uint32_t* n) {
   if (!c || !c->staged) return AM355_E_STATE;
   if (arena) *arena = c->raw.data();
@@ -496,6 +511,49 @@
   });
 }
 
+extern "C" int am355_test_span_build(am355_ctx* c, const void* briefs, uint32_t n, const uint32_t* slot_rank, uint32_t n_slots, const uint64_t* block_sums,
+                                     uint32_t n_sums, uint32_t n_distinct, uint32_t total_ops, uint32_t* region, uint32_t region_words, uint32_t spans_off,
+                                     uint32_t tab_off, uint32_t* words_out) {
+  if (!c || !region || !words_out || !slot_rank || !block_sums || (n && !briefs)) return AM355_E_ARG;
+  return guarded(c, [&]() -> int {
+    const size_t span_words = sizeof(ActorSpan) / 4 * (size_t)n;
+    if (n_slots == 0 || (n_slots & (n_slots - 1)) || n_sums < ((size_t)n + BLOCK - 1) / BLOCK * 8 || !span_build_takes(n, n_distinct) ||
+        (size_t)spans_off + span_words > region_words || (size_t)tab_off + n_distinct + 1 > region_words ||
+        ((size_t)spans_off < (size_t)tab_off + n_distinct + 1 && (size_t)tab_off < (size_t)spans_off + span_words))
+      return fail(c, AM355_E_ARG, "am355_test_span_build: a table leaves the region, the two overlap, or the inputs are short");
+    (void)hipSetDevice(c->device);
+    hipStream_t st = c->stream;
+    TestImage db, dr, ds, dreg;
+    DevBuf ws;
+    if (!db.up(briefs, sizeof(ChangeBrief) * (size_t)n, st) || !dr.up(slot_rank, 4 * (size_t)n_slots, st) || !ds.up(block_sums, 8 * (size_t)n_sums, st) ||
+        !dreg.up(region, 4 * (size_t)region_words, st) || !ws.ensure(span_build_bytes(n)))
+      return fail(c, AM355_E_NOMEM, "alloc");
+    span_build_clear(ws.p, st);
+    launch_span_tables((const ChangeBrief*)db.p, n, (const uint32_t*)dr.p, n_slots - 1, (const unsigned long long*)ds.p, n_distinct, total_ops, ws.p,
+                       (ActorSpan*)dreg.words(spans_off), dreg.words(tab_off), nullptr, 0, st);
+    dreg.down(region, st);
+    (void)hipMemcpyAsync(words_out, span_build_words(ws.p), 8, hipMemcpyDeviceToHost, st);
+    return test_finish(c);
+  });
+}
+
+extern "C" int am355_test_span_tables(am355_ctx* c, uint32_t* n_spans, uint32_t* n_tab, uint32_t* dev_spans, uint32_t* dev_tab, uint32_t* host_spans, uint32_t* host_tab) {
+  if (!c || !n_spans || !n_tab) return AM355_E_ARG;
+  if (!c->replayed || c->is_document || !c->p_spans || !c->p_tab_off) return AM355_E_STATE;
+  return guarded(c, [&]() -> int {
+    *n_spans = (uint32_t)c->spans.size();
+    *n_tab = (uint32_t)c->actor_tab_off.size();
+    if (!dev_spans || !dev_tab || !host_spans || !host_tab) return AM355_OK;
+    (void)hipSetDevice(c->device);
+    hipStream_t st = c->stream;
+    if (*n_spans) (void)hipMemcpyAsync(dev_spans, c->p_spans, sizeof(ActorSpan) * (size_t)*n_spans, hipMemcpyDeviceToHost, st);
+    if (*n_tab) (void)hipMemcpyAsync(dev_tab, c->p_tab_off, 4 * (size_t)*n_tab, hipMemcpyDeviceToHost, st);
+    if (*n_spans) memcpy(host_spans, c->spans.data(), sizeof(ActorSpan) * (size_t)*n_spans);
+    if (*n_tab) memcpy(host_tab, c->actor_tab_off.data(), 4 * (size_t)*n_tab);
+    return test_finish(c);
+  });
+}
+
 extern "C" int am355_get_rows(am355_ctx* c, uint32_t* obj_actor, uint32_t* obj_ctr, uint32_t* key_actor, uint32_t* key_ctr, uint32_t* key_off,
                               uint32_t* key_len, uint32_t* action, uint32_t* val_tl, uint32_t* val_off, uint32_t* pred_num, uint32_t* id_ctr,
                               uint32_t* id_actor, uint8_t* insert, uint32_t* succ_cnt) {
diff --git a/automerge_classic_amd/csrc/am355_ctx.h b/automerge_classic_amd/csrc/am355_ctx.h
--- a/automerge_classic_amd/csrc/am355_ctx.h
+++ b/automerge_classic_amd/csrc/am355_ctx.h
@@ -340,6 +340,7 @@
   HostBuf h_slots, h_hashes, h_has_dep, h_words, h_stage, h_s1;
   DevBuf d_s1;
   ChangeBrief* hp_briefs = nullptr;
+  const ChangeBrief* dp_briefs = nullptr;
   uint32_t* hp_distinct = nullptr;
   bool have_host_metas = false;
   uint32_t amap_cap = 0, slot_mask = 0, hash_mask = 0;
@@ -384,6 +385,11 @@
   DevBuf d_plans, d_amap, d_tables;
   ActorSpan* p_spans = nullptr;
   uint32_t* p_tab_off = nullptr;
+  DevBuf d_span_ws;
+  bool span_ws_clear = false;
+  bool spans_sorted = false;
+  bool span_redo_next = false;
+  uint64_t n_span_device = 0, n_span_redo = 0;
 
   DevBuf d_cols, d_pred, d_merge, d_sort, d_ir, d_counts;
   OpCols cols{};
diff --git a/automerge_classic_amd/csrc/am355_decode.h b/automerge_classic_amd/csrc/am355_decode.h
--- a/automerge_classic_amd/csrc/am355_decode.h
+++ b/automerge_classic_amd/csrc/am355_decode.h
@@ -26,6 +26,13 @@
 void launch_plan(const ChangeBrief* briefs, uint32_t n, const uint32_t* distinct, const uint32_t* slot_rank, uint32_t slot_mask, const unsigned long long* block_sums,
                  ChangePlan* plans, ChangePlan* plans_serial, const uint32_t* words, const uint32_t* plan_words, HostSignals* sig, uint32_t seq, hipStream_t st,
                  PlanTotals* dev_totals = nullptr, uint32_t* host_s1 = nullptr);
+constexpr uint32_t SPAN_BUILD_MAX_CHANGES = 65536;
+size_t span_build_bytes(uint32_t n);
+bool span_build_takes(uint32_t n, uint32_t n_distinct);
+void span_build_clear(void* ws, hipStream_t st);
+const uint32_t* span_build_words(const void* ws);
+void launch_span_tables(const ChangeBrief* briefs, uint32_t n, const uint32_t* slot_rank, uint32_t slot_mask, const unsigned long long* block_sums, uint32_t n_distinct,
+                        uint32_t total_ops, void* ws, ActorSpan* spans, uint32_t* tab_off, HostSignals* sig, uint32_t seq, hipStream_t st);
 void launch_decode_speculative(const uint8_t* arena, const ChangeMeta* metas, const ChangePlan* plans, uint32_t n_changes, const PlanTotals* totals, uint32_t cap_ops,
                                uint32_t cap_preds, uint32_t cap_distinct, const uint32_t* amap, const uint32_t* slot_rank, OpCols cols, uint32_t* flags, hipStream_t st,
                                hipStream_t aux, bool with_large, uint32_t shard_rank = 0, uint32_t shard_world = 1);
diff --git a/automerge_classic_amd/csrc/am355_decode.hip b/automerge_classic_amd/csrc/am355_decode.hip
--- a/automerge_classic_amd/csrc/am355_decode.hip
+++ b/automerge_classic_amd/csrc/am355_decode.hip
@@ -1140,21 +1140,60 @@
   block_scan3(valid ? br.n_ops : 0u, valid ? br.n_preds : 0u, valid ? br.n_entries : 0u, s_scan, ex, t1);
   block_scan3(small ? 1u : 0u, large ? 1u : 0u, serial ? 1u : 0u, s_scan, ex, t2);
   uint32_t mx_op = has ? br.start_op + br.n_ops - 1 : 0u, bad = in_range ? (br.flags_fits & 0x1fffffffu) : 0u, unknown = in_range ? (br.flags_fits & 0x20000000u) : 0u;
+  uint32_t no_ops = valid && !has ? 1u : 0u;
   for (int d = WAVE / 2; d >= 1; d >>= 1) {
     uint32_t o = __shfl_xor(mx_op, d), ob = __shfl_xor(bad, d), ou = __shfl_xor(unknown, d);
     mx_op = o > mx_op ? o : mx_op;
     bad |= ob;
     unknown |= ou;
+    no_ops += __shfl_xor(no_ops, d);
   }
   if ((threadIdx.x & (WAVE - 1)) == 0) {
     if (mx_op) atomicMax(&plan_words[1], mx_op);
     if (bad) atomicOr(&plan_words[2], bad);
     if (unknown) atomicOr(&plan_words[3], 1u);
+    if (no_ops) atomicAdd(&plan_words[4], no_ops);
   }
   if (threadIdx.x == 0) {
     unsigned long long* out = block_sums + (size_t)blockIdx.x * PLAN_SUMS;
     out[0] = t1[0]; out[1] = t1[1]; out[2] = t1[2]; out[3] = t2[0]; out[4] = t2[1]; out[5] = t2[2];
   }
+}
+
+struct PlanScan {
+  ChangeBrief br;
+  bool valid, has, small, large, serial;
+  unsigned long long e1[3], t1[3];
+  unsigned long long e2[3], t2[3];
+};
+template <bool CLASSES>
+__device__ __forceinline__ void plan_scan(const ChangeBrief* __restrict__ briefs, uint32_t n, const unsigned long long* __restrict__ block_sums,
+                                          unsigned long long (*s_scan)[3], unsigned long long* s_base, PlanScan& p) {
+  {
+    unsigned long long p0 = 0, p1 = 0, p2 = 0, p3 = 0, p4 = 0, p5 = 0;
+    for (uint32_t j = threadIdx.x; j < blockIdx.x; j += BLOCK) {
+      const unsigned long long* q = block_sums + (size_t)j * PLAN_SUMS;
+      p0 += q[0]; p1 += q[1]; p2 += q[2];
+      if (CLASSES) { p3 += q[3]; p4 += q[4]; p5 += q[5]; }
+    }
+    unsigned long long ex[3], t1[3], t2[3] = {0, 0, 0};
+    block_scan3(p0, p1, p2, s_scan, ex, t1);
+    if (CLASSES) block_scan3(p3, p4, p5, s_scan, ex, t2);
+    if (threadIdx.x == 0) { s_base[0] = t1[0]; s_base[1] = t1[1]; s_base[2] = t1[2]; s_base[3] = t2[0]; s_base[4] = t2[1]; s_base[5] = t2[2]; }
+    __syncthreads();
+  }
+  const uint32_t c = gtid();
+  const bool in_range = c < n;
+  p.br = ChangeBrief{};
+  if (in_range) p.br = briefs[c];
+  const ChangeBrief& br = p.br;
+  p.valid = in_range && !(br.flags_fits & 0x1fffffffu);
+  p.has = p.valid && br.n_ops != 0;
+  p.small = p.has && (br.flags_fits & 0x40000000u);
+  p.large = p.has && !p.small && (br.flags_fits & 0x80000000u);
+  p.serial = p.has && !p.small && !p.large;
+  block_scan3(p.valid ? br.n_ops : 0u, p.valid ? br.n_preds : 0u, p.valid ? br.n_entries : 0u, s_scan, p.e1, p.t1);
+  if (CLASSES) block_scan3(p.small ? 1u : 0u, p.large ? 1u : 0u, p.serial ? 1u : 0u, s_scan, p.e2, p.t2);
 }
 
 __global__ __launch_bounds__(BLOCK) void k_plan_apply(const ChangeBrief* __restrict__ briefs, uint32_t n, const uint32_t* __restrict__ slot_rank, uint32_t slot_mask,
@@ -1165,33 +1204,16 @@
   wave_priority_high();
   __shared__ unsigned long long s_scan[BLOCK / WAVE][3];
   __shared__ unsigned long long s_base[6];
-  {
-    unsigned long long p0 = 0, p1 = 0, p2 = 0, p3 = 0, p4 = 0, p5 = 0;
-    for (uint32_t j = threadIdx.x; j < blockIdx.x; j += BLOCK) {
-      const unsigned long long* q = block_sums + (size_t)j * PLAN_SUMS;
-      p0 += q[0]; p1 += q[1]; p2 += q[2]; p3 += q[3]; p4 += q[4]; p5 += q[5];
-    }
-    unsigned long long ex[3], t1[3], t2[3];
-    block_scan3(p0, p1, p2, s_scan, ex, t1);
-    block_scan3(p3, p4, p5, s_scan, ex, t2);
-    if (threadIdx.x == 0) { s_base[0] = t1[0]; s_base[1] = t1[1]; s_base[2] = t1[2]; s_base[3] = t2[0]; s_base[4] = t2[1]; s_base[5] = t2[2]; }
-    __syncthreads();
-  }
+  PlanScan p;
+  plan_scan<true>(briefs, n, block_sums, s_scan, s_base, p);
   const uint32_t c = gtid();
-  const bool in_range = c < n;
-  ChangeBrief br{};
-  if (in_range) br = briefs[c];
-  const bool valid = in_range && !(br.flags_fits & 0x1fffffffu);
-  const bool has = valid && br.n_ops != 0;
-  const bool small = has && (br.flags_fits & 0x40000000u), large = has && !small && (br.flags_fits & 0x80000000u), serial = has && !small && !large;
-  unsigned long long e1[3], e2[3], t1[3], t2[3];
-  block_scan3(valid ? br.n_ops : 0u, valid ? br.n_preds : 0u, valid ? br.n_entries : 0u, s_scan, e1, t1);
-  block_scan3(small ? 1u : 0u, large ? 1u : 0u, serial ? 1u : 0u, s_scan, e2, t2);
-  if (has) {
+  const ChangeBrief& br = p.br;
+  const unsigned long long *e1 = p.e1, *e2 = p.e2, *t1 = p.t1, *t2 = p.t2;
+  if (p.has) {
     ChangePlan pl{c, (uint32_t)(s_base[0] + e1[0]), (uint32_t)(s_base[1] + e1[1]), (uint32_t)(s_base[2] + e1[2]),
                   br.author_slot <= slot_mask ? slot_rank[br.author_slot] : 0u, br.n_entries};
-    if (small) plans[(uint32_t)(s_base[3] + e2[0])] = pl;
-    else if (large) plans[n - 1 - (uint32_t)(s_base[4] + e2[1])] = pl;
+    if (p.small) plans[(uint32_t)(s_base[3] + e2[0])] = pl;
+    else if (p.large) plans[n - 1 - (uint32_t)(s_base[4] + e2[1])] = pl;
     else plans_serial[(uint32_t)(s_base[5] + e2[2])] = pl;
   }
   if (blockIdx.x + 1 == gridDim.x && host_s1) {
@@ -1215,8 +1237,108 @@
     z.fallback = (plan_words[0] || ops >= 0x7ffffff0ull || preds >= 0xfffffff0ull || ent >= 0xfffffff0ull) ? 1u : 0u;
     z.flags_a = words[0] | plan_words[2]; z.fast_a = words[1]; z.total_entries = words[2]; z.n_distinct = distinct[0];
     z.reserved[0] = plan_words[3];
+    z.reserved[1] = plan_words[4];
     if (dev_totals) *dev_totals = z;
     signal_host((uint32_t*)&sig->plan, (const uint32_t*)&z, sizeof(PlanTotals) / 4, &sig->plan_seq, seq);
+  }
+}
+
+struct SpanItem { uint32_t rank, k, start_op, n_ops, op_base; };
+constexpr size_t SPAN_WS_WORDS = 16;
+constexpr uint32_t SPAN_RANKS_PER_THREAD = PLAN_RANK_MAX / BLOCK;
+static_assert(SPAN_RANKS_PER_THREAD * BLOCK == PLAN_RANK_MAX, "k_span_tables: the counters divide among the threads");
+
+__global__ __launch_bounds__(BLOCK) void k_span_tables(const ChangeBrief* __restrict__ briefs, uint32_t n, const uint32_t* __restrict__ slot_rank, uint32_t slot_mask,
+                                                       const unsigned long long* __restrict__ block_sums, uint32_t n_distinct, uint32_t total_ops, SpanItem* items,
+                                                       uint32_t* cnt, uint32_t* words, ActorSpan* spans, uint32_t* __restrict__ tab_off, HostSignals* sig, uint32_t seq) {
+  __shared__ unsigned long long s_scan[BLOCK / WAVE][3];
+  __shared__ unsigned long long s_base[6];
+  __shared__ uint32_t s_tab[PLAN_RANK_MAX + 1];
+  __shared__ uint32_t s_red[BLOCK / WAVE];
+  __shared__ uint32_t s_last, s_bad, s_placed;
+  const uint32_t t = threadIdx.x;
+  for (uint32_t k = t; k < PLAN_RANK_MAX; k += BLOCK) s_tab[k] = 0;
+  PlanScan p;
+  plan_scan<false>(briefs, n, block_sums, s_scan, s_base, p);
+  {
+    const uint32_t c = gtid();
+    SpanItem it{NONE32, NONE32, 0, 0, 0};
+    if (p.has) {
+      const uint32_t rank = p.br.author_slot <= slot_mask ? slot_rank[p.br.author_slot] : NONE32;
+      if (rank < n_distinct && rank < PLAN_RANK_MAX) {
+        const uint32_t k = p.br.seq >= 1 && p.br.seq - 1 < 0xffffffffull ? (uint32_t)(p.br.seq - 1) : NONE32;
+        it = SpanItem{rank, k, p.br.start_op, p.br.n_ops, (uint32_t)(s_base[0] + p.e1[0])};
+        atomicAdd(&s_tab[rank], 1u);
+      } else {
+        atomicOr(&words[0], 1u);
+      }
+    }
+    if (c < n) items[c] = it;
+    if (p.valid && !p.has) atomicAdd(&words[1], 1u);
+  }
+  __syncthreads();
+  for (uint32_t k = t; k < PLAN_RANK_MAX; k += BLOCK) {
+    const uint32_t v = s_tab[k];
+    if (v) atomicAdd(&cnt[k], v);
+  }
+  __threadfence();
+  __syncthreads();
+  if (t == 0) s_last = atomicAdd(&words[2], 1u) + 1 == gridDim.x ? 1u : 0u;
+  __syncthreads();
+  if (!s_last) return;
+  __threadfence();
+  const uint32_t nd = n_distinct < PLAN_RANK_MAX ? n_distinct : PLAN_RANK_MAX;
+  if (t == 0) { s_bad = (words[0] || n_distinct > PLAN_RANK_MAX) ? 1u : 0u; s_placed = 0; }
+  uint32_t v[SPAN_RANKS_PER_THREAD], mine = 0;
+#pragma unroll
+  for (uint32_t k = 0; k < SPAN_RANKS_PER_THREAD; k++) {
+    const uint32_t r = t * SPAN_RANKS_PER_THREAD + k;
+    v[k] = r < nd ? __hip_atomic_load(&cnt[r], __ATOMIC_RELAXED, __HIP_MEMORY_SCOPE_AGENT) : 0u;
+    mine += v[k];
+  }
+  uint32_t sum_all;
+  uint32_t ex = block_exclusive_scan_u32(mine, s_red, &sum_all);
+#pragma unroll
+  for (uint32_t k = 0; k < SPAN_RANKS_PER_THREAD; k++) {
+    s_tab[t * SPAN_RANKS_PER_THREAD + k] = ex;
+    ex += v[k];
+  }
+  if (t == BLOCK - 1) s_tab[PLAN_RANK_MAX] = ex;
+  __syncthreads();
+  uint32_t total = s_tab[nd];
+  if (total > n) total = 0;
+  uint32_t placed = 0;
+  for (uint32_t c = t; c < n; c += BLOCK) {
+    const SpanItem it = items[c];
+    if (it.rank == NONE32) continue;
+    const uint32_t first = it.rank < nd ? s_tab[it.rank] : 0u, len = it.rank < nd ? s_tab[it.rank + 1] - first : 0u;
+    if (it.k < len && first + it.k < total) { spans[first + it.k] = ActorSpan{it.start_op, it.n_ops, it.op_base}; placed++; }
+    else atomicOr(&s_bad, 1u);
+  }
+  if (placed) atomicAdd(&s_placed, placed);
+  __syncthreads();
+  if (t == 0 && s_placed != total) s_bad = 1;
+  for (uint32_t c = t; c < n; c += BLOCK) {
+    const SpanItem it = items[c];
+    if (it.rank == NONE32 || it.rank >= nd) continue;
+    const uint32_t first = s_tab[it.rank], len = s_tab[it.rank + 1] - first;
+    if (it.k >= len || first + it.k >= total) continue;
+    const ActorSpan s = spans[first + it.k];
+    bool ok = s.start_op == it.start_op && s.n_ops == it.n_ops && s.op_base == it.op_base && (unsigned long long)it.op_base + it.n_ops <= total_ops;
+    if (ok && it.k > 0) {
+      const ActorSpan q = spans[first + it.k - 1];
+      ok = (unsigned long long)q.start_op + q.n_ops <= it.start_op;
+    }
+    if (!ok) atomicOr(&s_bad, 1u);
+  }
+  __syncthreads();
+  const uint32_t bad = s_bad;
+  for (uint32_t i = t; i <= n_distinct; i += BLOCK) tab_off[i] = bad || i > nd ? 0u : s_tab[i];
+  if (t == 0) {
+    const uint32_t out[2] = {bad, words[1]};
+    words[4] = out[0];
+    words[5] = out[1];
+    if (sig) signal_host(sig->spans, out, 2, &sig->spans_seq, seq);
   }
 }
 
@@ -2248,6 +2370,24 @@
 
 size_t plan_block_sums_bytes(uint32_t n) { return sizeof(unsigned long long) * PLAN_SUMS * ((size_t)(n + BLOCK - 1) / BLOCK + 1); }
 
+size_t span_build_bytes(uint32_t n) { return 4 * (SPAN_WS_WORDS + PLAN_RANK_MAX) + sizeof(SpanItem) * (size_t)(n ? n : 1); }
+
+bool span_build_takes(uint32_t n, uint32_t n_distinct) { return n <= SPAN_BUILD_MAX_CHANGES && n_distinct <= PLAN_RANK_MAX; }
+
+void span_build_clear(void* ws, hipStream_t st) { (void)hipMemsetAsync(ws, 0, 4 * (SPAN_WS_WORDS + PLAN_RANK_MAX), st); }
+
+const uint32_t* span_build_words(const void* ws) { return (const uint32_t*)ws + 4; }
+
+void launch_span_tables(const ChangeBrief* briefs, uint32_t n, const uint32_t* slot_rank, uint32_t slot_mask, const unsigned long long* block_sums, uint32_t n_distinct,
+                        uint32_t total_ops, void* ws, ActorSpan* spans, uint32_t* tab_off, HostSignals* sig, uint32_t seq, hipStream_t st) {
+  uint32_t* words = (uint32_t*)ws;
+  uint32_t* cnt = words + SPAN_WS_WORDS;
+  SpanItem* items = (SpanItem*)(cnt + PLAN_RANK_MAX);
+  uint32_t nb = (n + BLOCK - 1) / BLOCK;
+  hipLaunchKernelGGL(k_span_tables, dim3(nb ? nb : 1), dim3(BLOCK), 0, st, briefs, n, slot_rank, slot_mask, block_sums, n_distinct, total_ops, items, cnt, words, spans,
+                     tab_off, sig, seq);
+}
+
 void launch_plan(const ChangeBrief* briefs, uint32_t n, const uint32_t* distinct, const uint32_t* slot_rank, uint32_t slot_mask, const unsigned long long* block_sums,
                  ChangePlan* plans, ChangePlan* plans_serial, const uint32_t* words, const uint32_t* plan_words, HostSignals* sig, uint32_t seq, hipStream_t st,
                  PlanTotals* dev_totals, uint32_t* host_s1) {
diff --git a/automerge_classic_amd/csrc/am355_internal.h b/automerge_classic_amd/csrc/am355_internal.h
--- a/automerge_classic_amd/csrc/am355_internal.h
+++ b/automerge_classic_amd/csrc/am355_internal.h
@@ -79,6 +79,8 @@
   uint32_t delta_end[16];
   volatile uint32_t mapmerge_seq;  uint32_t pad7[15];
   uint32_t mapmerge[16];
+  volatile uint32_t spans_seq;     uint32_t pad8[15];
+  uint32_t spans[16];
 };
 
 struct ActorSpan {
diff --git a/automerge_classic_amd/csrc/am355_merge.h b/automerge_classic_amd/csrc/am355_merge.h
--- a/automerge_classic_amd/csrc/am355_merge.h
+++ b/automerge_classic_amd/csrc/am355_merge.h
@@ -95,6 +95,8 @@
 enum { MERGE_FILL_ROWS = 1, MERGE_FILL_TABLES = 2 };
 bool merge_prepare(MergeBufs& b, hipStream_t aux, int what = MERGE_FILL_ROWS | MERGE_FILL_TABLES, const FillRanges* extra = nullptr);
 void merge_run(MergeBufs& b, PatchIR& ir, Counts* h_counts, hipStream_t st, hipEvent_t ev_counts, hipEvent_t ev_runs, bool resolved = false);
+void merge_run_first(MergeBufs& b, PatchIR& ir, Counts* h_counts, hipStream_t st, hipEvent_t ev_counts, hipEvent_t ev_runs, bool resolved = false);
+void merge_run_rest(MergeBufs& b, PatchIR& ir, Counts* h_counts, hipStream_t st, hipEvent_t ev_counts, hipEvent_t ev_runs);
 void merge_run_maps(MergeBufs& b, PatchIR& ir, Counts* h_counts, hipStream_t st);
 void merge_resolve(MergeBufs& b, hipStream_t st);
 
diff --git a/automerge_classic_amd/csrc/am355_merge.hip b/automerge_classic_amd/csrc/am355_merge.hip
--- a/automerge_classic_amd/csrc/am355_merge.hip
+++ b/automerge_classic_amd/csrc/am355_merge.hip
@@ -641,7 +641,10 @@
 }
 
 constexpr uint32_t HEAD_CHILD_MAX = 2048;
-constexpr uint32_t HEAD_CHILD_THREADS = 1024;
+constexpr uint32_t HEAD_CHILD_WGS = 4;
+constexpr uint32_t HEAD_CHILD_TILE = 512;
+constexpr uint32_t HEAD_CHILD_PER = HEAD_CHILD_MAX / (HEAD_CHILD_WGS * BLOCK);
+static_assert(HEAD_CHILD_PER * HEAD_CHILD_WGS * BLOCK == HEAD_CHILD_MAX, "head_children: every head child has a thread");
 
 __global__ __launch_bounds__(BLOCK) void k_child_push(MergeBufs b) {
   wave_priority_high();
@@ -654,33 +657,52 @@
   if (head_child && slot < HEAD_CHILD_MAX) b.head_child[slot] = v;
 }
 
-__global__ __launch_bounds__(HEAD_CHILD_THREADS) void k_head_children(MergeBufs b) {
-  wave_priority_high();
-  __shared__ unsigned long long s_id[HEAD_CHILD_MAX];
-  __shared__ uint32_t s_obj[HEAD_CHILD_MAX], s_row[HEAD_CHILD_MAX];
+__device__ __forceinline__ void head_children(const MergeBufs& b, uint32_t part) {
+  __shared__ unsigned long long s_id[HEAD_CHILD_TILE];
+  __shared__ uint32_t s_obj[HEAD_CHILD_TILE], s_row[HEAD_CHILD_TILE];
   const uint32_t n = b.counts->n_head_children;
-  if (n == 0 || n > HEAD_CHILD_MAX) return;
-  for (uint32_t k = threadIdx.x; k < n; k += HEAD_CHILD_THREADS) {
-    uint32_t v = b.head_child[k];
-    s_row[k] = v;
-    s_obj[k] = b.obj_row[v];
-    s_id[k] = pack_id(b.ops.id_ctr[v], b.ops.id_actor[v]);
-  }
-  __syncthreads();
-  for (uint32_t k = threadIdx.x; k < n; k += HEAD_CHILD_THREADS) {
-    const uint32_t obj = s_obj[k];
-    const unsigned long long kv = s_id[k];
-    unsigned long long best_id = 0;
-    uint32_t greater = 0, best = NONE32;
-    for (uint32_t j = 0; j < n; j++) {
-      if (s_obj[j] != obj || j == k) continue;
-      unsigned long long ku = s_id[j];
-      if (ku > kv) greater++;
-      else if (best == NONE32 || ku > best_id) { best = s_row[j]; best_id = ku; }
-    }
-    uint32_t v = s_row[k];
-    b.next_sib[v] = best;
-    if (greater == 0) b.first_child[b.n_ops + obj] = v;
+  if (n == 0 || n > HEAD_CHILD_MAX || part * BLOCK >= n) return;
+  uint32_t my_k[HEAD_CHILD_PER], my_row[HEAD_CHILD_PER], my_obj[HEAD_CHILD_PER], greater[HEAD_CHILD_PER], best[HEAD_CHILD_PER];
+  unsigned long long my_id[HEAD_CHILD_PER], best_id[HEAD_CHILD_PER];
+#pragma unroll
+  for (uint32_t m = 0; m < HEAD_CHILD_PER; m++) {
+    const uint32_t k = (m * HEAD_CHILD_WGS + part) * BLOCK + threadIdx.x;
+    my_k[m] = k;
+    my_row[m] = my_obj[m] = 0; my_id[m] = best_id[m] = 0;
+    greater[m] = 0; best[m] = NONE32;
+    if (k < n) {
+      const uint32_t v = b.head_child[k];
+      my_row[m] = v;
+      my_obj[m] = b.obj_row[v];
+      my_id[m] = pack_id(b.ops.id_ctr[v], b.ops.id_actor[v]);
+    }
+  }
+  for (uint32_t t0 = 0; t0 < n; t0 += HEAD_CHILD_TILE) {
+    const uint32_t cnt = n - t0 < HEAD_CHILD_TILE ? n - t0 : HEAD_CHILD_TILE;
+    for (uint32_t j = threadIdx.x; j < cnt; j += BLOCK) {
+      const uint32_t v = b.head_child[t0 + j];
+      s_row[j] = v;
+      s_obj[j] = b.obj_row[v];
+      s_id[j] = pack_id(b.ops.id_ctr[v], b.ops.id_actor[v]);
+    }
+    __syncthreads();
+#pragma unroll
+    for (uint32_t m = 0; m < HEAD_CHILD_PER; m++) {
+      if (my_k[m] >= n) continue;
+      for (uint32_t j = 0; j < cnt; j++) {
+        if (s_obj[j] != my_obj[m] || t0 + j == my_k[m]) continue;
+        const unsigned long long ku = s_id[j];
+        if (ku > my_id[m]) greater[m]++;
+        else if (best[m] == NONE32 || ku > best_id[m]) { best[m] = s_row[j]; best_id[m] = ku; }
+      }
+    }
+    __syncthreads();
+  }
+#pragma unroll
+  for (uint32_t m = 0; m < HEAD_CHILD_PER; m++) {
+    if (my_k[m] >= n) continue;
+    b.next_sib[my_row[m]] = best[m];
+    if (greater[m] == 0) b.first_child[b.n_ops + my_obj[m]] = my_row[m];
   }
 }
 
@@ -688,9 +710,15 @@
 __global__ __launch_bounds__(BLOCK) void k_child_order(MergeBufs b, uint32_t* __restrict__ is_head) {
   wave_priority_high();
   __shared__ uint32_t s_red[BLOCK / WAVE];
+  constexpr uint32_t EXTRA = FROM_LINKS ? 0u : HEAD_CHILD_WGS;
+  if (blockIdx.x < EXTRA) {
+    head_children(b, blockIdx.x);
+    return;
+  }
+  const uint32_t wg = blockIdx.x - EXTRA;
   const uint32_t ni = b.counts->n_list_ins;
-  if (blockIdx.x * BLOCK >= ni) return;
-  uint32_t i = gtid();
+  if (wg * BLOCK >= ni) return;
+  uint32_t i = wg * BLOCK + threadIdx.x;
   uint32_t head = 0;
   if (i < ni) {
     const OpCols& o = b.ops;
@@ -727,7 +755,7 @@
     head = (i > 0 && ps == b.ins_row[i - 1] && first && none_after) ? 0u : 1u;
     is_head[i] = head;
   }
-  carry_publish(b.cs_runs, head, s_red);
+  carry_publish_at(b.cs_runs, head, s_red, wg);
 }
 
 __global__ __launch_bounds__(BLOCK) void k_run_heads(MergeBufs b, const uint32_t* __restrict__ is_head, uint32_t* __restrict__ head_ex,
@@ -1548,7 +1576,36 @@
   if (b.n_ops) hipLaunchKernelGGL(k_resolve, grid_for(std::max(b.n_ops - b.first_row, 1u)), dim3(BLOCK), 0, st, b);
 }
 
+void merge_run_first(MergeBufs& b, PatchIR& ir, Counts* hc, hipStream_t st, hipEvent_t ev_counts, hipEvent_t ev_runs, bool resolved) {
+  const uint32_t N = b.n_ops;
+  if (!N) return;
+  Counts* hc_runs = hc + 1;
+  uint32_t* is_head = b.scan_a;
+  uint32_t* head_ex = b.scan_b;
+  uint32_t* heads = b.run_heads;
+  uint32_t* row_run = b.row_run;
+  if (!resolved) hipLaunchKernelGGL(k_resolve, grid_for(std::max(N - b.first_row, 1u)), dim3(BLOCK), 0, st, b);
+  hipLaunchKernelGGL(k_emit, grid_for(N), dim3(BLOCK), 0, st, b);
+  hipLaunchKernelGGL(k_compact_rows, grid_for(N), dim3(BLOCK), 0, st, b, ir);
+  if (!b.sig) (void)hipMemcpyAsync(hc, b.counts, sizeof(Counts), hipMemcpyDeviceToHost, st);
+  if (ev_counts) (void)hipEventRecord(ev_counts, st);
+  hipLaunchKernelGGL(k_child_push, grid_for(N), dim3(BLOCK), 0, st, b);
+  hipLaunchKernelGGL(k_child_order<false>, dim3(grid_for(N).x + HEAD_CHILD_WGS), dim3(BLOCK), 0, st, b, is_head);
+  hipLaunchKernelGGL(k_run_heads, grid_for(N), dim3(BLOCK), 0, st, b, (const uint32_t*)is_head, head_ex, heads, row_run);
+  if (!b.sig) {
+    (void)hipMemcpyAsync(hc_runs, b.counts, sizeof(Counts), hipMemcpyDeviceToHost, st);
+    (void)hipEventRecord(ev_runs, st);
+  }
+  AM355_LAUNCH_INDEPENDENT(k_euler_init_runs, grid_for(N), dim3(BLOCK), st, b, (const uint32_t*)heads, (const uint32_t*)row_run, b.euler_a);
+  hipLaunchKernelGGL(k_euler_rank_lds, dim3(1), dim3(EULER_LDS_THREADS), 0, st, b.counts, b.euler_a);
+}
+
 void merge_run(MergeBufs& b, PatchIR& ir, Counts* hc, hipStream_t st, hipEvent_t ev_counts, hipEvent_t ev_runs, bool resolved) {
+  merge_run_first(b, ir, hc, st, ev_counts, ev_runs, resolved);
+  merge_run_rest(b, ir, hc, st, ev_counts, ev_runs);
+}
+
+void merge_run_rest(MergeBufs& b, PatchIR& ir, Counts* hc, hipStream_t st, hipEvent_t ev_counts, hipEvent_t ev_runs) {
   const uint32_t N = b.n_ops;
   const bool trace = getenv("AM355_TRACE") != nullptr;
   auto t_begin = std::chrono::steady_clock::now();
@@ -1567,23 +1624,6 @@
   uint32_t* head_ex = b.scan_b;
   uint32_t* heads = b.run_heads;
   uint32_t* row_run = b.row_run;
-  if (!resolved) hipLaunchKernelGGL(k_resolve, grid_for(std::max(N - b.first_row, 1u)), dim3(BLOCK), 0, st, b);
-  hipLaunchKernelGGL(k_emit, grid_for(N), dim3(BLOCK), 0, st, b);
-  hipLaunchKernelGGL(k_compact_rows, grid_for(N), dim3(BLOCK), 0, st, b, ir);
-  if (!b.sig) (void)hipMemcpyAsync(hc, b.counts, sizeof(Counts), hipMemcpyDeviceToHost, st);
-  if (ev_counts) (void)hipEventRecord(ev_counts, st);
-  hipLaunchKernelGGL(k_child_push, grid_for(N), dim3(BLOCK), 0, st, b);
-  hipLaunchKernelGGL(k_head_children, dim3(1), dim3(HEAD_CHILD_THREADS), 0, st, b);
-  hipLaunchKernelGGL(k_child_order<false>, grid_for(N), dim3(BLOCK), 0, st, b, is_head);
-  hipLaunchKernelGGL(k_run_heads, grid_for(N), dim3(BLOCK), 0, st, b, (const uint32_t*)is_head, head_ex, heads, row_run);
-  if (!b.sig) {
-    (void)hipMemcpyAsync(hc_runs, b.counts, sizeof(Counts), hipMemcpyDeviceToHost, st);
-    (void)hipEventRecord(ev_runs, st);
-  }
-  AM355_LAUNCH_INDEPENDENT(k_euler_init_runs, grid_for(N), dim3(BLOCK), st, b, (const uint32_t*)heads, (const uint32_t*)row_run, b.euler_a);
-  hipLaunchKernelGGL(k_euler_rank_lds, dim3(1), dim3(EULER_LDS_THREADS), 0, st, b.counts, b.euler_a);
-
-  lap("first half enqueued");
   MapKeyStats key_stats;
   if (b.sig) read_phase_counts(b, &b.sig->counts_seq, b.sig->counts, hc, st, &key_stats);
   else (void)hipEventSynchronize(ev_counts);
diff --git a/automerge_classic_amd/csrc/am355_replay.hip b/automerge_classic_amd/csrc/am355_replay.hip
--- a/automerge_classic_amd/csrc/am355_replay.hip
+++ b/automerge_classic_amd/csrc/am355_replay.hip
@@ -423,6 +423,7 @@
   c->max_op = max_op;
   c->clock_seq.clear();
   for (uint32_t a : c->clock_actor) c->clock_seq.push_back(clock[a]);
+  c->spans_sorted = false;
   c->actor_tab_off.assign(na + 1, 0);
   for (uint32_t a = 0; a < na; a++) c->actor_tab_off[a + 1] = c->actor_tab_off[a] + span_cnt[a];
   c->spans.resize(c->actor_tab_off[na]);
@@ -433,7 +434,10 @@
     size_t k_n = c->actor_tab_off[a + 1] - c->actor_tab_off[a];
     bool sorted = true;
     for (size_t k = 1; k < k_n; k++) sorted = sorted && v[k - 1].start_op <= v[k].start_op;
-    if (!sorted) std::sort(v, v + k_n, [](const ActorSpan& x, const ActorSpan& y) { return x.start_op < y.start_op; });
+    if (!sorted) {
+      std::sort(v, v + k_n, [](const ActorSpan& x, const ActorSpan& y) { return x.start_op < y.start_op; });
+      c->spans_sorted = true;
+    }
     for (size_t k = 1; k < k_n; k++)
       if ((uint64_t)v[k - 1].start_op + v[k - 1].n_ops > v[k].start_op) {
         c->flags |= AM355_F_DUP_OPID;
@@ -688,12 +692,30 @@
   c->spec_launched = false;
   const bool second_class = tot.n_small && (tot.n_large || tot.n_serial);
   hipStream_t fill_stream = second_class ? c->stream4 : c->stream3;
+  const bool dev_tables = !go && tot.reserved[1] == 0 && span_build_takes(n, n_distinct) && c->shard_world == 1 && c->dp_briefs && c->span_ws_clear;
+  c->span_ws_clear = false;
+  HostSignals* sig = c->h_sig.as<HostSignals>();
+  if (dev_tables)
+    launch_span_tables(c->dp_briefs, n, c->d_slot_rank.as<uint32_t>(), c->slot_mask, c->d_plan_sums.as<unsigned long long>(), n_distinct, tot.n_ops, c->d_span_ws.p,
+                       c->p_spans, c->p_tab_off, sig, c->sig_seq, c->stream4);
   if (!merge_prepare(c->mb, fill_stream)) return fail(c, AM355_E_DEVICE, "merge fills: more ranges than one launch takes");
   if (second_class) {
     HIPCHK(c, hipEventRecord(c->ev_join, c->stream3));
     HIPCHK(c, hipStreamWaitEvent(st, c->ev_join, 0));
   }
   lap("fills enqueued");
+  Counts* hc = c->h_counts.as<Counts>();
+  const hipEvent_t ev_counts = (c->phase_events || !c->mb.sig) ? c->ev_counts.h : nullptr;
+  if (dev_tables) {
+    if (!second_class) {
+      HIPCHK(c, hipEventRecord(c->ev_fills, fill_stream));
+      HIPCHK(c, hipStreamWaitEvent(c->stream4, c->ev_fills, 0));
+    }
+    HIPCHK(c, hipEventRecord(c->ev_tables, c->stream4));
+    HIPCHK(c, hipStreamWaitEvent(st, c->ev_tables, 0));
+    merge_run_first(c->mb, c->ir, hc, st, ev_counts, c->ev_runs);
+    lap("tables and first half of the merge enqueued");
+  }
   if (go) HIPCHK(c, hipEventSynchronize(go->ready));
   auto t0 = std::chrono::steady_clock::now();
   std::vector<uint32_t> slot_rank;
@@ -702,8 +724,8 @@
   lap("plan_fast done");
   if (rc == AM355_OK && (c->n_ops != tot.n_ops || c->n_preds != tot.n_preds || c->max_op != tot.max_op || c->actors.size() != n_distinct))
     rc = fail(c, AM355_E_DEVICE, "internal: device and host plans disagree (%llu / %u ops)", (unsigned long long)c->n_ops, tot.n_ops);
-  if (rc) { (void)hipStreamSynchronize(st); return rc; }
-  {
+  if (rc) { (void)hipStreamSynchronize(c->stream4); (void)hipStreamSynchronize(c->stream3); (void)hipStreamSynchronize(st); return rc; }
+  auto upload_host_tables = [&]() -> int {
     uint8_t* h = c->h_stage.as<uint8_t>();
     size_t b_spans = sizeof(ActorSpan) * c->spans.size(), b_tab = 4 * c->actor_tab_off.size();
     if (b_spans) memcpy(h, c->spans.data(), b_spans);
@@ -711,10 +733,46 @@
     HIPCHK(c, hipMemcpyAsync(d_tables, h, o_tab + b_tab, hipMemcpyHostToDevice, fill_stream));
     HIPCHK(c, hipEventRecord(c->ev_tables, fill_stream));
     HIPCHK(c, hipStreamWaitEvent(st, c->ev_tables, 0));
-  }
-  lap("tables enqueued");
-  Counts* hc = c->h_counts.as<Counts>();
-  merge_run(c->mb, c->ir, hc, st, (c->phase_events || !c->mb.sig) ? c->ev_counts.h : nullptr, c->ev_runs);
+    return AM355_OK;
+  };
+  if (dev_tables) {
+    const bool told = wait_host_signal(&sig->spans_seq, c->sig_seq, c->stream4);
+    const bool withdrawn = !told || sig->spans[0] != 0;
+    const bool redo = withdrawn || c->spans_sorted || c->span_redo_next;
+    c->span_redo_next = false;
+    if (!redo) {
+      c->n_span_device++;
+      merge_run_rest(c->mb, c->ir, hc, st, ev_counts, c->ev_runs);
+    } else {
+      c->n_span_redo++;
+      HIPCHK(c, hipStreamSynchronize(st));
+      c->sig_seq++;
+      c->mb.sig_seq = c->sig_seq;
+      HIPCHK(c, hipMemsetAsync(c->d_counts.p, 0, c->mb.counts_bytes, st));
+      if (!merge_prepare(c->mb, st)) return fail(c, AM355_E_DEVICE, "merge fills: more ranges than one launch takes");
+      if (second_class) {
+        HIPCHK(c, hipEventRecord(c->ev_fork, st));
+        HIPCHK(c, hipStreamWaitEvent(c->stream3, c->ev_fork, 0));
+      }
+      launch_decode_planned(c->d_arena.as<uint8_t>(), c->d_metas.as<ChangeMeta>(), c->d_plans.as<ChangePlan>(), c->d_plans.as<ChangePlan>() + std::max(n, 1u), n,
+                            tot.n_small, tot.n_large, tot.n_serial, c->d_amap_prov.as<uint32_t>(), c->d_slot_rank.as<uint32_t>(), c->cols,
+                            &c->d_counts.as<Counts>()->flags, st, c->stream3, c->shard_rank, c->shard_world);
+      if (second_class) {
+        HIPCHK(c, hipEventRecord(c->ev_join, c->stream3));
+        HIPCHK(c, hipStreamWaitEvent(st, c->ev_join, 0));
+      }
+      fill_stream = st;
+      int ru = upload_host_tables();
+      if (ru) return ru;
+      lap("span tables redone by the host");
+      merge_run(c->mb, c->ir, hc, st, ev_counts, c->ev_runs);
+    }
+  } else {
+    int ru = upload_host_tables();
+    if (ru) return ru;
+    lap("tables enqueued");
+    merge_run(c->mb, c->ir, hc, st, ev_counts, c->ev_runs);
+  }
   HIPCHK(c, hipEventRecord(c->ev[5], st));
   if (hc->flags) return error_for_flags(c, hc->flags, "op set rejected");
   c->counts = *hc;
@@ -1782,6 +1840,7 @@
   const uint32_t* h_wa = c->h_s1.as<uint32_t>();
   c->hp_distinct = (uint32_t*)(c->h_s1.as<uint8_t>() + s1_distinct);
   c->hp_briefs = (ChangeBrief*)(c->h_s1.as<uint8_t>() + s1_briefs);
+  c->dp_briefs = d_briefs;
   uint32_t* d_words = c->d_words.as<uint32_t>();
   uint32_t* h_words = c->h_words.as<uint32_t>();
   HostSignals* sig = c->h_sig.as<HostSignals>();
@@ -1867,6 +1926,10 @@
     launch_plan(d_briefs, n, d_distinct, c->d_slot_rank.as<uint32_t>(), c->slot_mask, c->d_plan_sums.as<unsigned long long>(), c->d_plans.as<ChangePlan>(),
                 c->d_plans.as<ChangePlan>() + n1, d_wa, d_wa + 8, sig, c->sig_seq, sa, spec_possible ? c->d_plan_totals.as<PlanTotals>() : nullptr,
                 c->h_s1.as<uint32_t>());
+    if (attempt == 0) {
+      c->span_ws_clear = span_build_takes(n, 0) && c->shard_world == 1 && c->d_span_ws.ensure(span_build_bytes(n));
+      if (c->span_ws_clear) span_build_clear(c->d_span_ws.p, c->stream4);
+    }
     const bool want_large_spec = spec_possible && attempt == 0 && c->hint_large != 0;
     if (want_large_spec) HIPCHK(c, hipEventRecord(c->ev_plan, sa));
     if (spec_possible && attempt == 0) {
diff --git a/automerge_classic_amd/csrc/am355_scan.h b/automerge_classic_amd/csrc/am355_scan.h
--- a/automerge_classic_amd/csrc/am355_scan.h
+++ b/automerge_classic_amd/csrc/am355_scan.h
@@ -53,14 +53,15 @@
   size_t wgs = ((size_t)n_elems + BLOCK - 1) / BLOCK + 1;
   return wgs + (wgs >> CARRY_GROUP_SHIFT) + 2;
 }
-__device__ __forceinline__ uint32_t carry_publish(const CarryScan& c, uint32_t v, uint32_t* s) {
+__device__ __forceinline__ uint32_t carry_publish_at(const CarryScan& c, uint32_t v, uint32_t* s, uint32_t wg) {
   uint32_t total = block_sum_u32(v, s);
   if (threadIdx.x == 0) {
-    c.wg_sum[blockIdx.x] = total;
-    if (total) atomicAdd(&c.group_sum[(size_t)(blockIdx.x >> CARRY_GROUP_SHIFT) * CARRY_GROUP_STRIDE], total);
+    c.wg_sum[wg] = total;
+    if (total) atomicAdd(&c.group_sum[(size_t)(wg >> CARRY_GROUP_SHIFT) * CARRY_GROUP_STRIDE], total);
   }
   return total;
 }
+__device__ __forceinline__ uint32_t carry_publish(const CarryScan& c, uint32_t v, uint32_t* s) { return carry_publish_at(c, v, s, blockIdx.x); }
 __device__ __forceinline__ uint32_t carry_prefix(const CarryScan& c, uint32_t v, uint32_t* s) {
   uint32_t g = blockIdx.x >> CARRY_GROUP_SHIFT, first = g << CARRY_GROUP_SHIFT;
   uint32_t part = 0;
diff --git a/automerge_classic_amd/engine.py b/automerge_classic_amd/engine.py
--- a/automerge_classic_amd/engine.py
+++ b/automerge_classic_amd/engine.py
@@ -79,7 +79,8 @@
                     ("am355_test_sort_bits", [vp, vp, vp, u32, ci, ci, vp, ctypes.POINTER(ci)]), ("am355_test_chain_mark", [vp, vp, vp, u32, u32]),
                     ("am355_test_remap", [vp, vp, u32, u32, vp, u32, vp, u32, ctypes.POINTER(u32)]), ("am355_test_fill", [vp, vp, u32, u32, vp, u32, ctypes.POINTER(u32)]),
                     ("am355_test_copy", [vp, vp, sz, vp, sz, ci, vp, u32, ctypes.POINTER(u32)]), ("am355_test_signal_words", [vp, vp, u32, vp, u32, u32, vp, u32, vp]),
-                    ("am355_test_carried_scan", [vp, vp, u32, vp, vp, vp])):
+                    ("am355_test_carried_scan", [vp, vp, u32, vp, vp, vp]), ("am355_chain_counters", [vp, vp]), ("am355_set_span_redo", [vp, ci]),
+                    ("am355_test_span_build", [vp, vp, u32, vp, u32, vp, u32, u32, u32, vp, u32, u32, u32, vp]), ("am355_test_span_tables", [vp] * 7)):
         if not hasattr(L, f):
             continue
         getattr(L, f).argtypes = args
@@ -468,6 +469,31 @@
         self._check(self._L.am355_test_carried_scan(self._h, v.ctypes.data, v.size, out.ctypes.data, out_wg.ctypes.data, tot.ctypes.data))
         return out, out_wg, tot
 
+    def chain_counters(self):
+        out = (ctypes.c_uint64 * 4)()
+        self._check(self._L.am355_chain_counters(self._h, out))
+        return int(out[0]), int(out[1]), int(out[2])
+
+    def set_span_redo(self, on=True):
+        self._check(self._L.am355_set_span_redo(self._h, 1 if on else 0))
+
+    def span_build(self, briefs, slot_rank, block_sums, n_distinct, total_ops, region, spans_off, tab_off):
+        b = np.ascontiguousarray(briefs)
+        assert b.itemsize == 32
+        r, s, reg = self._img(slot_rank), self._img(block_sums, np.uint64), self._img(region)
+        w = np.zeros(2, dtype=np.uint32)
+        self._check(self._L.am355_test_span_build(self._h, b.ctypes.data if b.size else None, b.size, r.ctypes.data, r.size, s.ctypes.data, s.size, n_distinct, total_ops,
+                                                  reg.ctypes.data, reg.size, spans_off, tab_off, w.ctypes.data))
+        return reg, int(w[0]), int(w[1])
+
+    def span_tables(self):
+        ns, nt = ctypes.c_uint32(0), ctypes.c_uint32(0)
+        self._check(self._L.am355_test_span_tables(self._h, ctypes.byref(ns), ctypes.byref(nt), None, None, None, None))
+        ds, hs = np.full((ns.value, 3), 0xA5A5A5A5, dtype=np.uint32), np.zeros((ns.value, 3), dtype=np.uint32)
+        dt, ht = np.full(nt.value, 0xA5A5A5A5, dtype=np.uint32), np.zeros(nt.value, dtype=np.uint32)
+        self._check(self._L.am355_test_span_tables(self._h, ctypes.byref(ns), ctypes.byref(nt), ds.ctypes.data, dt.ctypes.data, hs.ctypes.data, ht.ctypes.data))
+        return ds, dt, hs, ht
+
     def rows(self):
         n = int(self.stats().n_ops)
         names = ["obj_actor", "obj_ctr", "key_actor", "key_ctr", "key_off", "key_len", "action", "val_tl", "val_off", "pred_num",
diff --git a/include/am355.h b/include/am355.h
--- a/include/am355.h
+++ b/include/am355.h
@@ -179,6 +179,11 @@
 int am355_test_signal_words(am355_ctx *ctx, const uint32_t *a, uint32_t n_a, const uint32_t *b, uint32_t n_b, uint32_t seq, uint32_t *host_words, uint32_t host_words_n,
                             uint32_t *seq_word);
 int am355_test_carried_scan(am355_ctx *ctx, const uint32_t *v, uint32_t n, uint32_t *out, uint32_t *out_wg, uint32_t *wg_total);
+int am355_chain_counters(const am355_ctx *ctx, uint64_t out[4]);
+int am355_set_span_redo(am355_ctx *ctx, int on);
+int am355_test_span_build(am355_ctx *ctx, const void *briefs, uint32_t n, const uint32_t *slot_rank, uint32_t n_slots, const uint64_t *block_sums, uint32_t n_sums,
+                          uint32_t n_distinct, uint32_t total_ops, uint32_t *region, uint32_t region_words, uint32_t spans_off, uint32_t tab_off, uint32_t *words_out);
+int am355_test_span_tables(am355_ctx *ctx, uint32_t *n_spans, uint32_t *n_tab, uint32_t *dev_spans, uint32_t *dev_tab, uint32_t *host_spans, uint32_t *host_tab);
 int am355_get_rows(am355_ctx *ctx, uint32_t *obj_actor, uint32_t *obj_ctr, uint32_t *key_actor, uint32_t *key_ctr, uint32_t *key_off,
                    uint32_t *key_len, uint32_t *action, uint32_t *val_tl, uint32_t *val_off, uint32_t *pred_num, uint32_t *id_ctr,
                    uint32_t *id_actor, uint8_t *insert, uint32_t *succ_cnt);
```
